# khiner/MeshEditor

Measured on AMD Instinct MI355X. Metric: eigenpairs/sec (K/M assembly + 50-mode solve, 100k-tet mesh), higher is better.
Workload: dtype f64; 1 GPU; cube_s100k: Kuhn mesh 105456 tets / 446631 DOF, NumModes=50 NumFemModes=65, P=10 excitation points, one mesh per GPU; eigenpairs_per_mesh=65, kept_modes_per_mesh=50, parallelism=mesh-per-gpu x1

## Files before the change

mesheditor_amd/csrc/lab/mh_lab.hip:

```cpp
#include "../mh_common.h"
#include "modalhip_lab.h"

#include <algorithm>

void mh_elementwise_apply(mh_context *ctx, const mh_system *sys, double sigma, const double *x, double *y, uint32_t w);

namespace {
constexpr int TB = 256;
__global__ void k_lab_ref_to_panel(const double *__restrict__ x, const uint32_t *__restrict__ perm, uint32_t nnodes, uint32_t width, double *__restrict__ panel) {
    const size_t i = size_t(blockIdx.x) * blockDim.x + threadIdx.x;
    if (i >= size_t(nnodes) * 3 * width) return;
    const uint32_t c = uint32_t(i % width), comp = uint32_t((i / width) % 3), node = uint32_t(i / (size_t(3) * width));
    panel[i] = x[size_t(c) * (size_t(3) * nnodes) + size_t(3) * perm[node] + comp];
}
__global__ void k_lab_panel_to_ref(const double *__restrict__ panel, const uint32_t *__restrict__ perm, uint32_t nnodes, uint32_t width, double *__restrict__ y) {
    const size_t i = size_t(blockIdx.x) * blockDim.x + threadIdx.x;
    if (i >= size_t(nnodes) * 3 * width) return;
    const uint32_t c = uint32_t(i % width), comp = uint32_t((i / width) % 3), node = uint32_t(i / (size_t(3) * width));
    y[size_t(c) * (size_t(3) * nnodes) + size_t(3) * perm[node] + comp] = panel[i];
}
}

namespace {
typedef float f4_stream __attribute__((ext_vector_type(4)));
__global__ void __launch_bounds__(256) k_stream_copy(const f4_stream *__restrict__ src, f4_stream *__restrict__ dst, size_t count) {
    for (size_t i = size_t(blockIdx.x) * 256 + threadIdx.x; i < count; i += size_t(gridDim.x) * 256) dst[i] = src[i];
}
template<int U, bool NT, int T = 256, bool NTL = NT> __global__ void __launch_bounds__(T) k_stream_copy_u(const f4_stream *__restrict__ src, f4_stream *__restrict__ dst, size_t count) {
    const size_t stride = size_t(gridDim.x) * T;
    for (size_t base = size_t(blockIdx.x) * T + threadIdx.x; base < count; base += stride * U) {
        f4_stream v[U];
#pragma unroll
        for (int u = 0; u < U; ++u) {
            const size_t i = base + size_t(u) * stride;
            if (i < count) v[u] = NTL ? __builtin_nontemporal_load(src + i) : src[i];
        }
#pragma unroll
        for (int u = 0; u < U; ++u) {
            const size_t i = base + size_t(u) * stride;
            if (i < count) {
                if (NT) __builtin_nontemporal_store(v[u], dst + i);
                else dst[i] = v[u];
            }
        }
    }
}
template<int U, bool NT> __global__ void __launch_bounds__(256) k_stream_read_u(const f4_stream *__restrict__ src, size_t count, float *__restrict__ out) {
    const size_t stride = size_t(gridDim.x) * 256;
    f4_stream acc = {0, 0, 0, 0};
    for (size_t base = size_t(blockIdx.x) * 256 + threadIdx.x; base < count; base += stride * U) {
        f4_stream v[U];
#pragma unroll
        for (int u = 0; u < U; ++u) {
            const size_t i = base + size_t(u) * stride;
            v[u] = i < count ? (NT ? __builtin_nontemporal_load(src + i) : src[i]) : f4_stream{0, 0, 0, 0};
        }
#pragma unroll
        for (int u = 0; u < U; ++u) acc += v[u];
    }
    float s = acc[0] + acc[1] + acc[2] + acc[3];
    for (int off = 32; off > 0; off >>= 1) s += __shfl_xor(s, off, 64);
    if ((threadIdx.x & 63) == 0) atomicAdd(out + blockIdx.x, s);
}
__global__ void __launch_bounds__(256) k_stream_read(const f4_stream *__restrict__ src, size_t count, float *__restrict__ out) {
    f4_stream acc = {0, 0, 0, 0};
    for (size_t i = size_t(blockIdx.x) * 256 + threadIdx.x; i < count; i += size_t(gridDim.x) * 256) acc += src[i];
    float s = acc[0] + acc[1] + acc[2] + acc[3];
    for (int off = 32; off > 0; off >>= 1) s += __shfl_xor(s, off, 64);
    if ((threadIdx.x & 63) == 0) atomicAdd(out + blockIdx.x, s);
}
}

namespace {
std::vector<uint32_t> lab_point_ref(const mh_system *s) {
    const std::vector<uint32_t> perm = s->perm.to_host(), corner = s->p1_corner.to_host();
    std::vector<uint32_t> ref(s->n_points);
    std::vector<uint8_t> seen(s->n_points, 0);
    for (uint32_t p = 0; p < s->n_points; ++p) {
        ref[p] = perm[corner[p]];
        if (ref[p] >= s->n_points || seen[ref[p]]) mh_throw(MH_EINVAL, "hierarchy export: P1 point %u has reference id %u", p, ref[p]);
        seen[ref[p]] = 1;
    }
    return ref;
}
const PatchSet &lab_patches(const mh_system *s, int level) { return level == 2 ? s->patches2 : s->patches1; }
}

extern "C" {
uint32_t mhl_graph_aggregates(const uint32_t *row_ptr, const uint32_t *col, uint32_t n, uint32_t target, uint32_t max_order, uint32_t *agg_of) {
    std::vector<uint32_t> rp(row_ptr, row_ptr + n + 1), cl(col, col + row_ptr[n]), out;
    const uint32_t na = mh_graph_aggregates(rp, cl, n, target, max_order, out);
    std::copy(out.begin(), out.end(), agg_of);
    return na;
}

int mhl_system_elementwise_matvec(mh_system *s, const double *x, double *y, uint32_t width) {
    if (!s || !x || !y || width == 0) return MH_EINVAL;
    mh_context *ctx = s->ctx;
    try {
        HIP_CHECK(hipSetDevice(ctx->device));
        const size_t n = size_t(3) * s->n_nodes;
        DevArray<double> xr(ctx, n * width), xp(ctx, n * width), yp(ctx, n * width);
        xr.upload(x, n * width);
        k_lab_ref_to_panel<<<div_up(n * width, TB), TB, 0, ctx->stream>>>(xr, s->perm, s->n_nodes, width, xp);
        KERNEL_CHECK();
        mh_elementwise_apply(ctx, s, -15791.367041742974, xp, yp, width);
        k_lab_panel_to_ref<<<div_up(n * width, TB), TB, 0, ctx->stream>>>(yp, s->perm, s->n_nodes, width, xr.get());
        KERNEL_CHECK();
        xr.download(y, n * width);
        return MH_OK;
    } catch (const std::exception &e) { return mh_guard(ctx, e); }
}

int mhl_system_bench_spmm(mh_system *s, uint32_t width, uint32_t reps, double *avg_ms, double *algorithmic_bytes) {
    if (!s || width == 0 || reps == 0 || !avg_ms) return MH_EINVAL;
    mh_context *ctx = s->ctx;
    try {
        HIP_CHECK(hipSetDevice(ctx->device));
        const size_t n = size_t(3) * s->n_nodes;
        DevArray<double> x(ctx, n * width), y(ctx, n * width);
        std::vector<double> hx(n * width);
        for (size_t i = 0; i < hx.size(); ++i) hx[i] = double((i * 2654435761u) % 1000) * 1e-3 - 0.5;
        x.upload(hx.data(), hx.size());
        HIP_CHECK(hipStreamSynchronize(ctx->stream));
        for (int warm = 0; warm < 2; ++warm) mh_spmm(ctx, s->L2, s->L2.kval, x, y, nullptr, nullptr, width);
        hipEvent_t e0, e1;
        HIP_CHECK(hipEventCreate(&e0));
        HIP_CHECK(hipEventCreate(&e1));
        HIP_CHECK(hipEventRecord(e0, ctx->stream));
        for (uint32_t r = 0; r < reps; ++r) mh_spmm(ctx, s->L2, s->L2.kval, x, y, nullptr, nullptr, width);
        HIP_CHECK(hipEventRecord(e1, ctx->stream));
        HIP_CHECK(hipEventSynchronize(e1));
        float ms = 0;
        HIP_CHECK(hipEventElapsedTime(&ms, e0, e1));
        (void)hipEventDestroy(e0);
        (void)hipEventDestroy(e1);
        *avg_ms = ms / reps;
        if (algorithmic_bytes) *algorithmic_bytes = 76.0 * double(s->L2.n_blocks) + 4.0 * (double(s->n_nodes) + 1) + 16.0 * double(n) * width;
        return MH_OK;
    } catch (const std::exception &e) { return mh_guard(ctx, e); }
}

int mhl_system_bench_cheb_step(mh_system *s, int level, uint32_t width, uint32_t slabs, uint32_t reps, double *avg_ms) {
    if (!s || !avg_ms || width == 0 || slabs == 0 || width % (4 * slabs) || reps == 0 || (level != 1 && level != 2)) return MH_EINVAL;
    mh_context *ctx = s->ctx;
    try {
        HIP_CHECK(hipSetDevice(ctx->device));
        const BsrLevel &lvl = level == 2 ? s->L2 : s->L1;
        if (!lvl.aval32.get() || !lvl.dinv32.get()) mh_throw(MH_EINVAL, "bench_cheb_step: no single-precision operator (solve the system once first)");
        const size_t n = size_t(3) * lvl.n_nodes;
        const uint32_t wc = width / slabs;
        std::vector<DevArray<float>> d(slabs), d2(slabs), r(slabs), x(slabs);
        std::vector<float> h(n * wc);
        for (size_t i = 0; i < h.size(); ++i) h[i] = float((i * 2654435761u) % 1000) * 1e-3f - 0.5f;
        for (uint32_t q = 0; q < slabs; ++q) {
            for (auto *a : {&d[q], &d2[q], &r[q], &x[q]}) {
                a->reset(ctx, n * wc);
                a->upload(h.data(), h.size());
            }
        }
        HIP_CHECK(hipStreamSynchronize(ctx->stream));
        auto run = [&] {
            for (uint32_t q = 0; q < slabs; ++q)
                if (!mh_spmm_f32_cheb_step(ctx, lvl, d[q], d2[q], r[q], x[q], lvl.dinv32, 0.3f, 0.1f, wc)) mh_throw(MH_EINVAL, "bench_cheb_step: width %u not served by the wide kernel", wc);
        };
        run();
        run();
        hipEvent_t e0, e1;
        HIP_CHECK(hipEventCreate(&e0));
        HIP_CHECK(hipEventCreate(&e1));
        HIP_CHECK(hipEventRecord(e0, ctx->stream));
        for (uint32_t rep = 0; rep < reps; ++rep) run();
        HIP_CHECK(hipEventRecord(e1, ctx->stream));
        HIP_CHECK(hipEventSynchronize(e1));
        float ms = 0;
        HIP_CHECK(hipEventElapsedTime(&ms, e0, e1));
        (void)hipEventDestroy(e0);
        (void)hipEventDestroy(e1);
        *avg_ms = ms / reps;
        return MH_OK;
    } catch (const std::exception &e) { return mh_guard(ctx, e); }
}

int mhl_system_bench_elementwise(mh_system *s, uint32_t width, uint32_t reps, double *avg_ms) {
    if (!s || width == 0 || reps == 0 || !avg_ms) return MH_EINVAL;
    mh_context *ctx = s->ctx;
    try {
        HIP_CHECK(hipSetDevice(ctx->device));
        const size_t n = size_t(3) * s->n_nodes;
        DevArray<double> x(ctx, n * width), y(ctx, n * width);
        std::vector<double> hx(n * width);
        for (size_t i = 0; i < hx.size(); ++i) hx[i] = double((i * 2654435761u) % 1000) * 1e-3 - 0.5;
        x.upload(hx.data(), hx.size());
        HIP_CHECK(hipStreamSynchronize(ctx->stream));
        for (int warm = 0; warm < 2; ++warm) mh_elementwise_apply(ctx, s, -15791.367041742974, x, y, width);
        hipEvent_t e0, e1;
        HIP_CHECK(hipEventCreate(&e0));
        HIP_CHECK(hipEventCreate(&e1));
        HIP_CHECK(hipEventRecord(e0, ctx->stream));
        for (uint32_t r = 0; r < reps; ++r) mh_elementwise_apply(ctx, s, -15791.367041742974, x, y, width);
        HIP_CHECK(hipEventRecord(e1, ctx->stream));
        HIP_CHECK(hipEventSynchronize(e1));
        float ms = 0;
        HIP_CHECK(hipEventElapsedTime(&ms, e0, e1));
        (void)hipEventDestroy(e0);
        (void)hipEventDestroy(e1);
        *avg_ms = ms / reps;
        return MH_OK;
    } catch (const std::exception &e) { return mh_guard(ctx, e); }
}

}

namespace {
double lab_mapped_update_mismatches(mh_context *ctx, bool gaps, size_t n, uint32_t wa, uint32_t wb) {
    const uint32_t b = (wa + wa / 2 + 3u) & ~1u, pitch = (wa + 1u) & ~1u, m = wa + 2 * wb, nc = wa + wb;
    std::vector<uint32_t> map(wa);
    for (uint32_t k = 0; k < wa; ++k) map[k] = gaps ? k + k / 2 : k;
    auto fill = [](std::vector<double> &v, size_t salt) {
        for (size_t i = 0; i < v.size(); ++i) v[i] = double(((i + salt) * 2654435761u) % 1000) * 1e-3 - 0.5;
    };
    std::vector<double> hx(n * b), hw(n * wb), hp(n * wb), hc(size_t(m) * nc);
    fill(hx, 0), fill(hw, 7919), fill(hp, 104729), fill(hc, 1299709);
    struct Out { std::vector<double> xn, x, p; };
    auto run = [&](int form) {
        DevArray<double> dx(ctx, n * b), dw(ctx, n * wb), dp(ctx, n * wb), dc(ctx, size_t(m) * nc), dxn(ctx, n * pitch), dpo(ctx, n * wb);
        DevArray<uint32_t> dmap(ctx, wa);
        dx.upload(hx.data(), hx.size());
        dw.upload(hw.data(), hw.size());
        dp.upload(hp.data(), hp.size());
        dc.upload(hc.data(), hc.size());
        dmap.upload(map.data(), wa);
        dxn.zero();
        if (form == 0) mh_combine(ctx, n, dx, wa, dw, wb, dp, wb, dc, nc, dxn, wa, dpo, false, b, dmap, pitch);
        else mh_combine(ctx, n, dx, wa, dw, wb, dp, wb, dc, nc, dxn, wa, dpo, false, b, dmap, pitch, nullptr, 0, 0, dx, b, dmap);
        Out o{std::vector<double>(n * pitch), std::vector<double>(n * b), std::vector<double>(n * wb)};
        dxn.download(o.xn.data(), o.xn.size());
        dx.download(o.x.data(), o.x.size());
        dpo.download(o.p.data(), o.p.size());
        return o;
    };
    const Out one = run(0), two = run(1);
    auto differing = [](const std::vector<double> &a, const std::vector<double> &c) {
        size_t d = 0;
        for (size_t i = 0; i < a.size(); ++i) d += !(a[i] == c[i]);
        return d;
    };
    size_t bad = differing(one.x, hx);
    for (size_t r = 0; r < n; ++r)
        for (uint32_t c = 0; c < nc; ++c) {
            double ref = 0, mag = 0;
            for (uint32_t k = 0; k < m; ++k) {
                const double s = k < wa ? hx[r * b + map[k]] : k < wa + wb ? hw[r * wb + (k - wa)] : hp[r * wb + (k - wa - wb)];
                ref += s * hc[size_t(k) * nc + c];
                mag += std::abs(s * hc[size_t(k) * nc + c]);
            }
            const double got = c < wa ? one.xn[r * pitch + c] : one.p[r * wb + (c - wa)];
            bad += !(std::abs(got - ref) <= 2.0 * m * 2.3e-16 * mag);
        }
    std::vector<double> want = hx;
    size_t written = 0;
    for (size_t r = 0; r < n; ++r)
        for (uint32_t k = 0; k < wa; ++k) {
            want[r * b + map[k]] = one.xn[r * pitch + k];
            written += want[r * b + map[k]] != hx[r * b + map[k]];
        }
    if (written < n * wa / 2) mh_throw(MH_EHIP, "mapped update check: the update left %zu of %zu entries as they were", n * wa - written, n * size_t(wa));
    bad += differing(two.xn, one.xn) + differing(two.x, want) + differing(two.p, one.p);
    return double(bad);
}
}

extern "C" {
int mhl_context_bench_dense(mh_context *ctx, int kind, uint64_t n, uint32_t wa, uint32_t wb, uint32_t reps, double *avg_ms) {
    if (!ctx || !avg_ms || n == 0 || wa == 0 || wb == 0 || reps == 0 || kind < 0 || kind > 3) return MH_EINVAL;
    try {
        HIP_CHECK(hipSetDevice(ctx->device));
        std::lock_guard<std::mutex> lock(mh_solve_mutex());
        if (kind >= 2) {
            *avg_ms = lab_mapped_update_mismatches(ctx, kind == 3, n, wa, wb);
            return MH_OK;
        }
        DevArray<double> x(ctx, n * wa), y(ctx, n * wb), g(ctx, size_t(wa + wb) * (wa + wb)), z(ctx, n * wa);
        std::vector<double> h(n * std::max(wa, wb));
        for (size_t i = 0; i < h.size(); ++i) h[i] = double((i * 2654435761u) % 1000) * 1e-3 - 0.5;
        x.upload(h.data(), n * wa);
        y.upload(h.data(), n * wb);
        g.upload(h.data(), g.count);
        HIP_CHECK(hipStreamSynchronize(ctx->stream));
        auto run = [&]() {
            if (kind == 0) mh_gram(ctx, n, x, wa, y, wb, g, wa);
            else mh_combine(ctx, n, x, wa, y, wb, nullptr, 0, g, wa, z, wa, nullptr);
        };
        run();
        hipEvent_t e0, e1;
        HIP_CHECK(hipEventCreate(&e0));
        HIP_CHECK(hipEventCreate(&e1));
        HIP_CHECK(hipEventRecord(e0, ctx->stream));
        for (uint32_t r = 0; r < reps; ++r) run();
        HIP_CHECK(hipEventRecord(e1, ctx->stream));
        HIP_CHECK(hipEventSynchronize(e1));
        float ms = 0;
        HIP_CHECK(hipEventElapsedTime(&ms, e0, e1));
        (void)hipEventDestroy(e0);
        (void)hipEventDestroy(e1);
        *avg_ms = ms / reps;
        return MH_OK;
    } catch (const std::exception &e) { return mh_guard(ctx, e); }
}

int mhl_context_tridiagonalize_full(mh_context *ctx, int variant, uint32_t m, const double *a, double *d, double *e, double *reflectors, double *tau, uint32_t reps, double *avg_ms);
int mhl_context_tridiagonalize(mh_context *ctx, int variant, uint32_t m, const double *a, double *d, double *e, uint32_t reps, double *avg_ms) {
    return mhl_context_tridiagonalize_full(ctx, variant, m, a, d, e, nullptr, nullptr, reps, avg_ms);
}

int mhl_context_tridiagonalize_full(mh_context *ctx, int variant, uint32_t m, const double *a, double *d, double *e, double *reflectors, double *tau, uint32_t reps, double *avg_ms) {
    if (!ctx || !a || !d || !e || m < 2 || variant < 0 || variant > 3 || m > (variant == 2 ? 768u : 256u)) return MH_EINVAL;
    try {
        HIP_CHECK(hipSetDevice(ctx->device));
        MhSharedPhase not_during_a_factorisation(ctx->device);
        DevArray<double> da(ctx, size_t(m) * m), work(ctx, size_t(m) * m), dd(ctx, m), de(ctx, m), dtau(ctx, m);
        da.upload(a, size_t(m) * m);
        hipEvent_t e0, e1;
        HIP_CHECK(hipEventCreate(&e0));
        HIP_CHECK(hipEventCreate(&e1));
        float total = 0;
        for (uint32_t r = 0; r < std::max(1u, reps); ++r) {
            HIP_CHECK(hipMemcpyAsync(work, da, size_t(m) * m * sizeof(double), hipMemcpyDeviceToDevice, ctx->stream));
            HIP_CHECK(hipEventRecord(e0, ctx->stream));
            if (variant == 2) mh_sytrd_wide(ctx, work, m, dd, de, dtau);
            else mh_sytrd_small(ctx, work, m, dd, de, dtau, variant);
            HIP_CHECK(hipEventRecord(e1, ctx->stream));
            HIP_CHECK(hipEventSynchronize(e1));
            float ms = 0;
            HIP_CHECK(hipEventElapsedTime(&ms, e0, e1));
            total += ms;
        }
        (void)hipEventDestroy(e0);
        (void)hipEventDestroy(e1);
        dd.download(d, m);
        de.download(e, m - 1);
        if (reflectors) work.download(reflectors, size_t(m) * m);
        if (tau) dtau.download(tau, m);
        if (mh_sytrd_gave_up(ctx)) mh_throw(MH_EHIP, "tridiagonalisation: a workgroup timed out waiting for the others' values");
        if (avg_ms) *avg_ms = total / std::max(1u, reps);
        return MH_OK;
    } catch (const std::exception &e) { return mh_guard(ctx, e); }
}

int mhl_context_tridiag_lowest(mh_context *ctx, uint32_t m, uint32_t k, const double *d, const double *e, double *w, double *z, double *quality, int *taken) {
    if (!ctx || !d || !e || !w || !z || !quality || !taken || m < 2 || m > 768 || k < 1) return MH_EINVAL;
    try {
        HIP_CHECK(hipSetDevice(ctx->device));
        MhSharedPhase not_during_a_factorisation(ctx->device);
        DevArray<double> dd(ctx, m), de(ctx, m), dw(ctx, k), dz(ctx, size_t(m) * k);
        dd.upload(d, m);
        de.zero();
        de.upload(e, m - 1);
        bool ok;
        double q = std::numeric_limits<double>::quiet_NaN();
        if (m <= 256) {
            DevArray<double> ufac(ctx, size_t(3) * m * k), qv(ctx, 8), lam(ctx, k);
            ok = mh_tridiag_lowest(ctx, dd, de, m, k, dw, dz, m, ufac, qv, lam);
            if (ok) qv.download(&q, 1);
        } else {
            DevArray<double> work(ctx, size_t(5) * k * m + size_t(2) * k * k + 8);
            DevArray<int> info(ctx, 2);
            ok = mh_tridiag_lowest_wide(ctx, dd, de, m, k, dw, dz, m, work, info, &q);
        }
        *taken = ok ? 1 : 0;
        if (ok) {
            dw.download(w, k);
            dz.download(z, size_t(m) * k);
            *quality = q;
        }
        HIP_CHECK(hipStreamSynchronize(ctx->stream));
        return MH_OK;
    } catch (const std::exception &ex) { return mh_guard(ctx, ex); }
}

int mhl_context_rr_solve(mh_context *ctx, uint32_t m, const double *a, const double *mmat, uint32_t nwant, int gm_is_identity, double *evals, double *vectors, uint32_t *ncols,
                         double *host_evals, double *trace) {
    if (!ctx || !a || (!mmat && !gm_is_identity) || !evals || !vectors || !ncols || !trace || m < 1 || m > 1024 || nwant > m) return MH_EINVAL;
    struct TraceOn {
        mh_context *ctx;
        ~TraceOn() { ctx->rr_trace = nullptr; }
    };
    try {
        HIP_CHECK(hipSetDevice(ctx->device));
        MhSharedPhase not_during_a_factorisation(ctx->device);
        const size_t mm = size_t(m) * m;
        DevArray<double> gA(ctx, mm), gM(ctx, mm), ev(ctx, m), ework(ctx, m);
        DevArray<int> info(ctx, 2);
        info.zero();
        gA.upload(a, mm);
        if (mmat) gM.upload(mmat, mm);
        else gM.zero();
        if (ctx->rr_check) HIP_CHECK(hipMemsetAsync(ctx->rr_check, 0, sizeof(unsigned long long), ctx->stream));
        MhRrTrace tr;
        std::vector<double> hv;
        int hinfo;
        {
            ctx->rr_trace = &tr;
            TraceOn off{ctx};
            hinfo = mh_rr_solve(ctx, gA, gM, m, ev, ework, info, nwant, gm_is_identity != 0, host_evals ? &hv : nullptr);
        }
        unsigned long long check = 0;
        if (ctx->rr_check) HIP_CHECK(hipMemcpyAsync(&check, ctx->rr_check, sizeof(check), hipMemcpyDeviceToHost, ctx->stream));
        HIP_CHECK(hipStreamSynchronize(ctx->stream));
        double checkd;
        memcpy(&checkd, &check, sizeof(checkd));
        const bool partial = tr.solver == MhRrTrace::SMALL_PARTIAL || tr.solver == MhRrTrace::WIDE_PARTIAL;
        *ncols = hinfo ? 0 : (partial ? nwant : m);
        trace[0] = tr.reduction, trace[1] = tr.defect, trace[2] = tr.solver, trace[3] = tr.quality, trace[4] = checkd, trace[5] = double(hv.size());
        if (hinfo) return MH_EFACTOR;
        ev.download(evals, *ncols);
        gA.download(vectors, size_t(m) * *ncols);
        if (host_evals && !hv.empty()) std::copy(hv.begin(), hv.end(), host_evals);
        return MH_OK;
    } catch (const std::exception &ex) { return mh_guard(ctx, ex); }
}

int mhl_system_precondition(mh_system *s, double sigma, int precision, const double *x, double *y, uint32_t width) {
    if (!s || !x || !y || width == 0 || width > 1024 || (precision != 0 && precision != 1)) return MH_EINVAL;
    mh_context *ctx = s->ctx;
    try {
        HIP_CHECK(hipSetDevice(ctx->device));
        const size_t n = size_t(3) * s->n_nodes;
        DevArray<double> xr(ctx, n * width), xp(ctx, n * width), yp(ctx, n * width);
        xr.upload(x, n * width);
        k_lab_ref_to_panel<<<div_up(n * width, TB), TB, 0, ctx->stream>>>(xr, s->perm, s->n_nodes, width, xp);
        KERNEL_CHECK();
        mh_precondition_panel(s, sigma, precision, xp, yp, width);
        k_lab_panel_to_ref<<<div_up(n * width, TB), TB, 0, ctx->stream>>>(yp, s->perm, s->n_nodes, width, xr.get());
        KERNEL_CHECK();
        xr.download(y, n * width);
        return MH_OK;
    } catch (const std::exception &e) { return mh_guard(ctx, e); }
}

int mhl_system_hierarchy_sizes(mh_system *s, double sigma, int rebuild, uint64_t *sizes) {
    if (!s || !sizes) return MH_EINVAL;
    mh_context *ctx = s->ctx;
    try {
        HIP_CHECK(hipSetDevice(ctx->device));
        std::lock_guard<std::mutex> lock(mh_solve_mutex());
        if (rebuild) s->hierarchy_ready = false;
        mh_build_hierarchy(s, sigma);
        sizes[0] = s->n_points, sizes[1] = s->n_agg, sizes[2] = uint64_t(6) * s->n_agg, sizes[3] = s->L1.n_blocks;
        for (int level : {2, 1}) {
            const PatchSet &ps = lab_patches(s, level);
            uint64_t *o = sizes + (level == 2 ? 4 : 12);
            o[0] = ps.n_patches, o[1] = ps.npe, o[2] = ps.n_clusters, o[3] = ps.cluster_rows, o[4] = ps.cinv64.count, o[5] = ps.n_bad_elements,
            o[6] = ps.largest_cluster, o[7] = s->dropped_patches[level == 2 ? 0 : 1];
        }
        return MH_OK;
    } catch (const std::exception &e) { return mh_guard(ctx, e); }
}

int mhl_system_hierarchy_export(mh_system *s, uint32_t width, double *scalars, uint32_t *agg_of, double *agg_t, uint32_t *l1_row, uint32_t *l1_col, double *l1_val,
                                double *a0) {
    if (!s || !scalars || width == 0) return MH_EINVAL;
    mh_context *ctx = s->ctx;
    try {
        HIP_CHECK(hipSetDevice(ctx->device));
        std::lock_guard<std::mutex> lock(mh_solve_mutex());
        if (!s->hierarchy_ready) mh_throw(MH_EINVAL, "hierarchy export: no hierarchy built");
        MhCycleShape sh;
        mh_cycle_shape(s, width, &sh);
        const double sc[10] = {s->L2.lmax, s->L1.lmax, mh_coarse_lift(s), double(sh.deg2), sh.ratio, double(sh.deg1), double(sh.gamma), sh.ratio1, s->sigma_built,
                               double(s->worst_quality)};
        std::copy(sc, sc + 10, scalars);
        const std::vector<uint32_t> ref = lab_point_ref(s);
        if (agg_of) {
            const std::vector<uint32_t> h = s->agg_of.to_host();
            for (uint32_t p = 0; p < s->n_points; ++p) agg_of[ref[p]] = h[p];
        }
        if (agg_t) {
            const std::vector<double> h = s->agg_t.to_host();
            for (uint32_t p = 0; p < s->n_points; ++p) std::copy(h.begin() + 18 * size_t(p), h.begin() + 18 * size_t(p + 1), agg_t + 18 * size_t(ref[p]));
        }
        if (l1_row || l1_col) {
            const std::vector<uint32_t> rp = s->L1.row_ptr.to_host(), cl = s->L1.col.to_host();
            for (uint32_t r = 0; r < s->L1.n_nodes; ++r)
                for (uint32_t b = rp[r]; b < rp[r + 1]; ++b) {
                    if (l1_row) l1_row[b] = ref[r];
                    if (l1_col) l1_col[b] = ref[cl[b]];
                }
        }
        if (l1_val) s->L1.aval.download(l1_val, s->L1.n_blocks * 9);
        if (a0) s->a0.download(a0, s->a0.count);
        return MH_OK;
    } catch (const std::exception &e) { return mh_guard(ctx, e); }
}

int mhl_system_patch_export(mh_system *s, int level, uint32_t *nodes, double *weight, double *inv64, uint32_t *cluster_row, uint32_t *cluster_ptr, double *cinv64) {
    if (!s || (level != 1 && level != 2)) return MH_EINVAL;
    mh_context *ctx = s->ctx;
    try {
        HIP_CHECK(hipSetDevice(ctx->device));
        std::lock_guard<std::mutex> lock(mh_solve_mutex());
        if (!s->hierarchy_ready) mh_throw(MH_EINVAL, "patch export: no hierarchy built");
        const PatchSet &ps = lab_patches(s, level);
        std::vector<uint32_t> node_ref;
        if (level == 2) node_ref = s->perm.to_host();
        else node_ref = lab_point_ref(s);
        if (nodes && ps.n_patches) {
            const std::vector<uint32_t> h = ps.nodes.to_host();
            for (size_t i = 0; i < h.size(); ++i) nodes[i] = node_ref[h[i]];
        }
        if (weight && ps.n_patches) ps.weight.download(weight, ps.n_patches);
        if (inv64 && ps.n_patches) ps.inv64.download(inv64, ps.inv64.count);
        if (cluster_row && ps.n_clusters) {
            const std::vector<uint32_t> h = ps.cluster_row.to_host();
            for (size_t i = 0; i < h.size(); ++i) cluster_row[i] = 3 * node_ref[h[i] / 3] + h[i] % 3;
        }
        if (cluster_ptr && ps.n_clusters) std::copy(ps.h_cluster_ptr.begin(), ps.h_cluster_ptr.end(), cluster_ptr);
        if (cinv64 && ps.n_clusters) ps.cinv64.download(cinv64, ps.cinv64.count);
        return MH_OK;
    } catch (const std::exception &e) { return mh_guard(ctx, e); }
}

int mhl_context_potrf_inverse(mh_context *ctx, uint32_t w, const double *a, const double *dscale, double *l, double *linv, int *info2) {
    if (!ctx || !a || !dscale || !l || !linv || !info2 || w < 1 || w > 128) return MH_EINVAL;
    try {
        HIP_CHECK(hipSetDevice(ctx->device));
        MhSharedPhase not_during_a_factorisation(ctx->device);
        DevArray<double> da(ctx, size_t(w) * w), dd(ctx, w), dl(ctx, size_t(w) * w);
        DevArray<int> info(ctx, 2);
        da.upload(a, size_t(w) * w);
        dd.upload(dscale, w);
        mh_potrf_small_inverse(ctx, da, w, info, dd, dl);
        da.download(l, size_t(w) * w);
        dl.download(linv, size_t(w) * w);
        info.download(info2, 2);
        return MH_OK;
    } catch (const std::exception &e) { return mh_guard(ctx, e); }
}

int mhl_context_spd_inverse(mh_context *ctx, uint32_t w, const double *a, double *out, uint32_t reps, double *avg_ms) {
    if (!ctx || !a || !out || w < 1 || w > 128) return MH_EINVAL;
    try {
        HIP_CHECK(hipSetDevice(ctx->device));
        MhSharedPhase not_during_a_factorisation(ctx->device);
        DevArray<double> da(ctx, size_t(w) * w), dout(ctx, size_t(w) * w);
        DevArray<int> info(ctx, 1);
        info.zero();
        da.upload(a, size_t(w) * w);
        hipEvent_t e0, e1;
        HIP_CHECK(hipEventCreate(&e0));
        HIP_CHECK(hipEventCreate(&e1));
        float total = 0;
        for (uint32_t r = 0; r < std::max(1u, reps); ++r) {
            HIP_CHECK(hipEventRecord(e0, ctx->stream));
            mh_spd_inverse_small(ctx, da, w, w, dout, w, info);
            HIP_CHECK(hipEventRecord(e1, ctx->stream));
            HIP_CHECK(hipEventSynchronize(e1));
            float ms = 0;
            HIP_CHECK(hipEventElapsedTime(&ms, e0, e1));
            total += ms;
        }
        (void)hipEventDestroy(e0);
        (void)hipEventDestroy(e1);
        dout.download(out, size_t(w) * w);
        int hinfo = 0;
        info.download(&hinfo, 1);
        if (avg_ms) *avg_ms = total / std::max(1u, reps);
        return hinfo ? MH_EFACTOR : MH_OK;
    } catch (const std::exception &e) { return mh_guard(ctx, e); }
}

int mhl_context_small_gemm(mh_context *ctx, int ta, int tb, uint32_t M, uint32_t N, uint32_t K, double alpha, const double *a, uint32_t lda, const double *b, uint32_t ldb, double beta,
                           double *c, uint32_t ldc, uint32_t reps, double *avg_ms) {
    if (!ctx || !a || !b || !c || !M || !N || !K || lda < (ta ? K : M) || ldb < (tb ? N : K) || ldc < M) return MH_EINVAL;
    try {
        HIP_CHECK(hipSetDevice(ctx->device));
        MhSharedPhase not_during_a_factorisation(ctx->device);
        const size_t na = size_t(lda) * (ta ? M : K), nb = size_t(ldb) * (tb ? K : N), nc = size_t(ldc) * N;
        DevArray<double> da(ctx, na), db(ctx, nb), dc(ctx, nc), work(ctx, nc);
        da.upload(a, na);
        db.upload(b, nb);
// ... 232 lines not shown
```

mesheditor_amd/csrc/mh_common.h:

```cpp
#pragma once
#include "../../include/modalhip.h"

#include <hip/hip_runtime.h>
#include <rocblas/rocblas.h>
#include <rocsolver/rocsolver.h>

#include <algorithm>
#include <cstdarg>
#include <cstdio>
#include <cstdlib>
#include <cstring>
#include <iterator>
#include <limits>
#include <atomic>
#include <map>
#include <memory>
#include <mutex>
#include <stdexcept>
#include <string>
#include <vector>

struct MhError : std::runtime_error {
    int code;
    MhError(int c, const std::string &m) : std::runtime_error(m), code(c) {}
// ... 239 lines not shown
            ahead_ev.push_back(e);
        }
        return aux2_stream != nullptr;
    }
    rocblas_handle blas{nullptr};
    rocblas_handle blas_aux{nullptr};
    DevicePool pool;
    std::string last_error;
    hipEvent_t ev0{nullptr}, ev1{nullptr};
    void *gram_ws{nullptr};
    size_t gram_ws_bytes{0};
    uint32_t *iota{nullptr};
    unsigned long long *sytrd_xch{nullptr};
    uint32_t sytrd_epoch{0};
    int *sytrd_flag{nullptr};
    unsigned long long *sytrd_xch_wide{nullptr};
    uint32_t sytrd_epoch_wide{0};
    bool exchange_disabled{false};
    uint32_t sytrd_redos{0};
    unsigned long long *rr_check{nullptr};
    struct MhRrTrace *rr_trace{nullptr};
    bool time_kernels{false};
    std::vector<std::pair<hipEvent_t, hipEvent_t>> timer_events;
    std::vector<double> timer_work;
    std::vector<int> timer_class;
    size_t timer_used{0};
    struct ClassTotals {
        double ms{0}, work{0};
        uint64_t launches{0};
    } totals[MH_KERNEL_CLASSES];
};
void mh_timer_flush(mh_context *ctx);
struct TimedLaunch {
    mh_context *ctx;
    bool on;
    size_t slot{0};
    TimedLaunch(mh_context *c, int kernel_class, double work) : ctx(c), on(c->time_kernels) {
        if (!on) return;
        if (ctx->timer_used == ctx->timer_events.size()) {
            hipEvent_t a, b;
            HIP_CHECK(hipEventCreate(&a));
            HIP_CHECK(hipEventCreate(&b));
            ctx->timer_events.emplace_back(a, b);
            ctx->timer_work.push_back(0);
            ctx->timer_class.push_back(0);
        }
        slot = ctx->timer_used++;
        ctx->timer_work[slot] = work;
        ctx->timer_class[slot] = kernel_class;
        HIP_CHECK(hipEventRecord(ctx->timer_events[slot].first, ctx->stream));
    }
    ~TimedLaunch() {
        if (on) (void)hipEventRecord(ctx->timer_events[slot].second, ctx->stream);
    }
    TimedLaunch(const TimedLaunch &) = delete;
    TimedLaunch &operator=(const TimedLaunch &) = delete;
};

template<typename T> struct DevArray {
    mh_context *ctx{nullptr};
    T *ptr{nullptr};
    size_t count{0};
    bool owned{true};
    DevArray() = default;
    DevArray(mh_context *c, size_t n) { reset(c, n); }
    DevArray(const DevArray &) = delete;
    DevArray &operator=(const DevArray &) = delete;
    DevArray(DevArray &&o) noexcept : ctx(o.ctx), ptr(o.ptr), count(o.count), owned(o.owned) { o.ptr = nullptr; o.count = 0; o.owned = true; }
    DevArray &operator=(DevArray &&o) noexcept {
        if (this != &o) {
            free();
            ctx = o.ctx; ptr = o.ptr; count = o.count; owned = o.owned;
            o.ptr = nullptr; o.count = 0; o.owned = true;
        }
        return *this;
    }
    void alias_of(const DevArray &o) {
        free();
        ctx = o.ctx; ptr = o.ptr; count = o.count;
        owned = false;
    }
    ~DevArray() { free(); }
    void reset(mh_context *c, size_t n) {
        free();
        ctx = c;
        count = n;
        ptr = n ? static_cast<T *>(c->pool.alloc(n * sizeof(T))) : nullptr;
        static const bool poison = getenv("MH_TEST") && strstr(getenv("MH_TEST"), "poison");
        if (poison && ptr) (void)hipMemsetAsync(ptr, 0xff, n * sizeof(T), c->stream);
    }
    void free() {
        if (ptr && ctx && owned) ctx->pool.release(ptr);
        ptr = nullptr;
        count = 0;
        owned = true;
    }
    T *get() const { return ptr; }
    operator T *() const { return ptr; }
    void zero() const { if (ptr) HIP_CHECK(hipMemsetAsync(ptr, 0, count * sizeof(T), ctx->stream)); }
    void upload(const T *src, size_t n) const { HIP_CHECK(hipMemcpyAsync(ptr, src, n * sizeof(T), hipMemcpyHostToDevice, ctx->stream)); }
    void download(T *dst, size_t n) const {
        HIP_CHECK(hipMemcpyAsync(dst, ptr, n * sizeof(T), hipMemcpyDeviceToHost, ctx->stream));
        HIP_CHECK(hipStreamSynchronize(ctx->stream));
    }
    std::vector<T> to_host() const {
        std::vector<T> h(count);
        if (count) download(h.data(), count);
        return h;
    }
};

struct MhLevelStructure {
    uint32_t n_nodes{0};
    uint64_t n_blocks{0};
    DevArray<uint32_t> row_ptr, col;
    DevArray<uint32_t> seg, pay;
};
struct mh_structure {
    mh_context *ctx{nullptr};
    uint32_t n_points{0}, kept_tets{0}, n_nodes{0}, n_edges{0};
    DevArray<double> points;
    DevArray<uint32_t> tets;
    DevArray<uint32_t> elem_nodes_ref, elem_nodes, elem_p1;
    DevArray<double> elem_basis;
    DevArray<uint32_t> perm, inv_perm;
    bool relative{false};
    double origin[3]{0, 0, 0};
    double node_box[6]{0, 0, 0, 0, 0, 0};
    DevArray<double> node_xyz, p1_xyz;
    DevArray<uint32_t> parent_a, parent_b, p1_edge_ptr, p1_edge_mid, p1_corner;
    DevArray<double> tables2, tables1, support2, support1;
    MhLevelStructure L2, L1;
    uint32_t agg_target{16}, n_agg{0};
    DevArray<uint32_t> agg_of, agg_ptr, agg_nodes;
    DevArray<double> agg_t;
    uint32_t n_components{1}, unreferenced_points{0};
    DevArray<uint32_t> node_component;
    DevArray<double> component_centroid;
    uint64_t device_bytes() const;
};

struct mh_mesh {
    mh_context *ctx;
    uint32_t n_points{0}, n_tets{0};
    DevArray<double> points;
    DevArray<uint32_t> tets;
    mutable std::mutex structure_mutex;
    mutable std::shared_ptr<const mh_structure> structure;
    mutable std::atomic<uint64_t> structure_builds{0};
};

struct BsrLevel {
    int id{0};
    uint32_t n_nodes{0};
    uint64_t n_blocks{0};
    DevArray<uint32_t> row_ptr;
    DevArray<uint32_t> col;
    DevArray<double> kval;
    DevArray<double> mval;
    DevArray<double> aval;
    DevArray<double> dinv;
    DevArray<float> aval32, dinv32;
    double lmax{0};
};

struct PatchSet {
    uint32_t npe{0}, n_patches{0}, n_touched{0};
    DevArray<uint32_t> nodes;
    DevArray<double> inv64;
    DevArray<double> weight;
    DevArray<int> dropped;
    DevArray<float> inv32;
    DevArray<uint32_t> touched, t_ptr, t_patch, t_local;
    uint32_t n_clusters{0}, cluster_rows{0}, cluster_tiles{0};
    uint32_t n_bad_elements{0};
    uint32_t largest_cluster{0};
    std::vector<uint32_t> h_cluster_ptr;
    DevArray<uint32_t> cluster_row;
    DevArray<uint32_t> cluster_ptr;
    DevArray<uint64_t> cluster_inv_ptr;
    DevArray<uint32_t> tile_cluster, tile_row0;
    DevArray<double> cinv64;
    DevArray<float> cinv32;
    bool any() const { return n_patches || n_clusters; }
    static constexpr int kClusterSlices = 8;
    size_t scratch_rows() const { return size_t(n_patches) * 3 * npe + size_t(cluster_rows) * kClusterSlices; }
};

struct mh_system {
    mh_context *ctx;
    std::shared_ptr<const mh_structure> structure;
    uint32_t dropped_patches[2]{0, 0};
    double plain_residual{-1.0};
    mh_material material{};
    uint32_t n_points{0}, kept_tets{0}, n_nodes{0}, n_edges{0};
    bool lmax_widened{false};
    DevArray<double> points;
    DevArray<uint32_t> elem_nodes_ref;
    DevArray<uint32_t> elem_nodes;
    DevArray<double> elem_basis;
    DevArray<uint32_t> perm;
    DevArray<uint32_t> inv_perm;
    DevArray<double> node_xyz;
    DevArray<uint32_t> parent_a, parent_b;
    DevArray<uint32_t> p1_edge_ptr, p1_edge_mid;
    DevArray<uint32_t> p1_corner;
    DevArray<double> p1_xyz;
    BsrLevel L2, L1;
    uint32_t agg_target{16}, n_agg{0};
    DevArray<uint32_t> agg_of, agg_ptr, agg_nodes;
    DevArray<double> agg_t;
    DevArray<double> a0;
    uint32_t n_components{1};
    uint32_t unreferenced_points{0};
    DevArray<uint32_t> node_component;
    DevArray<double> component_centroid;
    PatchSet patches2, patches1;
    DevArray<uint32_t> elem_p1;
    float worst_quality{1.f};
    double sigma_built{0};
    bool hierarchy_ready{false};
    hipEvent_t coarse_done{nullptr};
    bool coarse_pending{false};
    double coarse_lift{0};
    DevArray<double> coarse_ws[5];
    DevArray<int> coarse_info;
    ~mh_system() {
        if (coarse_pending && coarse_done) (void)hipEventSynchronize(coarse_done);
        if (coarse_done) (void)hipEventDestroy(coarse_done);
    }
    DevArray<double> evecs;
    uint32_t evec_cols{0};
    mh_profile profile{};
};

inline int mh_guard(mh_context *ctx, const std::exception &e) {
    if (ctx) ctx->last_error = e.what();
    if (auto *m = dynamic_cast<const MhError *>(&e)) return m->code;
    return MH_EHIP;
}

#define MH_TRY(ctx_expr, body)                         \
    mh_context *ctx_guard_ = (ctx_expr);               \
    try {                                              \
        body;                                          \
        return MH_OK;                                  \
    } catch (const std::exception &e) {                \
        return mh_guard(ctx_guard_, e);                \
    }

inline unsigned div_up(size_t a, size_t b) { return unsigned((a + b - 1) / b); }

struct PerDeviceOnce {
    static constexpr int MaxDevices = 64;
    std::once_flag flag[MaxDevices];
    template<typename F> void run(int device, F &&f) { std::call_once(flag[device >= 0 && device < MaxDevices ? device : 0], std::forward<F>(f)); }
};

void mh_phase_shared_lock(int device);
void mh_phase_shared_unlock(int device);
struct MhSharedPhase {
    const int device;
    explicit MhSharedPhase(int dev) : device(dev) { mh_phase_shared_lock(device); }
    ~MhSharedPhase() { mh_phase_shared_unlock(device); }
    MhSharedPhase(const MhSharedPhase &) = delete;
    MhSharedPhase &operator=(const MhSharedPhase &) = delete;
};
std::mutex &mh_solve_mutex();
void mh_build_system(mh_context *ctx, const mh_mesh *mesh, const mh_material &mat, mh_system *sys);
void mh_build_hierarchy(mh_system *sys, double sigma, bool defer = false);
void mh_finish_hierarchy(mh_system *sys);
uint32_t mh_shift_invert_panel(mh_system *sys, double sigma, const double *b, double *x, uint32_t w, double rel_tol, uint32_t max_iters, double *worst_rel);
struct MhCycleShape {
    int deg2{2}, deg1{5}, gamma{3};
    double ratio{8.0}, ratio1{0.0};
};
void mh_cycle_shape(const mh_system *sys, uint32_t w, MhCycleShape *shape);
double mh_coarse_lift(const mh_system *sys);
void mh_precondition_panel(mh_system *sys, double sigma, int precision, const double *r, double *z, uint32_t w);
uint32_t mh_graph_aggregates(const std::vector<uint32_t> &row_ptr, const std::vector<uint32_t> &col, uint32_t n, uint32_t target, uint32_t max_order, std::vector<uint32_t> &agg_of);
void mh_select_patches(mh_system *sys, float threshold);
void mh_build_patch_inverses(mh_context *ctx, const BsrLevel &lvl, PatchSet &ps);
template<typename T>
void mh_apply_patches(mh_context *ctx, const PatchSet &ps, const T *in, const T *minus, uint32_t w, T coef, T *d, T *x, double *z, uint32_t wz, T *scratch);
void mh_gram(mh_context *ctx, size_t n, const double *x, uint32_t wa, const double *y, uint32_t wb, double *g, uint32_t ld, uint32_t ldy = 0, const uint32_t *ymap = nullptr);
void mh_combine(mh_context *ctx, size_t n, const double *x, uint32_t wx, const double *w, uint32_t ww, const double *p, uint32_t wp, const double *ct, uint32_t nc,
                double *out1, uint32_t n1, double *out2, bool accumulate = false, uint32_t ldx = 0, const uint32_t *xmap = nullptr, uint32_t ld1 = 0,
                const uint32_t *omap = nullptr, uint32_t col_begin = 0, uint32_t col_count = 0,
                double *out1_also = nullptr, uint32_t ld1_also = 0, const uint32_t *omap_also = nullptr);
bool mh_tridiag_lowest_wide(mh_context *ctx, const double *d, const double *e, uint32_t m, uint32_t k, double *w, double *z, uint32_t ldz, double *work, int *info2,
                            double *quality_host);
void mh_apply_q(mh_context *ctx, const double *a, const double *tau, uint32_t m, double *z, uint32_t ldz, uint32_t ncols);
bool mh_tridiag_lowest(mh_context *ctx, const double *d, const double *e, uint32_t m, uint32_t k, double *w, double *z, uint32_t ldz, double *ufac,
                       double *quality, double *lam_scratch);
struct MhRrTrace {
    enum Reduction { GIVEN_IDENTITY = 0, MEASURED_IDENTITY = 1, SERIES = 2, CHOLESKY = 3 };
    enum Solver { SYEVD = 0, SMALL_PARTIAL = 1, SMALL_STEDC = 2, WIDE_PARTIAL = 3, WIDE_STEDC_ORMTR = 4 };
    int reduction{-1};
    double defect{-1};
    int solver{-1};
    double quality{std::numeric_limits<double>::quiet_NaN()};
};
int mh_rr_solve(mh_context *ctx, double *gA, double *gM, uint32_t m, double *evals, double *ework, DevArray<int> &info, uint32_t nwant = 0, bool gm_is_identity = false,
                std::vector<double> *host_evals = nullptr);
void mh_spd_inverse_small(mh_context *ctx, const double *a, uint32_t lda, uint32_t w, double *out, uint32_t ldo, int *info);
void mh_potrf(mh_context *ctx, double *a, uint32_t ld, uint32_t w, int *info);
void mh_potrf_small(mh_context *ctx, double *a, uint32_t w, int *info);
void mh_potrf_small_inverse(mh_context *ctx, double *a, uint32_t w, int *info, const double *dscale, double *linv);
bool mh_sytrd_gave_up(mh_context *ctx);
void mh_sytrd_wide(mh_context *ctx, double *a, uint32_t m, double *d, double *e, double *tau);
void mh_sytrd_small(mh_context *ctx, double *a, uint32_t m, double *d, double *e, double *tau, int variant = -1);
void mh_small_gemm(mh_context *ctx, bool ta, bool tb, uint32_t M, uint32_t N, uint32_t K, double alpha, const double *a, uint32_t lda, const double *b, uint32_t ldb, double beta, double *c,
                   uint32_t ldc);
void mh_short_product(mh_context *ctx, size_t n, const double *a, uint32_t m, const double *ct, uint32_t nc, double *out, double *partial, uint32_t slices);
void mh_pack_stacked(mh_context *ctx, const double *c1, uint32_t r1, const double *c2, uint32_t r2, uint32_t cols, double scale, double *ct);
void mh_pack_coefficients(mh_context *ctx, const double *c1, uint32_t n1, const double *c2, uint32_t n2, uint32_t m, uint32_t ld, double *ct);
void mh_spmm_mapped(mh_context *ctx, const BsrLevel &lvl, const double *vals9, const double *x, double *y, const double *mscal, double *y2, uint32_t w, uint32_t ldy,
                    uint32_t wreal, const uint32_t *omap, const double *res_theta = nullptr, double *res_out = nullptr, double *res_partial = nullptr,
                    const double *res_dinv = nullptr);
bool mh_spmm_f32_cheb_step(mh_context *ctx, const BsrLevel &lvl, const float *d_in, float *d_out, float *r, float *x, const float *dinv, float c1, float c2,
                           uint32_t w);
void mh_spmm_f32(mh_context *ctx, const BsrLevel &lvl, const float *x, float *y, uint32_t w);
void mh_spmm_mixed(mh_context *ctx, const BsrLevel &lvl, const float *x, double *y, uint32_t w);
const uint32_t *mh_identity_map(mh_context *ctx);
void mh_spmm(mh_context *ctx, const BsrLevel &lvl, const double *vals9, const double *x, double *y, const double *mscal, double *y2, uint32_t w);
```

mesheditor_amd/csrc/mh_eigs.hip:

```cpp
#include "mh_common.h"

#include <algorithm>
#include <cmath>
#include <memory>
#include <condition_variable>
#include <mutex>
#include <numeric>
#include <optional>
#include <type_traits>

__global__ void k_shift_values(const double *kval, const double *mval, size_t nblocks, double sigma, double *aval, float *aval32);
__global__ void k_diag_inverse(const uint32_t *row_ptr, const uint32_t *col, const double *aval, uint32_t nnodes, double *dinv);
__global__ void k_coarse_matrix(const uint32_t *row_ptr, const uint32_t *col, const double *aval, const double *tmat, const uint32_t *agg_of, const uint32_t *agg_ptr,
                                const uint32_t *agg_nodes, uint32_t nagg, double *a0);
__global__ void k_fix_coarse_diag(double *a0, uint32_t n0, double rel);

namespace {
constexpr int TB = 256;

std::mutex g_solve_mutex;
struct Switches {
    bool verbose = getenv("MH_VERBOSE") != nullptr;
    bool fp32_prec = !(getenv("MH_PRECOND_FP64") && atoi(getenv("MH_PRECOND_FP64")) != 0);
    int deg2 = 0, deg1 = 0, gamma = 0;
    double cheb_ratio = 0.0, cheb_ratio1 = 0.0;
    bool test_sytrd_giveup = getenv("MH_TEST") && strstr(getenv("MH_TEST"), "sytrd_giveup");
    bool no_tridiag_wide = getenv("MH_TEST") && strstr(getenv("MH_TEST"), "no_tridiag_wide");
    bool test_last_resort = getenv("MH_TEST") && strstr(getenv("MH_TEST"), "last_resort");
    bool test_coarse_pivot = getenv("MH_TEST") && strstr(getenv("MH_TEST"), "coarse_pivot");
    bool test_selfcheck_fail = getenv("MH_TEST") && strstr(getenv("MH_TEST"), "selfcheck_fail");
    bool lmax_low = getenv("MH_TEST") && strstr(getenv("MH_TEST"), "lmax_low");
    bool potrf_chain = getenv("MH_TEST") && strstr(getenv("MH_TEST"), "potrf_chain");
    bool no_poly_start = getenv("MH_TEST") && strstr(getenv("MH_TEST"), "no_poly_start");
    bool fresh_structure = getenv("MH_TEST") && strstr(getenv("MH_TEST"), "fresh_structure");
    bool copy_passes = getenv("MH_TEST") && strstr(getenv("MH_TEST"), "copy_passes");
    Switches() {
        if (const char *c = getenv("MH_CYCLE")) {
            double v[5] = {0, 0, 0, 0, 0};
            sscanf(c, "%lf,%lf,%lf,%lf,%lf", &v[0], &v[1], &v[2], &v[3], &v[4]);
            deg2 = std::max(0, int(v[0])), deg1 = std::max(0, int(v[1])), gamma = std::max(0, int(v[2]));
            cheb_ratio = v[3];
            cheb_ratio1 = v[4];
        }
    }
};
const Switches &switches() {
    static const Switches s;
    return s;
}
constexpr int kPowerIterations = 20;
constexpr uint32_t kPrecondColumns = 256;
constexpr uint32_t kSkipP = 4;
constexpr uint32_t kGuardPercent = 10;
constexpr float kFlatShape = 1e-4f;
constexpr size_t kDenseLastResort = 12288;
constexpr int kLastResortCg = 8;

struct PhaseLock {
    std::mutex m;
    std::condition_variable cv;
    int readers = 0, writers_waiting = 0;
    bool writer = false;
    void lock_shared() {
        std::unique_lock<std::mutex> l(m);
        cv.wait(l, [&] { return !writer && writers_waiting == 0; });
        ++readers;
    }
    void unlock_shared() {
        std::unique_lock<std::mutex> l(m);
        if (--readers == 0) cv.notify_all();
    }
    void lock() {
        std::unique_lock<std::mutex> l(m);
        ++writers_waiting;
        cv.wait(l, [&] { return !writer && readers == 0; });
        --writers_waiting;
        writer = true;
    }
    void unlock() {
        std::unique_lock<std::mutex> l(m);
        writer = false;
        cv.notify_all();
    }
};
constexpr int kMaxDevices = 64;
PhaseLock g_phase_of_device[kMaxDevices];
PhaseLock &phase_of(int device) { return g_phase_of_device[unsigned(device) % kMaxDevices]; }
const bool g_concurrent = !(getenv("MH_CONCURRENT_SOLVES") && atoi(getenv("MH_CONCURRENT_SOLVES")) == 0);
struct SharedPhase {
    PhaseLock &phase;
    bool held = false, enabled = true;
    explicit SharedPhase(int device, bool on = true) : phase(phase_of(device)), enabled(on) { acquire(); }
    ~SharedPhase() { release(); }
    void acquire() { if (g_concurrent && enabled && !held) { phase.lock_shared(); held = true; } }
    void release() { if (held) { phase.unlock_shared(); held = false; } }
};
struct ExclusivePhase {
    PhaseLock &phase;
    bool held = false;
    explicit ExclusivePhase(int device) : phase(phase_of(device)) {
        if (g_concurrent) {
            phase.lock();
            held = true;
            (void)hipSetDevice(device);
            (void)hipDeviceSynchronize();
        }
    }
    ~ExclusivePhase() { if (held) phase.unlock(); }
};

struct Timer {
    mh_context *ctx;
    hipEvent_t a, b;
    explicit Timer(mh_context *c) : ctx(c) {
        HIP_CHECK(hipEventCreate(&a));
        HIP_CHECK(hipEventCreate(&b));
        HIP_CHECK(hipEventRecord(a, ctx->stream));
    }
    double stop() {
        HIP_CHECK(hipEventRecord(b, ctx->stream));
        HIP_CHECK(hipEventSynchronize(b));
        float ms = 0;
        HIP_CHECK(hipEventElapsedTime(&ms, a, b));
        return ms * 1e-3;
    }
    ~Timer() {
        (void)hipEventDestroy(a);
        (void)hipEventDestroy(b);
    }
};

__global__ void k_random_panel(double *__restrict__ x, size_t rows, uint32_t w, uint32_t col0, uint64_t seed) {
    const size_t j = size_t(blockIdx.x) * blockDim.x + threadIdx.x;
    const uint32_t wf = w - col0;
    if (j >= rows * wf) return;
    const size_t i = (j / wf) * w + col0 + j % wf;
    auto mix = [](uint64_t z) {
        z += 0x9e3779b97f4a7c15ull;
        z = (z ^ (z >> 30)) * 0xbf58476d1ce4e5b9ull;
        z = (z ^ (z >> 27)) * 0x94d049bb133111ebull;
        return z ^ (z >> 31);
    };
    const uint64_t a = mix(seed + 2 * i), b = mix(seed + 2 * i + 1);
    const double u1 = (double(a >> 11) + 1.0) * (1.0 / 9007199254740993.0), u2 = double(b >> 11) * (1.0 / 9007199254740992.0);
    x[i] = sqrt(-2.0 * log(u1)) * cos(6.283185307179586 * u2);
}

template<typename T>
__global__ void k_cheb_init(const T *__restrict__ b, const T *__restrict__ t, const T *__restrict__ dinv, T inv_theta, T *__restrict__ r, T *__restrict__ d,
                            T *__restrict__ x, int accumulate, size_t rows, uint32_t w) {
    const size_t i = size_t(blockIdx.x) * blockDim.x + threadIdx.x;
    if (i >= rows * w) return;
    const T rv = t ? b[i] - t[i] : b[i];
    const T dv = dinv[i / w] * rv * inv_theta;
    r[i] = rv;
    d[i] = dv;
    x[i] = accumulate ? x[i] + dv : dv;
}
typedef float f4_t __attribute__((ext_vector_type(4)));
__global__ void k_cheb_init_v4(const f4_t *__restrict__ b, const f4_t *__restrict__ t, const float *__restrict__ dinv, float inv_theta, f4_t *__restrict__ r,
                               f4_t *__restrict__ d, f4_t *__restrict__ x, int accumulate, size_t rows, uint32_t w4) {
    const size_t i = size_t(blockIdx.x) * blockDim.x + threadIdx.x;
    if (i >= rows * w4) return;
    const f4_t rv = t ? b[i] - t[i] : b[i];
    const f4_t dv = (dinv[i / w4] * inv_theta) * rv;
    r[i] = rv;
    d[i] = dv;
    x[i] = accumulate ? x[i] + dv : dv;
}
__global__ void k_cheb_last_v4(const f4_t *__restrict__ t, const float *__restrict__ dinv, float c1, float c2, const f4_t *__restrict__ r, const f4_t *__restrict__ d,
                               const f4_t *__restrict__ x, double *__restrict__ z, size_t rows, uint32_t w4, uint32_t wo) {
    const size_t i = size_t(blockIdx.x) * blockDim.x + threadIdx.x;
    if (i >= rows * w4) return;
    const size_t row = i / w4;
    const uint32_t c = uint32_t(i % w4) * 4;
    const f4_t rv = r[i] - t[i];
    const f4_t zv = x[i] + (c1 * d[i] + (c2 * dinv[row]) * rv);
#pragma unroll
    for (int e = 0; e < 4; ++e)
        if (c + e < wo) z[row * wo + c + e] = double(zv[e]);
}
__global__ void k_prolong_p1_v4(const f4_t *__restrict__ x1, const uint32_t *__restrict__ pa, const uint32_t *__restrict__ pb, f4_t *__restrict__ x2, uint32_t nnodes,
                                uint32_t w4) {
    const size_t i = size_t(blockIdx.x) * blockDim.x + threadIdx.x;
    if (i >= size_t(nnodes) * 3 * w4) return;
    const uint32_t c = uint32_t(i % w4), comp = uint32_t((i / w4) % 3), node = uint32_t(i / (size_t(3) * w4));
    const uint32_t a = pa[node], bb = pb[node];
    const f4_t va = x1[(size_t(3) * a + comp) * w4 + c];
    x2[i] += a == bb ? va : 0.5f * (va + x1[(size_t(3) * bb + comp) * w4 + c]);
}
struct PanelColumns {
    uint32_t pitch;
    uint32_t count;
    const uint32_t *map;
    __device__ __forceinline__ size_t at(size_t row, uint32_t c) const { return row * pitch + (map ? map[c] : c); }
};
__global__ void k_cheb_init_convert(const double *__restrict__ src, PanelColumns sc, const float *__restrict__ dinv, float inv_theta, float *__restrict__ b32,
                                    float *__restrict__ r, float *__restrict__ d, float *__restrict__ x, size_t rows, uint32_t w) {
    const size_t i = size_t(blockIdx.x) * blockDim.x + threadIdx.x;
    if (i >= rows * w) return;
    const size_t row = i / w;
    const uint32_t c = uint32_t(i % w);
    const float rv = c < sc.count ? float(src[sc.at(row, c)]) : 0.f;
    const float dv = dinv[row] * rv * inv_theta;
    b32[i] = rv;
    r[i] = rv;
    d[i] = dv;
    x[i] = dv;
}
template<typename T>
__global__ void k_cheb_step(const T *__restrict__ t, const T *__restrict__ dinv, T c1, T c2, T *__restrict__ r, T *__restrict__ d, T *__restrict__ x, size_t rows,
                            uint32_t w) {
    const size_t i = size_t(blockIdx.x) * blockDim.x + threadIdx.x;
    if (i >= rows * w) return;
    const T rv = r[i] - t[i];
    const T dv = c1 * d[i] + c2 * dinv[i / w] * rv;
    r[i] = rv;
    d[i] = dv;
    x[i] += dv;
}
template<typename T>
__global__ void k_cheb_last(const T *__restrict__ t, const T *__restrict__ dinv, T c1, T c2, const T *__restrict__ r, const T *__restrict__ d, const T *__restrict__ x,
                            double *__restrict__ z, size_t rows, uint32_t w, uint32_t wo) {
    const size_t i = size_t(blockIdx.x) * blockDim.x + threadIdx.x;
    if (i >= rows * w) return;
    const size_t row = i / w;
    const uint32_t c = uint32_t(i % w);
    if (c >= wo) return;
    const T rv = r[i] - t[i];
    z[row * wo + c] = double(x[i] + (c1 * d[i] + c2 * dinv[row] * rv));
}
template<typename S, typename D> __global__ void k_convert(const S *__restrict__ src, D *__restrict__ dst, size_t count) {
    const size_t i = size_t(blockIdx.x) * blockDim.x + threadIdx.x;
    if (i < count) dst[i] = D(src[i]);
}
template<typename S, typename D> __global__ void k_convert_pitch(const S *__restrict__ src, uint32_t ws, D *__restrict__ dst, uint32_t wd, size_t rows) {
    const size_t i = size_t(blockIdx.x) * blockDim.x + threadIdx.x;
    if (i >= rows * wd) return;
    const size_t row = i / wd;
    const uint32_t c = uint32_t(i % wd);
    dst[i] = c < ws ? D(src[row * ws + c]) : D(0);
}

template<typename T>
__global__ void k_restrict_p1(const T *__restrict__ b, const T *__restrict__ t, const uint32_t *__restrict__ p1_corner, const uint32_t *__restrict__ eptr,
                              const uint32_t *__restrict__ emid, T *__restrict__ r1, uint32_t npts, uint32_t w, PanelColumns bc = PanelColumns{0, 0, nullptr}) {
    const size_t i = size_t(blockIdx.x) * blockDim.x + threadIdx.x;
    if (i >= size_t(npts) * 3 * w) return;
    const uint32_t c = uint32_t(i % w), comp = uint32_t((i / w) % 3), p = uint32_t(i / (size_t(3) * w));
    if (!bc.pitch) bc.pitch = bc.count = w;
    auto res = [&](uint32_t node) {
        const size_t row = size_t(3) * node + comp;
        return (c < bc.count ? b[bc.at(row, c)] : T(0)) - t[row * w + c];
    };
    T s = res(p1_corner[p]);
    T h = 0;
    for (uint32_t e = eptr[p]; e < eptr[p + 1]; ++e) h += res(emid[e]);
    r1[i] = s + T(0.5) * h;
}
template<typename T>
__global__ void k_prolong_p1(const T *__restrict__ x1, const uint32_t *__restrict__ pa, const uint32_t *__restrict__ pb, T *__restrict__ x2, uint32_t nnodes,
                             uint32_t w) {
    const size_t i = size_t(blockIdx.x) * blockDim.x + threadIdx.x;
    if (i >= size_t(nnodes) * 3 * w) return;
    const uint32_t c = uint32_t(i % w), comp = uint32_t((i / w) % 3), node = uint32_t(i / (size_t(3) * w));
    const uint32_t a = pa[node], bb = pb[node];
    const T va = x1[(size_t(3) * a + comp) * w + c];
    x2[i] += a == bb ? va : T(0.5) * (va + x1[(size_t(3) * bb + comp) * w + c]);
}
template<typename T>
__global__ void k_restrict_agg(const T *__restrict__ b, const T *__restrict__ t, const double *__restrict__ tmat, double *__restrict__ r0,
                               const uint32_t *__restrict__ agg_ptr, const uint32_t *__restrict__ agg_nodes, uint32_t nagg, uint32_t w) {
    const size_t i = size_t(blockIdx.x) * blockDim.x + threadIdx.x;
    if (i >= size_t(nagg) * 6 * w) return;
    const uint32_t c = uint32_t(i % w), q = uint32_t((i / w) % 6), a = uint32_t(i / (size_t(6) * w));
    double s = 0;
    for (uint32_t l = agg_ptr[a]; l < agg_ptr[a + 1]; ++l) {
        const uint32_t nd = agg_nodes[l];
        const double *tm = tmat + 18 * size_t(nd);
        for (int p = 0; p < 3; ++p) {
            const size_t o = (size_t(3) * nd + p) * w + c;
            s += tm[6 * p + q] * double(b[o] - t[o]);
        }
    }
    r0[i] = s;
}
template<typename T>
__global__ void k_prolong_agg(const double *__restrict__ x0, const double *__restrict__ tmat, T *__restrict__ x1, const uint32_t *__restrict__ agg_of, uint32_t npts,
                              uint32_t w) {
    const size_t i = size_t(blockIdx.x) * blockDim.x + threadIdx.x;
    if (i >= size_t(npts) * 3 * w) return;
    const uint32_t c = uint32_t(i % w), p = uint32_t((i / w) % 3), nd = uint32_t(i / (size_t(3) * w));
    const uint32_t a = agg_of[nd];
    const double *tm = tmat + 18 * size_t(nd) + 6 * p;
    double s = 0;
    for (int q = 0; q < 6; ++q) s += tm[q] * x0[(size_t(6) * a + q) * w + c];
    x1[i] += T(s);
}

__global__ void k_residual(const double *__restrict__ ax, const double *__restrict__ mx, const double *__restrict__ theta, const uint32_t *__restrict__ idx,
                           double *__restrict__ r, size_t rows, uint32_t b, uint32_t w) {
    const size_t i = size_t(blockIdx.x) * blockDim.x + threadIdx.x;
    if (i >= rows * w) return;
    const uint32_t k = uint32_t(i % w);
    const size_t row = i / w;
    const uint32_t src = idx ? idx[k] : k;
    r[i] = ax[row * b + src] - theta[src] * mx[row * b + src];
}

__global__ void k_residual_norms(const double *__restrict__ ax, const double *__restrict__ mx, const double *__restrict__ xx, const double *__restrict__ theta,
                                 double near_limit, double *__restrict__ r, size_t rows, uint32_t b, uint32_t rows_per_block, double *__restrict__ partial,
                                 const double *__restrict__ dinv) {
    const uint32_t c = blockIdx.y * blockDim.x + threadIdx.x;
    if (c >= b) return;
    const size_t r0 = size_t(blockIdx.x) * rows_per_block, r1 = min(rows, r0 + rows_per_block);
    const double th = theta[c];
    const bool need_x = fabs(th) < near_limit;
    double sr = 0, sm = 0, sx = 0;
    for (size_t row = r0; row < r1; ++row) {
        const size_t i = row * b + c;
        const double m = mx[i], res = ax[i] - th * m;
        const double wgt = dinv ? dinv[row] : 1.0;
        r[i] = res;
        sr += res * res * wgt;
        sm += m * m * wgt;
        if (need_x) {
            const double x = xx[i];
            sx += dinv ? x * x / wgt : x * x;
        }
    }
    double *p = partial + size_t(blockIdx.x) * 3 * b;
    p[c] = sr;
    p[b + c] = sm;
    p[2 * size_t(b) + c] = sx;
}

__global__ void k_colsumsq_partial(const double *__restrict__ x, size_t rows, uint32_t w, double *__restrict__ partial, uint32_t rows_per_block) {
    const uint32_t c = blockIdx.y * blockDim.x + threadIdx.x;
    if (c >= w) return;
    const size_t r0 = size_t(blockIdx.x) * rows_per_block, r1 = min(rows, r0 + rows_per_block);
    double s = 0;
    for (size_t r = r0; r < r1; ++r) {
        const double v = x[r * w + c];
        s += v * v;
    }
    partial[size_t(blockIdx.x) * w + c] = s;
}
__global__ void k_colsum_partial(const double *__restrict__ x, size_t rows, uint32_t w, double *__restrict__ partial, uint32_t rows_per_block) {
    const uint32_t c = blockIdx.y * blockDim.x + threadIdx.x;
    if (c >= w) return;
    const size_t r0 = size_t(blockIdx.x) * rows_per_block, r1 = min(rows, r0 + rows_per_block);
    double s = 0;
    for (size_t r = r0; r < r1; ++r) s += x[r * w + c];
    partial[size_t(blockIdx.x) * w + c] = s;
}
__global__ void k_colsumsq_final(const double *__restrict__ partial, uint32_t nblocks, uint32_t w, double *__restrict__ out) {
    __shared__ double s[256];
    const uint32_t c = blockIdx.x;
    double acc = 0;
    for (uint32_t b = threadIdx.x; b < nblocks; b += 256) acc += partial[size_t(b) * w + c];
    s[threadIdx.x] = acc;
    __syncthreads();
    for (int h = 128; h > 0; h >>= 1) {
        if (int(threadIdx.x) < h) s[threadIdx.x] += s[threadIdx.x + h];
        __syncthreads();
    }
    if (threadIdx.x == 0) out[c] = s[0];
}
__global__ void k_scale_cols_inv_sqrt(double *__restrict__ x, const double *__restrict__ sumsq, size_t rows, uint32_t w) {
    const size_t i = size_t(blockIdx.x) * blockDim.x + threadIdx.x;
    if (i >= rows * w) return;
    const double s = sumsq[i % w];
    x[i] *= s > 0 ? rsqrt(s) : 0.0;
}
__global__ void k_dinv_mul(const double *__restrict__ t, const double *__restrict__ dinv, double *__restrict__ v, size_t rows, uint32_t w) {
    const size_t i = size_t(blockIdx.x) * blockDim.x + threadIdx.x;
    if (i < rows * w) v[i] = dinv[i / w] * t[i];
}

__global__ void k_set_identity_blocks(double *__restrict__ ga, double *__restrict__ gm, const double *__restrict__ theta, uint32_t b, uint32_t ld) {
    const uint32_t i = blockIdx.x * blockDim.x + threadIdx.x;
    if (i >= b) return;
    ga[size_t(i) * ld + i] = theta[i];
    gm[size_t(i) * ld + i] = 1.0;
}
__global__ void k_place_block(double *__restrict__ dst, uint32_t ld, const double *__restrict__ src, uint32_t w) {
    const uint32_t i = blockIdx.x * blockDim.x + threadIdx.x;
    if (i >= w * w) return;
    const uint32_t r = i % w, c = i / w;
    dst[size_t(c) * ld + r] = src ? src[size_t(c) * w + r] : (r == c ? 1.0 : 0.0);
}
__global__ void k_scale_gram(double *__restrict__ g, uint32_t w, uint32_t ld, double *__restrict__ dscale) {
    const uint32_t i = blockIdx.x * blockDim.x + threadIdx.x;
    if (i >= w * w) return;
    const uint32_t r = i % w, c = i / w;
    const double dr = g[size_t(r) * ld + r], dc = g[size_t(c) * ld + c];
    const double sr = dr > 0 ? rsqrt(dr) : 0.0, sc = dc > 0 ? rsqrt(dc) : 0.0;
    if (r == c) dscale[r] = sr;
    g[size_t(w) * ld + size_t(c) * ld + r] = g[size_t(c) * ld + r] * sr * sc;
}
__global__ void k_unscale_chol(double *__restrict__ l, uint32_t w, uint32_t ld, const double *__restrict__ dscale) {
    const uint32_t i = blockIdx.x * blockDim.x + threadIdx.x;
    if (i >= w * w) return;
    const uint32_t r = i % w, c = i / w;
    if (r < c) { l[size_t(c) * ld + r] = 0; return; }
    const double d = dscale[r];
    l[size_t(c) * ld + r] = d > 0 ? l[size_t(c) * ld + r] / d : (r == c ? 1.0 : 0.0);
}
__global__ void k_build_cp(const double *__restrict__ c, const uint32_t *__restrict__ idx, uint32_t b, uint32_t m, uint32_t w, uint32_t ldc,
                           double *__restrict__ cp, uint32_t ldp) {
    const uint32_t i = blockIdx.x * blockDim.x + threadIdx.x;
    if (i >= m * w) return;
    const uint32_t r = i % m, k = i / m;
    cp[size_t(k) * ldp + r] = r < b ? 0.0 : c[size_t(idx ? idx[k] : k) * ldc + r];
}
__global__ void k_gather_cols(const double *__restrict__ src, const uint32_t *__restrict__ idx, double *__restrict__ dst, size_t rows, uint32_t wsrc, uint32_t w) {
    const size_t i = size_t(blockIdx.x) * blockDim.x + threadIdx.x;
    if (i >= rows * w) return;
    dst[i] = src[(i / w) * wsrc + idx[i % w]];
}
__global__ void k_scatter_cols(const double *__restrict__ src, const uint32_t *__restrict__ idx, double *__restrict__ dst, size_t rows, uint32_t wdst, uint32_t w) {
    const size_t i = size_t(blockIdx.x) * blockDim.x + threadIdx.x;
    if (i >= rows * w) return;
    dst[(i / w) * wdst + idx[i % w]] = src[i];
}
__global__ void k_scatter_cols_pitch(const double *__restrict__ src, uint32_t wsrc, const uint32_t *__restrict__ idx, double *__restrict__ dst, size_t rows, uint32_t wdst,
                                     uint32_t w) {
    const size_t i = size_t(blockIdx.x) * blockDim.x + threadIdx.x;
    if (i >= rows * w) return;
    dst[(i / w) * wdst + idx[i % w]] = src[(i / w) * wsrc + i % w];
}
__global__ void k_sub_block(double *__restrict__ dst, uint32_t ld, const double *__restrict__ src, uint32_t lds, uint32_t rows, uint32_t cols) {
    const uint32_t i = blockIdx.x * blockDim.x + threadIdx.x;
    if (i >= rows * cols) return;
    const uint32_t r = i % rows, c = i / rows;
    dst[size_t(c) * ld + r] -= src[size_t(c) * lds + r];
}
__global__ void k_wblock_fix(double *__restrict__ bw, uint32_t ld, const double *__restrict__ u, const double *__restrict__ v, uint32_t w) {
    const uint32_t i = blockIdx.x * blockDim.x + threadIdx.x;
    if (i >= w * w) return;
    const uint32_t r = i % w, c = i / w;
    bw[size_t(c) * ld + r] += v[size_t(c) * w + r] - u[size_t(c) * w + r] - u[size_t(r) * w + c];
}
__global__ void k_load_seed(const float *__restrict__ seed, const uint32_t *__restrict__ perm, uint32_t nnodes, uint32_t ncols, uint32_t b, double *__restrict__ x) {
    const size_t i = size_t(blockIdx.x) * blockDim.x + threadIdx.x;
    if (i >= size_t(nnodes) * 3 * ncols) return;
    const uint32_t c = uint32_t(i % ncols), comp = uint32_t((i / ncols) % 3), node = uint32_t(i / (size_t(3) * ncols));
    x[(size_t(3) * node + comp) * b + c] = double(seed[size_t(c) * (size_t(3) * nnodes) + size_t(3) * perm[node] + comp]);
}
__global__ void k_inject_rbm(const double *__restrict__ xyz, const uint32_t *__restrict__ component, const double *__restrict__ centroid, uint32_t ncomp, uint32_t nnodes,
                             double *__restrict__ x, uint32_t b, uint32_t col0) {
    const uint32_t i = blockIdx.x * blockDim.x + threadIdx.x;
    if (i >= nnodes) return;
    const uint32_t mine = component[i];
    const double rx = xyz[3 * size_t(i)] - centroid[3 * size_t(mine)], ry = xyz[3 * size_t(i) + 1] - centroid[3 * size_t(mine) + 1], rz = xyz[3 * size_t(i) + 2] - centroid[3 * size_t(mine) + 2];
    for (uint32_t c = 0; c < ncomp; ++c) {
        double *r0 = x + (size_t(3) * i) * b + col0 + 6 * c, *r1 = r0 + b, *r2 = r1 + b;
        const double on = c == mine ? 1.0 : 0.0;
        r0[0] = on; r1[0] = 0; r2[0] = 0;
        r0[1] = 0; r1[1] = on; r2[1] = 0;
        r0[2] = 0; r1[2] = 0; r2[2] = on;
        r0[3] = 0; r1[3] = -rz * on; r2[3] = ry * on;
        r0[4] = rz * on; r1[4] = 0; r2[4] = -rx * on;
        r0[5] = -ry * on; r1[5] = rx * on; r2[5] = 0;
    }
}
__device__ __forceinline__ unsigned long long mh_ordered_key(double v) {
    const unsigned long long u = (unsigned long long)__double_as_longlong(v);
    return (u >> 63) ? ~u : (u | 0x8000000000000000ull);
}
__device__ __forceinline__ double mh_from_ordered_key(unsigned long long k) {
    const unsigned long long u = (k >> 63) ? (k & 0x7fffffffffffffffull) : ~k;
    return __longlong_as_double((long long)u);
}
__global__ void k_bbox(const double *__restrict__ xyz, uint32_t nnodes, unsigned long long *__restrict__ box) {
    const uint32_t i = blockIdx.x * blockDim.x + threadIdx.x;
    for (int a = 0; a < 3; ++a) {
        double lo = i < nnodes ? xyz[3 * size_t(i) + a] : 1e300, hi = i < nnodes ? xyz[3 * size_t(i) + a] : -1e300;
        for (int off = 32; off > 0; off >>= 1) lo = fmin(lo, __shfl_xor(lo, off, 64)), hi = fmax(hi, __shfl_xor(hi, off, 64));
        if ((threadIdx.x & 63) == 0) {
            atomicMin(box + a, mh_ordered_key(lo));
            atomicMax(box + 3 + a, mh_ordered_key(hi));
        }
    }
}
__global__ void k_inject_poly(const double *__restrict__ xyz, const double *__restrict__ box, uint32_t nnodes, const uint32_t *__restrict__ triples, uint32_t ntriples,
                              double *__restrict__ x, uint32_t b, uint32_t col0) {
    const uint32_t i = blockIdx.x * blockDim.x + threadIdx.x;
    if (i >= nnodes) return;
    double t[3], L[3][7];
    for (int a = 0; a < 3; ++a) {
        const double lo = box[a], hi = box[3 + a];
        const double half = fmax(0.5 * (hi - lo), 1e-300);
        t[a] = (xyz[3 * size_t(i) + a] - 0.5 * (hi + lo)) / half;
        L[a][0] = 1.0, L[a][1] = t[a];
        for (int d = 2; d < 7; ++d) L[a][d] = ((2 * d - 1) * t[a] * L[a][d - 1] - (d - 1) * L[a][d - 2]) / d;
    }
    double *row[3] = {x + (size_t(3) * i) * b + col0, x + (size_t(3) * i + 1) * b + col0, x + (size_t(3) * i + 2) * b + col0};
    uint32_t col = 0;
    auto put = [&](double v0, double v1, double v2) {
        row[0][col] = v0, row[1][col] = v1, row[2][col] = v2;
        ++col;
    };
    put(t[0], 0, 0), put(0, t[1], 0), put(0, 0, t[2]), put(t[1], t[0], 0), put(t[2], 0, t[0]), put(0, t[2], t[1]);
    for (uint32_t q = 0; q < ntriples; ++q) {
        const uint32_t tr = triples[q];
        const double v = L[0][tr & 0xff] * L[1][(tr >> 8) & 0xff] * L[2][(tr >> 16) & 0xff];
        put(v, 0, 0), put(0, v, 0), put(0, 0, v);
    }
}
__global__ void k_copy_cols(const double *__restrict__ src, uint32_t wsrc, double *__restrict__ dst, uint32_t wdst, size_t rows, uint32_t ncols) {
    const size_t i = size_t(blockIdx.x) * blockDim.x + threadIdx.x;
    if (i >= rows * ncols) return;
    dst[(i / ncols) * wdst + i % ncols] = src[(i / ncols) * wsrc + i % ncols];
}
__global__ void k_bsr_to_dense(const uint32_t *__restrict__ row_ptr, const uint32_t *__restrict__ col, const double *__restrict__ v9, const double *__restrict__ ms,
                               uint32_t nnodes, double *__restrict__ a, double *__restrict__ m) {
    const uint32_t r = blockIdx.x * blockDim.x + threadIdx.x;
    if (r >= nnodes) return;
    const size_t n = size_t(3) * nnodes;
    for (uint32_t p = row_ptr[r]; p < row_ptr[r + 1]; ++p) {
        const uint32_t c = col[p];
        for (int i = 0; i < 3; ++i) {
            for (int j = 0; j < 3; ++j) a[(size_t(3) * c + j) * n + size_t(3) * r + i] = v9[9 * size_t(p) + 3 * i + j];
            m[(size_t(3) * c + i) * n + size_t(3) * r + i] = ms[p];
        }
    }
}
__global__ void k_colmajor_to_panel(const double *__restrict__ z, size_t n, uint32_t ncols, double *__restrict__ x) {
    const size_t i = size_t(blockIdx.x) * blockDim.x + threadIdx.x;
    if (i >= n * ncols) return;
    x[i] = z[size_t(i % ncols) * n + i / ncols];
}

__global__ void k_symmetrize_lower(double *__restrict__ a, uint32_t n, uint32_t ld) {
    const size_t i = size_t(blockIdx.x) * blockDim.x + threadIdx.x;
    if (i >= size_t(n) * n) return;
    const uint32_t r = uint32_t(i % n), c = uint32_t(i / n);
    if (r < c) a[size_t(c) * ld + r] = a[size_t(r) * ld + c];
}

unsigned grid1(size_t count) { return div_up(count, TB); }

void gram(mh_context *ctx, size_t n, const double *xa, uint32_t wa, const double *yb, uint32_t wb, double *g, uint32_t ld) {
    mh_gram(ctx, n, xa, wa, yb, wb, g, ld);
}
void panel_mul(mh_context *ctx, size_t n, const double *x, uint32_t wa, const double *c, uint32_t ld, double *z, uint32_t wz, double alpha, double beta) {
    if (!wz) return;
    if (!wa) return;
    ROCBLAS_CHECK(rocblas_dgemm(ctx->blas, rocblas_operation_transpose, rocblas_operation_none, wz, rocblas_int(n), wa, &alpha, c, ld, x, wa, &beta, z, wz));
}
void panel_trsm(mh_context *ctx, size_t n, double *wp, uint32_t w, const double *l, uint32_t ld) {
    const double one = 1;
    ROCBLAS_CHECK(rocblas_dtrsm(ctx->blas, rocblas_side_left, rocblas_fill_lower, rocblas_operation_none, rocblas_diagonal_non_unit, w, rocblas_int(n), &one, l, ld, wp, w));
}


void small_dgemm(mh_context *ctx, rocblas_operation ta, rocblas_operation tb, rocblas_int M, rocblas_int N, rocblas_int K, const double *alpha, const double *a, rocblas_int lda, const double *b,
                 rocblas_int ldb, const double *beta, double *c, rocblas_int ldc) {
    if (M <= 1024 && N <= 1024 && K <= 4096)
        mh_small_gemm(ctx, ta != rocblas_operation_none, tb != rocblas_operation_none, uint32_t(M), uint32_t(N), uint32_t(K), *alpha, a, uint32_t(lda), b, uint32_t(ldb), *beta, c, uint32_t(ldc));
    else
        ROCBLAS_CHECK(rocblas_dgemm(ctx->blas, ta, tb, M, N, K, alpha, a, lda, b, ldb, beta, c, ldc));
}

__global__ void k_identity_defect(const double *__restrict__ g, uint32_t m, unsigned long long *__restrict__ out) {
    const uint32_t i = blockIdx.x * blockDim.x + threadIdx.x;
    double d = 0;
    if (i < m * m) {
        const uint32_t r = i % m, c = i / m;
        if (r >= c) d = fabs(g[i] - (r == c ? 1.0 : 0.0));
    }
    for (int off = 32; off > 0; off >>= 1) d = fmax(d, __shfl_xor(d, off, 64));
    if ((threadIdx.x & 63) == 0 && d > 0) atomicMax(out, (unsigned long long)__double_as_longlong(d));
}

__global__ void k_defect_matrix(const double *__restrict__ g, uint32_t m, double *__restrict__ e) {
    const uint32_t i = blockIdx.x * blockDim.x + threadIdx.x;
    if (i >= m * m) return;
    const uint32_t r = i % m, c = i / m;
    e[i] = (r >= c ? g[i] : g[size_t(r) * m + c]) - (r == c ? 1.0 : 0.0);
}
__global__ void k_inverse_sqrt_series(const double *__restrict__ e, const double *__restrict__ e2, uint32_t m, double *__restrict__ s) {
    const uint32_t i = blockIdx.x * blockDim.x + threadIdx.x;
    if (i >= m * m) return;
    s[i] = (i % m == i / m ? 1.0 : 0.0) - 0.5 * e[i] + 0.375 * e2[i];
}

__global__ void __launch_bounds__(256) k_rr_selfcheck(const double *__restrict__ a, uint32_t m, const double *__restrict__ z, uint32_t ldz, const double *__restrict__ theta, uint32_t ncols,
                                                      unsigned long long *__restrict__ worst) {
    __shared__ double zs[768], red[3][256];
    const uint32_t tid = threadIdx.x, j = blockIdx.x == 0 ? 0 : (blockIdx.x == 1 ? ncols / 2 : ncols - 1);
    for (uint32_t i = tid; i < m; i += 256) zs[i] = z[size_t(j) * ldz + i];
    __syncthreads();
    const double th = theta[j];
    double rmax = 0, azmax = 0, zmax = 0;
    bool nan = false;
    for (uint32_t i = tid; i < m; i += 256) {
        double az = 0, abs_az = 0;
        for (uint32_t c = 0; c < m; ++c) {
            const double t = a[size_t(c) * m + i] * zs[c];
            az += t, abs_az += fabs(t);
        }
        const double r = az - th * zs[i];
        nan = nan || !(r == r);
        rmax = fmax(rmax, fabs(r)), azmax = fmax(azmax, abs_az), zmax = fmax(zmax, fabs(zs[i]));
    }
    red[0][tid] = nan ? INFINITY : rmax, red[1][tid] = azmax, red[2][tid] = zmax;
    __syncthreads();
    for (int h = 128; h > 0; h >>= 1) {
        if (tid < uint32_t(h))
            for (int q = 0; q < 3; ++q) red[q][tid] = fmax(red[q][tid], red[q][tid + h]);
        __syncthreads();
    }
    if (tid == 0) {
        const double rel = red[0][0] / fmax(red[1][0] + fabs(th) * red[2][0], 1e-300);
        atomicMax(worst, (unsigned long long)__double_as_longlong(rel == rel ? rel : INFINITY));
    }
}
void rr_selfcheck(mh_context *ctx, const double *saved, uint32_t m, const double *z, uint32_t ldz, const double *theta, uint32_t ncols) {
    if (!ncols) return;
    if (!ctx->rr_check) {
        ctx->rr_check = static_cast<unsigned long long *>(ctx->pool.alloc(256));
        HIP_CHECK(hipMemsetAsync(ctx->rr_check, 0, 256, ctx->stream));
    }
    k_rr_selfcheck<<<3, 256, 0, ctx->stream>>>(saved, m, z, ldz, theta, ncols, ctx->rr_check);
    KERNEL_CHECK();
}

int host_info(DevArray<int> &info) { int hinfo = 0; info.download(&hinfo, 1); return hinfo; }
bool sytrd_gave_up(mh_context *ctx, int flag, double *gA, const double *saved, uint32_t m) {
    if (!flag && !switches().test_sytrd_giveup) return false;
    ++ctx->sytrd_redos;
    HIP_CHECK(hipMemcpyAsync(gA, saved, size_t(m) * m * sizeof(double), hipMemcpyDeviceToDevice, ctx->stream));
    return true;
}
bool accept_partial(mh_context *ctx, double quality, double *evals, const double *lam, uint32_t nwant) {
    if (!(quality < 1e-10)) return false;
    HIP_CHECK(hipMemcpyAsync(evals, lam, size_t(nwant) * sizeof(double), hipMemcpyDeviceToDevice, ctx->stream));
    return true;
}

int eig_tridiag_small(mh_context *ctx, double *gA, uint32_t m, double *evals, double *ework, DevArray<int> &info, uint32_t nwant, std::vector<double> *host_evals) {
    DevArray<double> z(ctx, size_t(m) * m), tau(ctx, m);
    const bool partial = nwant && nwant < m;
    DevArray<double> zl(ctx, partial ? size_t(m) * nwant : 0);
    double *zres = z.get();
    uint32_t ncols = m;
    HIP_CHECK(hipMemcpyAsync(z.get(), gA, size_t(m) * m * sizeof(double), hipMemcpyDeviceToDevice, ctx->stream));
    for (int attempt = 0; attempt < 2; ++attempt) {
        mh_sytrd_small(ctx, gA, m, evals, ework, tau, attempt == 0 ? -1 : 0);
        int gave_up = 0;
        const bool flagged = attempt == 0 && ctx->sytrd_flag;
        if (flagged) HIP_CHECK(hipMemcpyAsync(&gave_up, ctx->sytrd_flag, sizeof(int), hipMemcpyDeviceToHost, ctx->stream));
        if (partial) {
            DevArray<double> wv(ctx, 2 * m + 8), ufac(ctx, size_t(3) * m * nwant);
            double *zout = attempt == 0 ? zl.get() : z.get();
            if (mh_tridiag_lowest(ctx, evals, ework, m, nwant, wv, zout, m, ufac, wv.get() + m, wv.get() + m + 8)) {
                double qv[5] = {1, 0, 0, 0, 0};
                std::vector<double> lam_host(host_evals ? nwant : 0);
                HIP_CHECK(hipMemcpyAsync(qv, wv.get() + m, sizeof(qv), hipMemcpyDeviceToHost, ctx->stream));
                if (host_evals) HIP_CHECK(hipMemcpyAsync(lam_host.data(), wv.get(), size_t(nwant) * sizeof(double), hipMemcpyDeviceToHost, ctx->stream));
                HIP_CHECK(hipStreamSynchronize(ctx->stream));
                if (flagged && sytrd_gave_up(ctx, gave_up, gA, z, m)) continue;
                if (switches().verbose)
                    fprintf(stderr, "[rr] tridiagonal m %u lowest %u: residual / ||T|| %.2e; us: multisection %.0f, inverse iteration %.0f, Gram-Schmidt %.0f, output %.0f\n", m,
                            nwant, qv[0], qv[1] * 0.01, qv[2] * 0.01, qv[3] * 0.01, qv[4] * 0.01);
                if (ctx->rr_trace) ctx->rr_trace->quality = qv[0];
                if (accept_partial(ctx, qv[0], evals, wv, nwant)) {
                    if (host_evals) host_evals->swap(lam_host);
                    zres = zout, ncols = nwant;
                    break;
                }
            }
        }
        if (flagged) {
            HIP_CHECK(hipStreamSynchronize(ctx->stream));
            if (sytrd_gave_up(ctx, gave_up, gA, z, m)) continue;
        }
        ROCBLAS_CHECK(rocsolver_dstedc(ctx->blas, rocblas_evect_tridiagonal, m, evals, ework, z, m, info));
        if (const int hinfo = host_info(info)) return hinfo;
        break;
    }
    if (ctx->rr_trace) ctx->rr_trace->solver = ncols < m ? MhRrTrace::SMALL_PARTIAL : MhRrTrace::SMALL_STEDC;
    mh_apply_q(ctx, gA, tau, m, zres, m, ncols);
    if (zres == zl.get()) rr_selfcheck(ctx, z.get(), m, zres, m, evals, ncols);
    HIP_CHECK(hipMemcpyAsync(gA, zres, size_t(m) * ncols * sizeof(double), hipMemcpyDeviceToDevice, ctx->stream));
    return 0;
}

std::optional<int> eig_tridiag_wide(mh_context *ctx, double *gA, uint32_t m, double *evals, double *ework, DevArray<int> &info, uint32_t nwant) {
    DevArray<double> z(ctx, size_t(m) * m), saved(ctx, size_t(m) * m), tau(ctx, m);
    HIP_CHECK(hipMemcpyAsync(saved.get(), gA, size_t(m) * m * sizeof(double), hipMemcpyDeviceToDevice, ctx->stream));
    mh_sytrd_wide(ctx, gA, m, evals, ework, tau);
    int gave_up = 0;
    HIP_CHECK(hipMemcpyAsync(&gave_up, ctx->sytrd_flag, sizeof(int), hipMemcpyDeviceToHost, ctx->stream));
    HIP_CHECK(hipStreamSynchronize(ctx->stream));
    if (sytrd_gave_up(ctx, gave_up, gA, saved, m)) return std::nullopt;
    if (nwant && nwant < m && nwant <= 256 && !switches().no_tridiag_wide) {
        DevArray<double> work(ctx, size_t(5) * nwant * m + size_t(2) * nwant * nwant + 8), lam(ctx, nwant);
        double quality = 1.0;
        if (mh_tridiag_lowest_wide(ctx, evals, ework, m, nwant, lam, z, m, work, info, &quality)) {
            if (switches().verbose) fprintf(stderr, "[rr] tridiagonal m %u lowest %u (wide): residual / ||T|| %.2e\n", m, nwant, quality);
            if (ctx->rr_trace) ctx->rr_trace->quality = quality;
            if (accept_partial(ctx, quality, evals, lam, nwant)) {
                if (ctx->rr_trace) ctx->rr_trace->solver = MhRrTrace::WIDE_PARTIAL;
                mh_apply_q(ctx, gA, tau, m, z, m, nwant);
                rr_selfcheck(ctx, saved.get(), m, z, m, evals, nwant);
                HIP_CHECK(hipMemcpyAsync(gA, z.get(), size_t(m) * nwant * sizeof(double), hipMemcpyDeviceToDevice, ctx->stream));
                HIP_CHECK(hipStreamSynchronize(ctx->stream));
                return 0;
            }
        }
    }
    ROCBLAS_CHECK(rocsolver_dstedc(ctx->blas, rocblas_evect_tridiagonal, m, evals, ework, z, m, info));
    if (const int hinfo = host_info(info)) return hinfo;
    ROCBLAS_CHECK(rocsolver_dormtr(ctx->blas, rocblas_side_left, rocblas_fill_lower, rocblas_operation_none, m, m, gA, m, tau, z, m));
    if (ctx->rr_trace) ctx->rr_trace->solver = MhRrTrace::WIDE_STEDC_ORMTR;
    HIP_CHECK(hipMemcpyAsync(gA, z.get(), size_t(m) * m * sizeof(double), hipMemcpyDeviceToDevice, ctx->stream));
    HIP_CHECK(hipStreamSynchronize(ctx->stream));
    return 0;
}

}

int mh_rr_solve(mh_context *ctx, double *gA, double *gM, uint32_t m, double *evals, double *ework, DevArray<int> &info, uint32_t nwant, bool gm_is_identity,
                std::vector<double> *host_evals) {
    const double one = 1, zero = 0;
    k_symmetrize_lower<<<grid1(size_t(m) * m), TB, 0, ctx->stream>>>(gA, m, m);
    KERNEL_CHECK();
    bool identity = gm_is_identity, series = false;
    if (!identity) {
        static_assert(sizeof(unsigned long long) == sizeof(double), "defect word");
        unsigned long long *defect = reinterpret_cast<unsigned long long *>(ework);
        HIP_CHECK(hipMemsetAsync(defect, 0, sizeof(unsigned long long), ctx->stream));
        k_identity_defect<<<grid1(size_t(m) * m), TB, 0, ctx->stream>>>(gM, m, defect);
        KERNEL_CHECK();
        unsigned long long bits = 0;
        HIP_CHECK(hipMemcpyAsync(&bits, defect, sizeof(bits), hipMemcpyDeviceToHost, ctx->stream));
        HIP_CHECK(hipStreamSynchronize(ctx->stream));
        double d;
        memcpy(&d, &bits, sizeof(d));
        identity = d < 1e-11;
        if (switches().verbose) fprintf(stderr, "[rr] m %u identity defect %.2e\n", m, d);
        series = !identity && d < 1e-7;
        if (ctx->rr_trace) ctx->rr_trace->defect = d;
    }
    if (ctx->rr_trace) ctx->rr_trace->reduction = gm_is_identity ? MhRrTrace::GIVEN_IDENTITY : identity ? MhRrTrace::MEASURED_IDENTITY : series ? MhRrTrace::SERIES : MhRrTrace::CHOLESKY;
    DevArray<double> sroot, stmp;
    if (series) {
        sroot.reset(ctx, size_t(m) * m);
        stmp.reset(ctx, size_t(m) * m * 2);
        double *e = stmp.get(), *e2 = stmp.get() + size_t(m) * m;
        k_defect_matrix<<<grid1(size_t(m) * m), TB, 0, ctx->stream>>>(gM, m, e);
        KERNEL_CHECK();
        small_dgemm(ctx, rocblas_operation_none, rocblas_operation_none, m, m, m, &one, e, m, e, m, &zero, e2, m);
        k_inverse_sqrt_series<<<grid1(size_t(m) * m), TB, 0, ctx->stream>>>(e, e2, m, sroot);
        KERNEL_CHECK();
        small_dgemm(ctx, rocblas_operation_none, rocblas_operation_none, m, m, m, &one, sroot, m, gA, m, &zero, e, m);
        small_dgemm(ctx, rocblas_operation_none, rocblas_operation_none, m, m, m, &one, e, m, sroot, m, &zero, gA, m);
        k_symmetrize_lower<<<grid1(size_t(m) * m), TB, 0, ctx->stream>>>(gA, m, m);
        KERNEL_CHECK();
        identity = true;
    }
    if (!identity) {
        mh_potrf(ctx, gM, m, m, info);
        if (const int hinfo = host_info(info)) return hinfo;
        ROCBLAS_CHECK(rocblas_dtrsm(ctx->blas, rocblas_side_left, rocblas_fill_lower, rocblas_operation_none, rocblas_diagonal_non_unit, m, m, &one, gM, m, gA, m));
        ROCBLAS_CHECK(rocblas_dtrsm(ctx->blas, rocblas_side_right, rocblas_fill_lower, rocblas_operation_transpose, rocblas_diagonal_non_unit, m, m, &one, gM, m, gA, m));
    }
    std::optional<int> hinfo;
    if (m >= 8 && m <= 256) hinfo = eig_tridiag_small(ctx, gA, m, evals, ework, info, nwant, host_evals);
    else if (m > 256 && m <= 768 && !ctx->exchange_disabled) hinfo = eig_tridiag_wide(ctx, gA, m, evals, ework, info, nwant);
    if (!hinfo) {
        ROCBLAS_CHECK(rocsolver_dsyevd(ctx->blas, rocblas_evect_original, rocblas_fill_lower, m, gA, m, evals, ework, info));
        hinfo = host_info(info);
        if (ctx->rr_trace) ctx->rr_trace->solver = MhRrTrace::SYEVD;
    }
    if (*hinfo != 0) return *hinfo;
    if (series) {
        small_dgemm(ctx, rocblas_operation_none, rocblas_operation_none, m, m, m, &one, sroot, m, gA, m, &zero, stmp, m);
        HIP_CHECK(hipMemcpyAsync(gA, stmp.get(), size_t(m) * m * sizeof(double), hipMemcpyDeviceToDevice, ctx->stream));
        HIP_CHECK(hipStreamSynchronize(ctx->stream));
    } else if (!identity)
        ROCBLAS_CHECK(rocblas_dtrsm(ctx->blas, rocblas_side_left, rocblas_fill_lower, rocblas_operation_transpose, rocblas_diagonal_non_unit, m, m, &one, gM, m, gA, m));
    return 0;
}

namespace {

void colsumsq(mh_context *ctx, const double *x, size_t rows, uint32_t w, double *out, DevArray<double> &scratch) {
    const uint32_t rpb = 256;
    const uint32_t nb = div_up(rows, rpb);
    if (scratch.count < size_t(nb) * w) scratch.reset(ctx, size_t(nb) * w);
    dim3 grid(nb, div_up(w, 64));
    k_colsumsq_partial<<<grid, 64, 0, ctx->stream>>>(x, rows, w, scratch, rpb);
    KERNEL_CHECK();
    k_colsumsq_final<<<w, 256, 0, ctx->stream>>>(scratch, nb, w, out);
    KERNEL_CHECK();
}

template<typename F> void precondition_in_slabs(mh_context *ctx, size_t n, const double *r, double *z, uint32_t w, F &&one) {
    if (w <= kPrecondColumns) return one(r, z, w);
    const hipStream_t st = ctx->stream;
    const uint32_t slabs = div_up(w, kPrecondColumns), step = (div_up(w, slabs) + 3u) & ~3u;
    if (w > 1024) mh_throw(MH_EINVAL, "a block of %u columns exceeds the 1 024 the column maps cover", w);
    DevArray<double> rs(ctx, n * step), zs(ctx, n * step);
    const uint32_t *iota = mh_identity_map(ctx);
    for (uint32_t c0 = 0; c0 < w; c0 += step) {
        const uint32_t wc = std::min(step, w - c0);
        k_gather_cols<<<grid1(n * wc), TB, 0, st>>>(r, iota + c0, rs.get(), n, w, wc);
        KERNEL_CHECK();
        one(rs, zs, wc);
        k_scatter_cols<<<grid1(n * wc), TB, 0, st>>>(zs.get(), iota + c0, z, n, w, wc);
        KERNEL_CHECK();
    }
    HIP_CHECK(hipStreamSynchronize(st));
}

template<typename T> struct Precond {
    mh_system *sys;
    mh_context *ctx;
    uint32_t wmax;
    int deg2, deg1, gamma;
    double ratio, ratio1;
    DevArray<T> rin, z2, d2, t2, r2, r1, x1, d1, t1, rr1;
    DevArray<double> r0, x0, x0_partial;
    static constexpr uint32_t COARSE_SLICES = 8;
    DevArray<double> t2d, r1d, t1d;
    DevArray<T> patch_y;
    static constexpr bool kDouble = std::is_same<T, double>::value;
    static uint32_t pitch(uint32_t w) { return kDouble ? w : (w + 3u) & ~3u; }
    Precond(mh_system *s, uint32_t w_in) : sys(s), ctx(s->ctx), wmax(w_in) {
        const uint32_t w = pitch(w_in);
        const size_t n2 = size_t(3) * s->n_nodes, n1 = size_t(3) * s->n_points, n0 = size_t(6) * s->n_agg;
        d2.reset(ctx, n2 * w); t2.reset(ctx, n2 * w); r2.reset(ctx, n2 * w); z2.reset(ctx, n2 * w);
        if (!kDouble) {
            rin.reset(ctx, n2 * w);
            t2d.reset(ctx, n2 * w);
            r1d.reset(ctx, n1 * w); t1d.reset(ctx, n1 * w);
        }
        r1.reset(ctx, n1 * w); x1.reset(ctx, n1 * w); d1.reset(ctx, n1 * w); t1.reset(ctx, n1 * w); rr1.reset(ctx, n1 * w);
        r0.reset(ctx, n0 * w);
        x0.reset(ctx, n0 * w);
        x0_partial.reset(ctx, n0 * w * COARSE_SLICES);
        patch_y.reset(ctx, std::max(s->patches2.scratch_rows(), s->patches1.scratch_rows()) * w);
        MhCycleShape shape;
        mh_cycle_shape(s, w_in, &shape);
        deg2 = shape.deg2, deg1 = shape.deg1, gamma = shape.gamma, ratio = shape.ratio, ratio1 = shape.ratio1;
    }
    void spmm(const BsrLevel &lvl, const T *x, T *y, uint32_t w) {
        if constexpr (kDouble) mh_spmm(ctx, lvl, lvl.aval, x, y, nullptr, nullptr, w);
        else mh_spmm_f32(ctx, lvl, x, y, w);
    }
    static const T *dinv_of(const BsrLevel &lvl) {
        if constexpr (kDouble) return lvl.dinv.get();
        else return lvl.dinv32.get();
    }
    const PatchSet &patches_of(const BsrLevel &lvl) const { return lvl.id == 2 ? sys->patches2 : sys->patches1; }
    void cheb(const BsrLevel &lvl, int deg, const T *b, T *x, bool zero_init, T *r, T *d, T *t, uint32_t w, double *z_out = nullptr, uint32_t w_out = 0,
              const double *b_src = nullptr, PanelColumns b_cols = PanelColumns{0, 0, nullptr}, T *b_copy = nullptr) {
        const size_t rows = size_t(3) * lvl.n_nodes;
        const double lmax = lvl.lmax, lmin = lvl.lmax / (lvl.id == 1 && ratio1 > 0 ? ratio1 : ratio);
        const double theta = 0.5 * (lmax + lmin), delta = 0.5 * (lmax - lmin), sig = theta / delta;
        double rho = 1.0 / sig;
        const T *dinv = dinv_of(lvl);
        if (!zero_init) spmm(lvl, x, t, w);
        if constexpr (!kDouble) {
            if (b_src && zero_init) k_cheb_init_convert<<<grid1(rows * w), TB, 0, ctx->stream>>>(b_src, b_cols, dinv, float(1.0 / theta), b_copy, r, d, x, rows, w);
            else k_cheb_init_v4<<<grid1(rows * (w / 4)), TB, 0, ctx->stream>>>(reinterpret_cast<const f4_t *>(b), zero_init ? nullptr : reinterpret_cast<const f4_t *>(t), dinv,
                                                                               float(1.0 / theta), reinterpret_cast<f4_t *>(r), reinterpret_cast<f4_t *>(d),
                                                                               reinterpret_cast<f4_t *>(x), zero_init ? 0 : 1, rows, w / 4);
        } else {
            k_cheb_init<T><<<grid1(rows * w), TB, 0, ctx->stream>>>(b, zero_init ? nullptr : t, dinv, T(1.0 / theta), r, d, x, zero_init ? 0 : 1, rows, w);
        }
        KERNEL_CHECK();
        const PatchSet &ps = patches_of(lvl);
        mh_apply_patches<T>(ctx, ps, r, nullptr, w, T(1.0 / theta), d, x, nullptr, 0, patch_y.get());
        constexpr bool fuse_steps = true;
        T *cur = d, *alt = t;
        for (int k = 1; k < deg; ++k) {
            const double rho_new = 1.0 / (2 * sig - rho);
            const bool last = z_out && k + 1 == deg;
            bool fused = false;
            if constexpr (!kDouble) {
                if (fuse_steps && !last) fused = mh_spmm_f32_cheb_step(ctx, lvl, cur, alt, r, x, dinv, float(rho_new * rho), float(2 * rho_new / delta), w);
            }
            if (fused) {
                std::swap(cur, alt);
                mh_apply_patches<T>(ctx, ps, r, nullptr, w, T(2 * rho_new / delta), cur, x, nullptr, 0, patch_y.get());
            } else {
                spmm(lvl, cur, alt, w);
                if (!last) {
                    k_cheb_step<T><<<grid1(rows * w), TB, 0, ctx->stream>>>(alt, dinv, T(rho_new * rho), T(2 * rho_new / delta), r, cur, x, rows, w);
                } else if constexpr (kDouble) {
                    k_cheb_last<T><<<grid1(rows * w), TB, 0, ctx->stream>>>(alt, dinv, T(rho_new * rho), T(2 * rho_new / delta), r, cur, x, z_out, rows, w, w_out);
                } else {
                    k_cheb_last_v4<<<grid1(rows * (w / 4)), TB, 0, ctx->stream>>>(reinterpret_cast<const f4_t *>(alt), dinv, float(rho_new * rho), float(2 * rho_new / delta),
                                                                             reinterpret_cast<const f4_t *>(r), reinterpret_cast<const f4_t *>(cur),
                                                                             reinterpret_cast<const f4_t *>(x), z_out, rows, w / 4, w_out);
                }
                KERNEL_CHECK();
                if (!last) mh_apply_patches<T>(ctx, ps, r, nullptr, w, T(2 * rho_new / delta), cur, x, nullptr, 0, patch_y.get());
                else mh_apply_patches<T>(ctx, ps, r, alt, w, T(2 * rho_new / delta), nullptr, nullptr, z_out, w_out, patch_y.get());
            }
            rho = rho_new;
        }
        if (z_out && deg == 1) {
            k_convert_pitch<T, double><<<grid1(rows * w_out), TB, 0, ctx->stream>>>(x, w, z_out, w_out, rows);
            KERNEL_CHECK();
        }
    }
    void apply(const double *r_in, double *z_out, uint32_t w_in, uint32_t r_pitch = 0, const uint32_t *r_map = nullptr) {
        mh_finish_hierarchy(sys);
        if (kDouble && (r_map || (r_pitch && r_pitch != w_in))) mh_throw(MH_EINVAL, "the double-precision cycle takes a compact right-hand side");
        const PanelColumns r_cols{r_pitch ? r_pitch : w_in, w_in, r_map};
        const uint32_t w = pitch(w_in);
        const uint32_t nn = sys->n_nodes, np = sys->n_points, na = sys->n_agg;
        const size_t n2 = size_t(3) * nn, n1 = size_t(3) * np, n0 = size_t(6) * na;
        const T *r;
        if constexpr (kDouble) r = r_in;
        else r = rin.get();
        T *z = z2.get();
        if constexpr (kDouble) cheb(sys->L2, deg2, r, z, true, r2, d2, t2, w);
        else cheb(sys->L2, deg2, r, z, true, r2, d2, t2, w, nullptr, 0, r_in, r_cols, rin.get());
        if constexpr (kDouble) {
            spmm(sys->L2, z, t2, w);
            k_restrict_p1<double><<<grid1(n1 * w), TB, 0, ctx->stream>>>(r, t2.get(), sys->p1_corner, sys->p1_edge_ptr, sys->p1_edge_mid, r1.get(), np, w);
            KERNEL_CHECK();
        } else {
            mh_spmm_mixed(ctx, sys->L2, z, t2d, w);
            k_restrict_p1<double><<<grid1(n1 * w), TB, 0, ctx->stream>>>(r_in, t2d.get(), sys->p1_corner, sys->p1_edge_ptr, sys->p1_edge_mid, r1d.get(), np, w, r_cols);
            KERNEL_CHECK();
            k_convert<double, T><<<grid1(n1 * w), TB, 0, ctx->stream>>>(r1d.get(), r1.get(), n1 * w);
            KERNEL_CHECK();
        }
        for (int g = 0; g < gamma; ++g) {
            cheb(sys->L1, deg1, r1, x1, g == 0, rr1, d1, t1, w);
            if constexpr (kDouble) {
                spmm(sys->L1, x1, t1, w);
                k_restrict_agg<double><<<grid1(n0 * w), TB, 0, ctx->stream>>>(r1.get(), t1.get(), sys->agg_t, r0, sys->agg_ptr, sys->agg_nodes, na, w);
            } else {
                mh_spmm_mixed(ctx, sys->L1, x1, t1d, w);
                k_restrict_agg<double><<<grid1(n0 * w), TB, 0, ctx->stream>>>(r1d.get(), t1d.get(), sys->agg_t, r0, sys->agg_ptr, sys->agg_nodes, na, w);
            }
            KERNEL_CHECK();
            mh_short_product(ctx, n0, sys->a0, uint32_t(n0), r0, w, x0, x0_partial, COARSE_SLICES);
            k_prolong_agg<T><<<grid1(n1 * w), TB, 0, ctx->stream>>>(x0, sys->agg_t, x1.get(), sys->agg_of, np, w);
            KERNEL_CHECK();
            cheb(sys->L1, deg1, r1, x1, false, rr1, d1, t1, w);
        }
        if constexpr (kDouble) k_prolong_p1<T><<<grid1(n2 * w), TB, 0, ctx->stream>>>(x1.get(), sys->parent_a, sys->parent_b, z, nn, w);
        else k_prolong_p1_v4<<<grid1(n2 * (w / 4)), TB, 0, ctx->stream>>>(reinterpret_cast<const f4_t *>(x1.get()), sys->parent_a, sys->parent_b, reinterpret_cast<f4_t *>(z), nn, w / 4);
        KERNEL_CHECK();
        cheb(sys->L2, deg2, r, z, false, r2, d2, t2, w, z_out, w_in);
    }
};

double estimate_lmax(mh_context *ctx, BsrLevel &lvl, const PatchSet &ps) {
    const uint32_t w = 8;
    const size_t rows = size_t(3) * lvl.n_nodes;
    DevArray<double> v(ctx, rows * w), t(ctx, rows * w), nrm(ctx, w), scratch, py(ctx, ps.scratch_rows() * w);
    k_random_panel<<<grid1(rows * w), TB, 0, ctx->stream>>>(v, rows, w, 0, 0x5eedull);
    KERNEL_CHECK();
    colsumsq(ctx, v, rows, w, nrm, scratch);
    k_scale_cols_inv_sqrt<<<grid1(rows * w), TB, 0, ctx->stream>>>(v, nrm, rows, w);
    KERNEL_CHECK();
    constexpr int power_its = kPowerIterations;
    for (int it = 0; it < power_its; ++it) {
        mh_spmm(ctx, lvl, lvl.aval, v, t, nullptr, nullptr, w);
        k_dinv_mul<<<grid1(rows * w), TB, 0, ctx->stream>>>(t, lvl.dinv, v, rows, w);
        KERNEL_CHECK();
        mh_apply_patches<double>(ctx, ps, t, nullptr, w, 1.0, v, nullptr, nullptr, 0, py.get());
        const bool last = it + 1 == power_its, rescale = !last && (it % 4 == 3 || it + 2 == power_its);
        if (last || rescale) colsumsq(ctx, v, rows, w, nrm, scratch);
        if (rescale) {
            k_scale_cols_inv_sqrt<<<grid1(rows * w), TB, 0, ctx->stream>>>(v, nrm, rows, w);
            KERNEL_CHECK();
        }
    }
    auto h = nrm.to_host();
    double m = 0;
    for (double s : h) m = std::max(m, std::sqrt(s));
    return 1.1 * m * (switches().lmax_low ? 0.88 : 1.0);
}
}

void mh_cycle_shape(const mh_system *s, uint32_t w_in, MhCycleShape *shape) {
    MhCycleShape sh;
    const Switches &sw = switches();
    const bool surface_dominated = s->kept_tets < 4.5 * s->n_points;
    if (s->patches2.any()) {
        sh.deg2 = 5;
        sh.ratio = 60.0;
        const bool few_patches = uint64_t(s->patches2.n_bad_elements) * 500 < s->kept_tets;
        if (w_in > 128 || few_patches) sh.deg1 = 28, sh.gamma = 1, sh.ratio1 = 800.0;
    } else if (surface_dominated) {
        sh.deg2 = 5;
        sh.ratio = 60.0;
        sh.deg1 = 16, sh.gamma = 1, sh.ratio1 = 250.0;
    } else {
        sh.deg1 = 12, sh.gamma = 1, sh.ratio1 = 100.0;
    }
    if (sw.deg2 > 0) sh.deg2 = sw.deg2;
    if (sw.deg1 > 0) sh.deg1 = sw.deg1;
    if (sw.gamma > 0) sh.gamma = sw.gamma;
    if (sw.cheb_ratio > 0) sh.ratio = std::max(1.5, sw.cheb_ratio), sh.ratio1 = 0.0;
    if (sw.cheb_ratio1 > 0) sh.ratio1 = std::max(1.5, sw.cheb_ratio1);
    *shape = sh;
}

double mh_coarse_lift(const mh_system *sys) { return std::max(sys->coarse_lift, sys->worst_quality < kFlatShape ? 1e-8 : 1e-12); }

void mh_finish_hierarchy(mh_system *sys) {
    if (!sys->coarse_pending) return;
    mh_context *ctx = sys->ctx;
    sys->coarse_pending = false;
    HIP_CHECK(hipStreamWaitEvent(ctx->stream, sys->coarse_done, 0));
    int hinfo = 0;
    sys->coarse_info.download(&hinfo, 1);
    for (auto &ws : sys->coarse_ws) ws.reset(ctx, 0);
    for (PatchSet *ps : {&sys->patches2, &sys->patches1}) {
        if (!ps->any() || !ps->dropped.count) continue;
        int dropped[2] = {0, 0};
        ps->dropped.download(dropped, 2);
        sys->dropped_patches[ps->npe == 10 ? 0 : 1] = uint32_t(dropped[0]);
        if (dropped[0] && switches().verbose)
            fprintf(stderr, "[lobpcg] %d of %u + %u sliver patches / clusters of the %s level dropped (e.g. patch %d; clusters count from 1000000): their nodes keep the diagonal scaling only\n", dropped[0], ps->n_patches, ps->n_clusters,
                    ps->npe == 10 ? "P2" : "P1", dropped[1] - 1);
    }
    if (switches().test_coarse_pivot && sys->coarse_lift == 0) hinfo = 1;
    if (hinfo != 0) {
        sys->hierarchy_ready = false;
        mh_throw(MH_EFACTOR, "coarse operator not positive definite (pivot %d of a diagonal block): shift must be negative", hinfo);
    }
}

void mh_build_hierarchy(mh_system *sys, double sigma, bool defer) {
    mh_context *ctx = sys->ctx;
    if (sys->hierarchy_ready && sys->sigma_built == sigma) {
        if (!defer) mh_finish_hierarchy(sys);
        return;
    }
    mh_finish_hierarchy(sys);
    hipStream_t main_stream = ctx->stream;
    for (BsrLevel *lvl : {&sys->L2, &sys->L1}) {
        lvl->aval.reset(ctx, lvl->n_blocks * 9);
        lvl->dinv.reset(ctx, size_t(3) * lvl->n_nodes);
        lvl->aval32.reset(ctx, lvl->n_blocks * 9);
        k_shift_values<<<grid1(lvl->n_blocks * 9), TB, 0, ctx->stream>>>(lvl->kval, lvl->mval, lvl->n_blocks, sigma, lvl->aval, switches().copy_passes ? nullptr : lvl->aval32.get());
        KERNEL_CHECK();
        k_diag_inverse<<<grid1(lvl->n_nodes), TB, 0, ctx->stream>>>(lvl->row_ptr, lvl->col, lvl->aval, lvl->n_nodes, lvl->dinv);
        KERNEL_CHECK();
        mh_build_patch_inverses(ctx, *lvl, lvl->id == 2 ? sys->patches2 : sys->patches1);
    }
    const size_t n0 = size_t(6) * sys->n_agg;
    sys->a0.reset(ctx, n0 * n0);
    sys->a0.zero();
    k_coarse_matrix<<<sys->n_agg, 64, 0, ctx->stream>>>(sys->L1.row_ptr, sys->L1.col, sys->L1.aval, sys->agg_t, sys->agg_of, sys->agg_ptr, sys->agg_nodes, sys->n_agg, sys->a0);
    KERNEL_CHECK();
    k_fix_coarse_diag<<<grid1(n0), TB, 0, ctx->stream>>>(sys->a0, uint32_t(n0), mh_coarse_lift(sys));
    KERNEL_CHECK();
    DevArray<int> &info = sys->coarse_info;
    info.reset(ctx, 1);
    auto smoother_setup = [&] {
        for (BsrLevel *lvl : {&sys->L2, &sys->L1}) {
            lvl->lmax = estimate_lmax(ctx, *lvl, lvl->id == 2 ? sys->patches2 : sys->patches1);
            if (sys->lmax_widened) lvl->lmax *= 1.25;
            lvl->dinv32.reset(ctx, size_t(3) * lvl->n_nodes);
            if (switches().copy_passes) {
                k_convert<double, float><<<grid1(lvl->n_blocks * 9), TB, 0, ctx->stream>>>(lvl->aval.get(), lvl->aval32.get(), lvl->n_blocks * 9);
                KERNEL_CHECK();
            }
            k_convert<double, float><<<grid1(size_t(3) * lvl->n_nodes), TB, 0, ctx->stream>>>(lvl->dinv.get(), lvl->dinv32.get(), size_t(3) * lvl->n_nodes);
            KERNEL_CHECK();
        }
    };
    {
        const uint32_t nb = 128;
        DevArray<double> &cblk = sys->coarse_ws[0], &rblk = sys->coarse_ws[1], &pnext = sys->coarse_ws[4];
        DevArray<double> *pinv2[2] = {&sys->coarse_ws[2], &sys->coarse_ws[3]};
        cblk.reset(ctx, n0 * nb);
        rblk.reset(ctx, n0 * nb);
        pinv2[0]->reset(ctx, size_t(nb) * nb);
        pinv2[1]->reset(ctx, size_t(nb) * nb);
        pnext.reset(ctx, size_t(nb) * nb);
        info.zero();
        const bool side = ctx->aux_stream_ready();
        struct StreamGuard {
            mh_context *c;
            hipStream_t s;
            bool swapped{false};
            ~StreamGuard() {
                if (c->stream != s) {
                    c->stream = s;
                    if (swapped) std::swap(c->blas, c->blas_aux);
                    (void)hipStreamSynchronize(c->aux_stream);
                    if (c->aux2_stream) (void)hipStreamSynchronize(c->aux2_stream);
                }
            }
        } guard{ctx, main_stream};
        hipEvent_t forked = nullptr;
        if (side) {
            HIP_CHECK(hipEventCreateWithFlags(&forked, hipEventDisableTiming));
            HIP_CHECK(hipEventRecord(forked, main_stream));
            HIP_CHECK(hipStreamWaitEvent(ctx->aux_stream, forked, 0));
            ctx->stream = ctx->aux_stream;
            std::swap(ctx->blas, ctx->blas_aux);
            guard.swapped = true;
        }
        const size_t steps_total = div_up(n0, size_t(nb));
        const bool ahead = side && ctx->aux2_stream_ready(2 * steps_total);
        hipEvent_t *ev_piv = ctx->ahead_ev.data(), *ev_inv = ctx->ahead_ev.data() + steps_total;
        const double one = 1, zero = 0, mone = -1;
        const rocblas_int ld = rocblas_int(n0);
        double *a = sys->a0.get();
        uint32_t step = 0;
        for (size_t k0 = 0; k0 < n0; k0 += nb, ++step) {
            const rocblas_int w = rocblas_int(std::min<size_t>(nb, n0 - k0));
            double *pinv = pinv2[step & 1]->get();
            if (step == 0 || !ahead) mh_spd_inverse_small(ctx, a + k0 * n0 + k0, uint32_t(n0), uint32_t(w), pinv, uint32_t(w), info);
            else HIP_CHECK(hipStreamWaitEvent(ctx->stream, ev_inv[step], 0));
            HIP_CHECK(hipMemcpyAsync(cblk, a + k0 * n0, n0 * size_t(w) * sizeof(double), hipMemcpyDeviceToDevice, ctx->stream));
            ROCBLAS_CHECK(rocblas_dgemm(ctx->blas, rocblas_operation_none, rocblas_operation_none, w, ld, w, &one, pinv, w, a + k0, ld, &zero, rblk, w));
            const size_t k1 = k0 + nb;
            if (ahead && k1 < n0) {
                const uint32_t wn = uint32_t(std::min<size_t>(nb, n0 - k1));
                HIP_CHECK(hipMemcpy2DAsync(pnext.get(), size_t(wn) * sizeof(double), a + k1 * n0 + k1, n0 * sizeof(double), size_t(wn) * sizeof(double), wn, hipMemcpyDeviceToDevice, ctx->stream));
                mh_small_gemm(ctx, false, false, wn, wn, uint32_t(w), -1.0, cblk.get() + k1, uint32_t(n0), rblk.get() + k1 * size_t(w), uint32_t(w), 1.0, pnext.get(), wn);
                HIP_CHECK(hipEventRecord(ev_piv[step], ctx->stream));
                HIP_CHECK(hipStreamWaitEvent(ctx->aux2_stream, ev_piv[step], 0));
                hipStream_t elimination = ctx->stream;
                ctx->stream = ctx->aux2_stream;
                try {
                    mh_spd_inverse_small(ctx, pnext.get(), wn, wn, pinv2[(step + 1) & 1]->get(), wn, info);
                } catch (...) {
                    ctx->stream = elimination;
                    throw;
                }
                ctx->stream = elimination;
                HIP_CHECK(hipEventRecord(ev_inv[step + 1], ctx->aux2_stream));
            }
            ROCBLAS_CHECK(rocblas_dgemm(ctx->blas, rocblas_operation_none, rocblas_operation_none, ld, ld, w, &mone, cblk, ld, rblk, w, &one, a, ld));
            HIP_CHECK(hipMemcpy2DAsync(a + k0, n0 * sizeof(double), rblk.get(), size_t(w) * sizeof(double), size_t(w) * sizeof(double), n0, hipMemcpyDeviceToDevice, ctx->stream));
            ROCBLAS_CHECK(rocblas_dgemm(ctx->blas, rocblas_operation_none, rocblas_operation_none, ld, w, w, &mone, cblk, ld, pinv, w, &zero, a + k0 * n0, ld));
            HIP_CHECK(hipMemcpy2DAsync(a + k0 * n0 + k0, n0 * sizeof(double), pinv, size_t(w) * sizeof(double), size_t(w) * sizeof(double), size_t(w), hipMemcpyDeviceToDevice, ctx->stream));
        }
        k_symmetrize_lower<<<grid1(n0 * n0), TB, 0, ctx->stream>>>(sys->a0, uint32_t(n0), uint32_t(n0));
        KERNEL_CHECK();
        if (side) {
            ctx->stream = main_stream;
            std::swap(ctx->blas, ctx->blas_aux);
        }
        if (!sys->coarse_done) HIP_CHECK(hipEventCreateWithFlags(&sys->coarse_done, hipEventDisableTiming));
        HIP_CHECK(hipEventRecord(sys->coarse_done, side ? ctx->aux_stream : main_stream));
        sys->coarse_pending = true;
        smoother_setup();
        if (side) (void)hipEventDestroy(forked);
    }
    sys->sigma_built = sigma;
    sys->hierarchy_ready = true;
    if (!defer) {
        mh_finish_hierarchy(sys);
        HIP_CHECK(hipStreamSynchronize(ctx->stream));
    }
}

namespace {
__global__ void k_last_columns_to_panel(const double *__restrict__ z, size_t n, uint32_t ncols, const double *__restrict__ scale, double *__restrict__ x) {
    const size_t i = size_t(blockIdx.x) * blockDim.x + threadIdx.x;
    if (i >= n * ncols) return;
    const uint32_t j = uint32_t(i % ncols);
    x[i] = scale[j] * z[(n - 1 - j) * n + i / ncols];
}

void dense_eigs(mh_system *sys, uint32_t nev, double sigma, double *eigenvalues, bool inverse = false) {
    mh_context *ctx = sys->ctx;
    const size_t n = size_t(3) * sys->n_nodes;
    auto &lvl = sys->L2;
    DevArray<double> a(ctx, n * n), m(ctx, n * n), d(ctx, n), e(ctx, n);
    DevArray<int> info(ctx, 1);
    a.zero();
    m.zero();
    lvl.aval.reset(ctx, lvl.n_blocks * 9);
    k_shift_values<<<grid1(lvl.n_blocks * 9), TB, 0, ctx->stream>>>(lvl.kval, lvl.mval, lvl.n_blocks, sigma, lvl.aval, nullptr);
    KERNEL_CHECK();
    k_bsr_to_dense<<<grid1(lvl.n_nodes), TB, 0, ctx->stream>>>(lvl.row_ptr, lvl.col, lvl.aval, lvl.mval, lvl.n_nodes, a, m);
    KERNEL_CHECK();
    HIP_CHECK(hipStreamSynchronize(ctx->stream));
    ExclusivePhase alone_on_the_device(ctx->device);
    double *lhs = inverse ? m.get() : a.get(), *rhs = inverse ? a.get() : m.get();
    ROCBLAS_CHECK(rocsolver_dsygvd(ctx->blas, rocblas_eform_ax, rocblas_evect_original, rocblas_fill_lower, rocblas_int(n), lhs, rocblas_int(n), rhs, rocblas_int(n), d, e, info));
    int hinfo = 0;
    info.download(&hinfo, 1);
    if (hinfo != 0) mh_throw(hinfo > int(n) ? MH_EFACTOR : MH_ENOTCONVERGED, "dense sygvd failed (info %d)", hinfo);
    std::vector<double> th(n);
    d.download(th.data(), n);
    sys->evecs.reset(ctx, n * nev);
    sys->evec_cols = nev;
    if (!inverse) {
        for (uint32_t i = 0; i < nev; ++i) eigenvalues[i] = th[i] + sigma;
        k_colmajor_to_panel<<<grid1(n * nev), TB, 0, ctx->stream>>>(lhs, n, nev, sys->evecs);
    } else {
        std::vector<double> scale(nev);
        for (uint32_t i = 0; i < nev; ++i) {
            const double nu = th[n - 1 - i];
            if (!(nu > 0)) mh_throw(MH_ENOTCONVERGED, "dense inverse eigensolve: non-positive eigenvalue %g at position %u", nu, i);
            eigenvalues[i] = 1.0 / nu + sigma;
            scale[i] = 1.0 / std::sqrt(nu);
        }
        DevArray<double> dscale(ctx, nev);
        dscale.upload(scale.data(), nev);
        k_last_columns_to_panel<<<grid1(n * nev), TB, 0, ctx->stream>>>(lhs, n, nev, dscale, sys->evecs);
    }
    KERNEL_CHECK();
    HIP_CHECK(hipStreamSynchronize(ctx->stream));
}
}

namespace {
__global__ void k_axpy_panel(double *__restrict__ y, const double *__restrict__ b, size_t count) {
    const size_t i = size_t(blockIdx.x) * blockDim.x + threadIdx.x;
    if (i < count) y[i] = b[i] - y[i];
}
__global__ void k_coldot_partial(const double *__restrict__ x, const double *__restrict__ y, size_t rows, uint32_t w, double *__restrict__ partial, uint32_t rows_per_block) {
    const uint32_t c = blockIdx.y * blockDim.x + threadIdx.x;
    if (c >= w) return;
    const size_t r0 = size_t(blockIdx.x) * rows_per_block, r1 = min(rows, r0 + rows_per_block);
    double s = 0;
    for (size_t r = r0; r < r1; ++r) s += x[r * w + c] * y[r * w + c];
    partial[size_t(blockIdx.x) * w + c] = s;
}
__global__ void k_cg_advance(double *__restrict__ x, double *__restrict__ r, const double *__restrict__ p, const double *__restrict__ ap, const double *__restrict__ rz, const double *__restrict__ pap,
                             size_t count, uint32_t w) {
    const size_t i = size_t(blockIdx.x) * blockDim.x + threadIdx.x;
    if (i >= count) return;
    const uint32_t c = uint32_t(i % w);
    const double alpha = pap[c] > 0 ? rz[c] / pap[c] : 0.0;
    x[i] += alpha * p[i];
    r[i] -= alpha * ap[i];
}
__global__ void k_cg_direction(double *__restrict__ p, const double *__restrict__ z, const double *__restrict__ rz_new, const double *__restrict__ rz_old, size_t count, uint32_t w) {
    const size_t i = size_t(blockIdx.x) * blockDim.x + threadIdx.x;
    if (i >= count) return;
    const uint32_t c = uint32_t(i % w);
    const double beta = rz_old[c] > 0 ? rz_new[c] / rz_old[c] : 0.0;
    p[i] = z[i] + beta * p[i];
}
}

namespace {
struct PanelCg {
    mh_system *sys;
    mh_context *ctx;
    size_t n;
    uint32_t wmax;
    DevArray<double> rr, zz, p, ap, rz, rz_new, pap, scratch;
    static constexpr uint32_t rpb = 256;
    PanelCg(mh_system *s, uint32_t w) : sys(s), ctx(s->ctx), n(size_t(3) * s->n_nodes), wmax(w), rr(s->ctx, n * w), zz(s->ctx, n * w), p(s->ctx, n * w), ap(s->ctx, n * w), rz(s->ctx, w), rz_new(s->ctx, w),
                                        pap(s->ctx, w), scratch(s->ctx, size_t(div_up(n, rpb)) * w) {}
    void dot(const double *u, const double *v, double *out, uint32_t w) {
        const uint32_t nb = uint32_t(div_up(n, rpb));
        k_coldot_partial<<<dim3(nb, div_up(w, 64)), 64, 0, ctx->stream>>>(u, v, n, w, scratch, rpb);
        KERNEL_CHECK();
        k_colsumsq_final<<<w, 256, 0, ctx->stream>>>(scratch, nb, w, out);
        KERNEL_CHECK();
    }
    template<typename Prec> void solve(Prec &prec, const double *r, double *z, uint32_t w, int iters) {
        hipStream_t st = ctx->stream;
        HIP_CHECK(hipMemsetAsync(z, 0, n * w * sizeof(double), st));
        HIP_CHECK(hipMemcpyAsync(rr.get(), r, n * w * sizeof(double), hipMemcpyDeviceToDevice, st));
        prec.apply(rr, zz, w);
        HIP_CHECK(hipMemcpyAsync(p.get(), zz.get(), n * w * sizeof(double), hipMemcpyDeviceToDevice, st));
        dot(rr, zz, rz, w);
        for (int k = 0; k < iters; ++k) {
            mh_spmm(ctx, sys->L2, sys->L2.aval, p, ap, nullptr, nullptr, w);
            dot(p, ap, pap, w);
            k_cg_advance<<<grid1(n * w), TB, 0, st>>>(z, rr, p, ap, rz, pap, n * w, w);
            KERNEL_CHECK();
            if (k + 1 == iters) break;
            prec.apply(rr, zz, w);
            dot(rr, zz, rz_new, w);
            k_cg_direction<<<grid1(n * w), TB, 0, st>>>(p, zz, rz_new, rz, n * w, w);
            KERNEL_CHECK();
            HIP_CHECK(hipMemcpyAsync(rz.get(), rz_new.get(), w * sizeof(double), hipMemcpyDeviceToDevice, st));
        }
    }
};
}

namespace {
struct BlockLobpcg {
    mh_system *sys;
    mh_context *ctx;
    hipStream_t st;
    const size_t n;
    const uint32_t nev, b, mmax;
    const double sigma, residual_tol;
    const uint32_t max_iters;
    const float *seed_basis;
    const uint32_t seed_rows, seed_cols;
    const volatile unsigned char *cancel;
    volatile float *progress;
    mh_profile &prof;
    mh_profile *profile;
    SharedPhase iterating;
    Timer t_iter;
    double precond_seconds = 0;
    double best_worst_active = 1e300;
    int floor_strikes = 0;
    std::vector<double> hist_active;
    uint32_t pairs_at_floor = 0;
    DevArray<double> X, AX, MX, Xn, AXn, MXn, W, AW, MW, P, MP, Pn, MPn, R, Rw;
    DevArray<double> gA, gM, gM0, gA0, App, evals, ework, Cp, T1, H, H2, G, dscale, Linv, theta_d, rn_d, mn_d, scratch, Ct, norms_d, theta_act_d, Hp, Up, Vp, T1p;
    DevArray<double> Linv_p, T1p2;
    DevArray<uint32_t> idx_d, pos_d;
    DevArray<double> Rr, res_partial, res_blocks, res_norms_d;
    std::vector<double> rr_evals;
    std::vector<uint32_t> res_act, res_pos;
    std::vector<double> res_norms;
    uint32_t res_pitch = 0;
    bool res_ready = false, rw_from_rr = false;
    DevArray<int> info;
    int inner_cg = 0;
    std::unique_ptr<Precond<float>> prec32;
    std::unique_ptr<Precond<double>> prec64;
    std::unique_ptr<PanelCg> panel_cg;
    const bool verbose = switches().verbose, fp32_prec = switches().fp32_prec;
    const bool pproj_ok;
    const bool scaled_norms;
    bool warm = false;
    bool w_implicit = false;
    int last_spread = 1 << 20;
    bool p_needs_explicit = false;
    uint32_t wp = 0;
    uint32_t iters = 0, nconv = 0, redos_at_start = 0;
    bool poly_allowed = true;
    std::vector<double> theta, rn, mn, xn, norms, theta_act, hist_worst;
    double anorm = 0;
    std::vector<uint32_t> act, order, hist_nconv;
    std::vector<uint8_t> locked;
    bool converged = false;
    bool gm_identity = false;
    bool p_implicit = false;
    bool lazy_images = false;
    uint32_t w = 0, wa = 0, m = 0, wp_new = 0;

    BlockLobpcg(mh_system *system, uint32_t nev_, uint32_t block, double sigma_, double residual_tol_, uint32_t max_iters_, const float *seed_basis_, uint32_t seed_rows_,
                uint32_t seed_cols_, const volatile unsigned char *cancel_, volatile float *progress_, mh_profile &prof_, mh_profile *profile_, int inner_cg_ = 0)
        : sys(system), ctx(system->ctx), st(system->ctx->stream), n(size_t(3) * system->n_nodes), nev(nev_), b(block), mmax(3 * block), sigma(sigma_), residual_tol(residual_tol_),
          max_iters(max_iters_), seed_basis(seed_basis_), seed_rows(seed_rows_), seed_cols(seed_cols_), cancel(cancel_), progress(progress_), prof(prof_), profile(profile_),
          iterating(system->ctx->device, true), t_iter(system->ctx), pproj_ok(block <= 128), scaled_norms(system->patches2.any()), theta(block), rn(block), mn(block), xn(block), norms(3 * size_t(block)),
          theta_act(block), order(block), locked(block, 0) {
        inner_cg = inner_cg_;
        for (DevArray<double> *panel : {&X, &AX, &MX, &Xn, &AXn, &MXn, &W, &AW, &MW, &P, &Pn, &R, &Rw}) panel->reset(ctx, n * b);
        if (!pproj_ok)
            for (DevArray<double> *panel : {&MP, &MPn}) panel->reset(ctx, n * b);
        for (DevArray<double> *small : {&gA, &gM, &gM0, &gA0}) small->reset(ctx, size_t(mmax) * mmax);
        for (DevArray<double> *small : {&App, &H, &H2, &Linv, &Hp, &Up, &Vp, &T1p}) small->reset(ctx, size_t(b) * b);
        Linv_p.reset(ctx, size_t(b) * b);
        T1p2.reset(ctx, size_t(mmax) * b);
        for (DevArray<double> *small : {&Cp, &T1}) small->reset(ctx, size_t(mmax) * b);
        for (DevArray<double> *small : {&evals, &ework}) small->reset(ctx, mmax);
        for (DevArray<double> *small : {&dscale, &theta_d, &rn_d, &mn_d, &theta_act_d}) small->reset(ctx, b);
        G.reset(ctx, size_t(b) * 2 * b);
        Ct.reset(ctx, size_t(mmax) * 2 * b);
        norms_d.reset(ctx, 3 * size_t(b));
        idx_d.reset(ctx, b);
        pos_d.reset(ctx, b);
        if (b <= 128) {
            const uint32_t pmax = (b + 1u) & ~1u;
            Rr.reset(ctx, n * pmax);
            res_partial.reset(ctx, size_t(2) * sys->n_nodes * pmax);
            res_blocks.reset(ctx, size_t(div_up(sys->n_nodes, 48)) * 2 * pmax);
            res_norms_d.reset(ctx, size_t(2) * pmax);
            res_norms.resize(size_t(2) * pmax);
        }
        info.reset(ctx, 2);
        if (fp32_prec && !(sys->worst_quality < kFlatShape) && !inner_cg) prec32 = std::make_unique<Precond<float>>(sys, std::min(b, kPrecondColumns));
        else prec64 = std::make_unique<Precond<double>>(sys, std::min(b, kPrecondColumns));
        if (inner_cg) panel_cg = std::make_unique<PanelCg>(sys, std::min(b, kPrecondColumns));
        auto hd = sys->L2.dinv.to_host();
        double dmin = 1e300;
        for (double v : hd) dmin = std::min(dmin, v);
        anorm = sys->L2.lmax / dmin;
    }


    bool chol_orthonormalise(double *V, double *MV, double *AV, uint32_t w, bool transform_images = true, bool allow_implicit = false,
                             const double *hp = nullptr, uint32_t hp_rows = 0) {
        gram(ctx, n, V, w, MV, w, G, w);
        if (hp) {
            const double minus = -1, plus = 1;
            small_dgemm(ctx, rocblas_operation_transpose, rocblas_operation_none, rocblas_int(w), rocblas_int(w), rocblas_int(hp_rows), &minus, hp,
                                        rocblas_int(hp_rows), hp, rocblas_int(hp_rows), &plus, G, rocblas_int(w));
        }
        k_scale_gram<<<grid1(size_t(w) * w), TB, 0, st>>>(G, w, w, dscale);
        KERNEL_CHECK();
        double *Gs = G.get() + size_t(w) * w;
        int hinfo = 0;
        bool fused_inverse = false;
        {
            last_spread = 1 << 20;
            if (w <= 128) {
                fused_inverse = !switches().potrf_chain;
                if (fused_inverse) mh_potrf_small_inverse(ctx, Gs, w, info, dscale, Linv);
                else mh_potrf_small(ctx, Gs, w, info);
                int both[2] = {0, 0};
                info.download(both, 2);
                hinfo = both[0];
                last_spread = both[1];
            } else {
                mh_potrf(ctx, Gs, w, w, info);
                info.download(&hinfo, 1);
            }
        }
        p_needs_explicit = false;
        if (hp && (hinfo != 0 || last_spread >= 16 * 8)) {
            p_needs_explicit = true;
            return true;
        }
        if (hinfo != 0) return false;
        if (!fused_inverse) {
            k_unscale_chol<<<grid1(size_t(w) * w), TB, 0, st>>>(Gs, w, w, dscale);
            KERNEL_CHECK();
        }
        if (w > 256) {
            panel_trsm(ctx, n, V, w, Gs, w);
            if (MV && transform_images) panel_trsm(ctx, n, MV, w, Gs, w);
            if (AV && transform_images) panel_trsm(ctx, n, AV, w, Gs, w);
        } else {
            if (!fused_inverse) {
                HIP_CHECK(hipMemsetAsync(Linv, 0, size_t(w) * w * sizeof(double), st));
                ROCBLAS_CHECK(rocblas_dtrtri(ctx->blas, rocblas_fill_lower, rocblas_diagonal_non_unit, w, Gs, w, Linv, w));
            }
            w_implicit = allow_implicit && !transform_images && last_spread < 16 * 8;
            if (!w_implicit) mh_combine(ctx, n, V, w, nullptr, 0, nullptr, 0, Linv, w, V, w, nullptr);
            if (MV && transform_images) mh_combine(ctx, n, MV, w, nullptr, 0, nullptr, 0, Linv, w, MV, w, nullptr);
            if (AV && transform_images) mh_combine(ctx, n, AV, w, nullptr, 0, nullptr, 0, Linv, w, AV, w, nullptr);
        }
        return true;
    }

    void precondition(const double *r, double *z, uint32_t w, uint32_t r_pitch = 0, const uint32_t *r_map = nullptr) {
        if ((r_pitch || r_map) && !precondition_reads_columns(w)) mh_throw(MH_EINVAL, "this preconditioner path takes a compact right-hand side");
        precondition_in_slabs(ctx, n, r, z, w, [&](const double *rp, double *zp, uint32_t wc) {
            if (panel_cg) panel_cg->solve(*prec64, rp, zp, wc, inner_cg);
            else if (prec32) prec32->apply(rp, zp, wc, r_pitch, r_map);
            else prec64->apply(rp, zp, wc);
        });
    }
    bool precondition_reads_columns(uint32_t w) const { return prec32 && !panel_cg && w <= kPrecondColumns && !switches().copy_passes; }

    void start() {
        redos_at_start = ctx->sytrd_redos;
        if (ctx->rr_check) HIP_CHECK(hipMemsetAsync(ctx->rr_check, 0, sizeof(unsigned long long), st));
        const bool fill_late = !switches().copy_passes;
        if (!fill_late) {
            k_random_panel<<<grid1(n * b), TB, 0, st>>>(X, n, b, 0, 20260710ull);
            KERNEL_CHECK();
        }
        warm = seed_basis && seed_rows == n && seed_cols >= nev;
        if (warm && fill_late) {
            k_random_panel<<<grid1(n * b), TB, 0, st>>>(X, n, b, 0, 20260710ull);
            KERNEL_CHECK();
        }
        if (warm) {
            const uint32_t ncols = std::min(seed_cols, b);
            DevArray<float> seed(ctx, n * ncols);
            seed.upload(seed_basis, n * ncols);
            k_load_seed<<<grid1(n * ncols), TB, 0, st>>>(seed, sys->perm, sys->n_nodes, ncols, b, X);
            KERNEL_CHECK();
            HIP_CHECK(hipStreamSynchronize(st));
        }
        const uint32_t n_rigid = 6 * sys->n_components;
        const bool seed_rigid = b >= n_rigid + 6;
        if (!seed_rigid && sys->n_components > 1)
            mh_throw(MH_EINVAL, "the mesh consists of %u disconnected bodies (%u zero modes): more than a block of %u columns can seed", sys->n_components, n_rigid, b);
        const auto inject_rigid_modes = [&] {
            k_inject_rbm<<<grid1(sys->n_nodes), TB, 0, st>>>(sys->node_xyz, sys->node_component, sys->component_centroid, sys->n_components, sys->n_nodes, X, b, 0);
            KERNEL_CHECK();
        };
        bool with_poly = !warm && seed_rigid && !switches().no_poly_start && sys->n_components == 1 && poly_allowed;
        if (with_poly) {
            double box[6], longest = 0, shortest = 1e300;
            memcpy(box, sys->structure->node_box, sizeof(box));
            if (switches().fresh_structure) {
                DevArray<unsigned long long> keys(ctx, 6);
                const unsigned long long init[6] = {~0ull, ~0ull, ~0ull, 0, 0, 0};
                keys.upload(init, 6);
                k_bbox<<<grid1(sys->n_nodes), TB, 0, st>>>(sys->node_xyz, sys->n_nodes, keys);
                KERNEL_CHECK();
                unsigned long long hk[6];
                keys.download(hk, 6);
                for (int a = 0; a < 6; ++a) {
                    const unsigned long long u = (hk[a] >> 63) ? (hk[a] & 0x7fffffffffffffffull) : ~hk[a];
                    memcpy(&box[a], &u, sizeof(double));
                }
                if (memcmp(box, sys->structure->node_box, sizeof(box)) != 0) mh_throw(MH_EINVAL, "the structure's bounding box differs from the device's");
            }
            for (int a = 0; a < 3; ++a) longest = std::max(longest, box[3 + a] - box[a]), shortest = std::min(shortest, box[3 + a] - box[a]);
            with_poly = shortest >= 0.25 * longest;
            if (with_poly) {
                const uint32_t room = b - n_rigid, want = room - room / 4;
                std::vector<uint32_t> triples;
                for (uint32_t deg = 2; deg <= 6 && 6 + 3 * (triples.size() + (deg + 1) * (deg + 2) / 2) <= want; ++deg)
                    for (uint32_t a = deg + 1; a-- > 0;)
                        for (uint32_t bb = deg - a + 1; bb-- > 0;) triples.push_back(a | bb << 8 | (deg - a - bb) << 16);
                DevArray<double> box_d(ctx, 6);
                DevArray<uint32_t> tri_d(ctx, std::max<size_t>(1, triples.size()));
                box_d.upload(box, 6);
                if (!triples.empty()) tri_d.upload(triples.data(), triples.size());
                const uint32_t first_random = n_rigid + 6 + 3 * uint32_t(triples.size());
                if (fill_late && first_random < b) {
                    k_random_panel<<<grid1(n * (b - first_random)), TB, 0, st>>>(X, n, b, first_random, 20260710ull);
                    KERNEL_CHECK();
                }
                k_inject_poly<<<grid1(sys->n_nodes), TB, 0, st>>>(sys->node_xyz, box_d, sys->n_nodes, tri_d, uint32_t(triples.size()), X, b, n_rigid);
                KERNEL_CHECK();
                HIP_CHECK(hipStreamSynchronize(st));
            }
        }
        if (fill_late && !warm && !with_poly) {
            k_random_panel<<<grid1(n * b), TB, 0, st>>>(X, n, b, 0, 20260710ull);
            KERNEL_CHECK();
        }
        if (seed_rigid) inject_rigid_modes();
        if (!warm) {
            {
                mh_spmm(ctx, sys->L2, nullptr, X, nullptr, sys->L2.mval, MX, b);
                Timer tp(ctx);
                precondition(MX, Xn, b);
                precond_seconds += tp.stop();
                prof.op_applications += b;
                if (switches().copy_passes) HIP_CHECK(hipMemcpyAsync(X, Xn.get(), n * b * sizeof(double), hipMemcpyDeviceToDevice, st));
                else std::swap(X, Xn);
            }
            if (seed_rigid) inject_rigid_modes();
        }
        mh_spmm(ctx, sys->L2, nullptr, X, nullptr, sys->L2.mval, MX, b);
        if (!chol_orthonormalise(X, MX, nullptr, b, switches().copy_passes)) {
            if (with_poly) {
                if (verbose) fprintf(stderr, "[lobpcg] polynomial start block rank deficient: random block instead\n");
                poly_allowed = false;
                start();
                return;
            }
            mh_throw(MH_ENOTCONVERGED, "initial block is rank deficient");
        }
        mh_spmm(ctx, sys->L2, sys->L2.aval, X, AX, sys->L2.mval, MX, b);
        {
            gram(ctx, n, X, b, AX, b, gA, b);
            gram(ctx, n, X, b, MX, b, gM, b);
            const int hinfo = mh_rr_solve(ctx, gA, gM, b, evals, ework, info);
            if (hinfo != 0) mh_throw(MH_ENOTCONVERGED, "initial Rayleigh-Ritz failed (info %d)", hinfo);
            panel_mul(ctx, n, X, b, gA, b, Xn, b, 1.0, 0.0);
            panel_mul(ctx, n, AX, b, gA, b, AXn, b, 1.0, 0.0);
            panel_mul(ctx, n, MX, b, gA, b, MXn, b, 1.0, 0.0);
            std::swap(X, Xn); std::swap(AX, AXn); std::swap(MX, MXn);
            evals.download(theta.data(), b);
        }
    }

    bool converged_or_locked(uint32_t it) {
        if (cancel && *cancel) mh_throw(MH_ECANCELLED, "cancelled");
        if (g_concurrent) {
            iterating.release();
            iterating.acquire();
        }
        bool fused = res_ready;
        if (fused)
            for (const uint32_t i : res_act) fused = fused && !(std::abs(theta[i]) < 10.0 * std::abs(sigma));
        res_ready = false;
        rw_from_rr = fused;
        if (fused) {
            res_norms_d.download(res_norms.data(), size_t(2) * res_pitch);
            for (size_t k = 0; k < res_act.size(); ++k) {
                rn[res_act[k]] = res_norms[k];
                mn[res_act[k]] = res_norms[res_pitch + k];
            }
        } else {
        theta_d.upload(theta.data(), b);
        {
            const uint32_t rpb = 256, nblk = div_up(n, rpb);
            if (scratch.count < size_t(nblk) * 3 * b) scratch.reset(ctx, size_t(nblk) * 3 * b);
            dim3 grid(nblk, div_up(b, 64));
            k_residual_norms<<<grid, 64, 0, st>>>(AX, MX, X, theta_d, 10.0 * std::abs(sigma), R, n, b, rpb, scratch, scaled_norms ? sys->L2.dinv.get() : nullptr);
            KERNEL_CHECK();
            k_colsumsq_final<<<3 * b, 256, 0, st>>>(scratch, nblk, 3 * b, norms_d);
            KERNEL_CHECK();
            norms_d.download(norms.data(), 3 * size_t(b));
            std::copy(norms.begin(), norms.begin() + b, rn.begin());
            std::copy(norms.begin() + b, norms.begin() + 2 * b, mn.begin());
            std::copy(norms.begin() + 2 * b, norms.end(), xn.begin());
        }
        }
        act.clear();
        for (uint32_t i = 0; i < b; ++i) {
            const double rel = std::sqrt(rn[i]) / (std::abs(theta[i]) * std::sqrt(mn[i]));
            const bool near_shift = std::abs(theta[i]) < 10.0 * std::abs(sigma);
            const double floor_norm = scaled_norms ? sys->L2.lmax * std::sqrt(xn[i]) : anorm * std::sqrt(xn[i]);
            const double floor_factor = it == 0 && !warm && sys->worst_quality < kFlatShape ? 65536.0 : 256.0;
            const bool ok = rel < residual_tol || (near_shift && std::sqrt(rn[i]) < floor_factor * 2.2e-16 * floor_norm);
            if (ok) locked[i] = 1;
            if (!locked[i]) act.push_back(i);
        }
        std::iota(order.begin(), order.end(), 0u);
        std::stable_sort(order.begin(), order.end(), [&](uint32_t a, uint32_t c) { return theta[a] < theta[c]; });
        nconv = 0;
        for (uint32_t k = 0; k < nev; ++k) nconv += locked[order[k]];
        if (progress) *progress = 0.3f + 0.65f * float(nconv) / float(nev);
        if (verbose) {
            double worst = 0;
            for (uint32_t k = 0; k < nev; ++k) { const uint32_t i = order[k]; worst = std::max(worst, std::sqrt(rn[i]) / (std::abs(theta[i]) * std::sqrt(mn[i]))); }
            if (it == 0) fprintf(stderr, "[lobpcg] ||A|| <= %.3e, sliver patches %u + %u clusters (largest %u nodes; worst element shape %.2e), aggregates %u, lmax %.4f / %.4f\n", anorm, sys->patches2.n_patches, sys->patches2.n_clusters, sys->patches2.largest_cluster, double(sys->worst_quality), sys->n_agg, sys->L2.lmax, sys->L1.lmax);
            fprintf(stderr, "[lobpcg] it %3u conv %3u/%u active %zu wp %u worst %.2e  floor-ratio[0..7]:", it, nconv, nev, act.size(), wp, worst);
            for (uint32_t i = 0; i < std::min(8u, b); ++i) fprintf(stderr, " %.1f", xn[i] > 0 ? std::sqrt(rn[i]) / (2.2e-16 * (scaled_norms ? sys->L2.lmax : anorm) * std::sqrt(xn[i])) : 0.0);
            fprintf(stderr, "  theta0 %.6e\n", theta[0]);
        }
        iters = it;
        if (nconv >= nev || act.empty()) { converged = nconv >= nev; return true; }
        if (it == max_iters) return true;
        {
            double worst = 0;
            for (uint32_t k = 0; k < nev; ++k) { const uint32_t i = order[k]; worst = std::max(worst, std::sqrt(rn[i]) / (std::abs(theta[i]) * std::sqrt(mn[i]))); }
            hist_worst.push_back(worst);
            hist_nconv.push_back(nconv);
            const size_t h = hist_worst.size();
            if (prec32 && it >= 10 && h > 6 && hist_nconv[h - 7] == nconv && worst > 0.5 * hist_worst[h - 7]) {
                if (verbose) fprintf(stderr, "[lobpcg] it %3u stagnation: switching the preconditioner to double precision\n", it);
                prec32.reset();
                prec64 = std::make_unique<Precond<double>>(sys, std::min(b, kPrecondColumns));
            }
            double worst_active = 0;
            for (uint32_t k = 0; k < nev; ++k) {
                const uint32_t i = order[k];
                if (!locked[i]) worst_active = std::max(worst_active, std::sqrt(rn[i]) / (std::abs(theta[i]) * std::sqrt(mn[i])));
            }
            best_worst_active = std::min(best_worst_active, worst_active);
            hist_active.push_back(worst_active);
            if (inner_cg > 0 && it >= 40) {
                const size_t h = hist_active.size();
                if (h > 30 && hist_nconv[h - 31] == nconv && worst_active > 0.9 * hist_active[h - 31] && worst_active <= 10.0 * residual_tol) {
                    pairs_at_floor = nev > nconv ? nev - nconv : 0;
                    if (verbose) fprintf(stderr, "[lobpcg] it %3u: %u pairs have sat at a residual of %.2e (tolerance %.1e) for thirty iterations -- the rounding floor of this mesh; handed on as they are\n", it, pairs_at_floor, worst_active, residual_tol);
                    converged = true;
                    return true;
                }
            }
            floor_strikes = it >= 20 && worst_active > 1e3 * best_worst_active ? floor_strikes + 1 : 0;
            if (floor_strikes >= 3)
                mh_throw(MH_ENOTCONVERGED, "LOBPCG: %u of %u pairs converged; the others sit at the rounding floor (residual %.1e and growing, best %.1e, tolerance %.1e)", nconv, nev,
                         worst_active, best_worst_active, residual_tol);
        }
        return false;
    }

    void search_directions(uint32_t it) {
        w = uint32_t(act.size());
        idx_d.upload(act.data(), w);
        const double *residuals = Rw.get();
        const bool in_place = precondition_reads_columns(w);
        uint32_t r_pitch = 0;
        const uint32_t *r_map = nullptr;
        if (rw_from_rr) {
            if (act == res_act && res_pitch == w) {
                residuals = Rr.get();
            } else {
                std::vector<uint32_t> &pos = res_pos;
                pos.assign(w, 0);
                size_t q = 0;
                for (uint32_t k = 0; k < w; ++k) {
                    while (q < res_act.size() && res_act[q] != act[k]) ++q;
                    if (q == res_act.size()) mh_throw(MH_EHIP, "active column %u was not active before", act[k]);
                    pos[k] = uint32_t(q);
                }
                pos_d.upload(pos.data(), w);
                if (in_place) {
                    residuals = Rr.get(), r_pitch = res_pitch, r_map = pos_d;
                } else {
                    k_gather_cols<<<grid1(n * w), TB, 0, st>>>(Rr, pos_d, Rw, n, res_pitch, w);
                    KERNEL_CHECK();
                }
            }
        } else if (in_place) {
            residuals = R.get(), r_pitch = b, r_map = idx_d;
        } else {
            k_gather_cols<<<grid1(n * w), TB, 0, st>>>(R, idx_d, Rw, n, b, w);
            KERNEL_CHECK();
        }
        for (uint32_t k = 0; k < w; ++k) theta_act[k] = theta[act[k]];
        theta_act_d.upload(theta_act.data(), w);
        {
            Timer tp(ctx);
            precondition(residuals, W, w, r_pitch, r_map);
            precond_seconds += tp.stop();
            prof.op_applications += w;
        }
        bool ok = true;
        p_implicit = false;
        if (pproj_ok && wp) {
            gram(ctx, n, MX, b, W, w, H, b);
            mh_pack_stacked(ctx, H, b, nullptr, 0, w, -1.0, Ct);
            mh_combine(ctx, n, X, b, nullptr, 0, nullptr, 0, Ct, w, W, w, nullptr, true);
            mh_spmm(ctx, sys->L2, sys->L2.aval, W, AW, sys->L2.mval, MW, w);
            gram(ctx, n, P, wp, MW, w, Hp, wp);
            lazy_images = true;
            w_implicit = false;
            ok = chol_orthonormalise(W, MW, AW, w, false, true, Hp, wp);
            if (!ok) mh_throw(MH_ENOTCONVERGED, "search directions lost rank at iteration %u", it);
            if (p_needs_explicit) {
                mh_pack_stacked(ctx, Hp, wp, nullptr, 0, w, -1.0, Ct);
                mh_combine(ctx, n, P, wp, nullptr, 0, nullptr, 0, Ct, w, W, w, nullptr, true);
                mh_spmm(ctx, sys->L2, sys->L2.aval, W, AW, sys->L2.mval, MW, w);
                lazy_images = w <= 256;
                ok = chol_orthonormalise(W, MW, AW, w, !lazy_images, lazy_images);
                if (!ok) mh_throw(MH_ENOTCONVERGED, "search directions lost rank at iteration %u", it);
            } else {
                p_implicit = true;
            }
        } else {
            gram(ctx, n, MX, b, W, w, H, b);
            if (wp) gram(ctx, n, MP, wp, W, w, H2, wp);
            mh_pack_stacked(ctx, H, b, H2, wp, w, -1.0, Ct);
            mh_combine(ctx, n, X, b, P, wp, nullptr, 0, Ct, w, W, w, nullptr, true);
            mh_spmm(ctx, sys->L2, sys->L2.aval, W, AW, sys->L2.mval, MW, w);
            lazy_images = w <= 256;
            w_implicit = false;
            ok = chol_orthonormalise(W, MW, AW, w, !lazy_images, lazy_images);
            if (!ok) mh_throw(MH_ENOTCONVERGED, "search directions lost rank at iteration %u", it);
        }
    }

    void rayleigh_ritz(uint32_t it) {
        wa = w;
        m = wa + w + wp;
        for (int attempt = 0; attempt < 2; ++attempt) {
            HIP_CHECK(hipMemsetAsync(gA, 0, size_t(m) * m * sizeof(double), st));
            HIP_CHECK(hipMemsetAsync(gM, 0, size_t(m) * m * sizeof(double), st));
            k_set_identity_blocks<<<grid1(wa), TB, 0, st>>>(gA, gM, theta_act_d, wa, m);
            KERNEL_CHECK();
            const double unit_one = 1;
            auto left_corrected = [&](double *block, uint32_t cols) {
                if (w_implicit)
                    ROCBLAS_CHECK(rocblas_dtrmm(ctx->blas, rocblas_side_left, rocblas_fill_lower, rocblas_operation_none, rocblas_diagonal_non_unit, rocblas_int(w),
                                                rocblas_int(cols), &unit_one, Linv, rocblas_int(w), block, rocblas_int(m), block, rocblas_int(m)));
            };
            mh_gram(ctx, n, W, w, AX, wa, gA.get() + wa, m, b, idx_d);
            left_corrected(gA.get() + wa, wa);
            const double unit = 1;
            auto untransformed = [&](double *block, uint32_t rows) {
                if (lazy_images)
                    ROCBLAS_CHECK(rocblas_dtrmm(ctx->blas, rocblas_side_right, rocblas_fill_lower, rocblas_operation_transpose, rocblas_diagonal_non_unit, rocblas_int(rows),
                                                rocblas_int(w), &unit, Linv, rocblas_int(w), block, rocblas_int(m), block, rocblas_int(m)));
            };
            gram(ctx, n, W, w, AW, w, gA.get() + size_t(wa) * m + wa, m);
            if (p_implicit && wp) {
                const double plus = 1, nil = 0;
                double *bw = gA.get() + size_t(wa) * m + wa, *bp = gA.get() + size_t(wa) * m + wa + w;
                gram(ctx, n, P, wp, AW, w, bp, m);
                small_dgemm(ctx, rocblas_operation_transpose, rocblas_operation_none, rocblas_int(w), rocblas_int(w), rocblas_int(wp), &plus, Hp, rocblas_int(wp), bp,
                                            rocblas_int(m), &nil, Up, rocblas_int(w));
                small_dgemm(ctx, rocblas_operation_none, rocblas_operation_none, rocblas_int(wp), rocblas_int(w), rocblas_int(wp), &plus, App, rocblas_int(wp), Hp,
                                            rocblas_int(wp), &nil, T1p, rocblas_int(wp));
                small_dgemm(ctx, rocblas_operation_transpose, rocblas_operation_none, rocblas_int(w), rocblas_int(w), rocblas_int(wp), &plus, Hp, rocblas_int(wp), T1p,
                                            rocblas_int(wp), &nil, Vp, rocblas_int(w));
                k_sub_block<<<grid1(size_t(wp) * w), TB, 0, st>>>(bp, m, T1p, wp, wp, w);
                k_wblock_fix<<<grid1(size_t(w) * w), TB, 0, st>>>(bw, m, Up, Vp, w);
                KERNEL_CHECK();
            }
            untransformed(gA.get() + size_t(wa) * m + wa, w);
            left_corrected(gA.get() + size_t(wa) * m + wa, w);
            const bool w_block_trusted = last_spread < 16 * 8 && !(p_implicit && wp == 0);
            gm_identity = w_block_trusted;
            if (w_block_trusted) {
                k_place_block<<<grid1(size_t(w) * w), TB, 0, st>>>(gM.get() + size_t(wa) * m + wa, m, nullptr, w);
                KERNEL_CHECK();
            } else {
                gram(ctx, n, W, w, MW, w, gM.get() + size_t(wa) * m + wa, m);
                untransformed(gM.get() + size_t(wa) * m + wa, w);
            }
            if (verbose) fprintf(stderr, "[lobpcg] it %3u Cholesky-QR diagonal spread 2^%.1f%s\n", it, last_spread / 16.0, w_block_trusted ? "" : " (W block measured)");
            if (wp) {
                if (!p_implicit) gram(ctx, n, P, wp, AW, w, gA.get() + size_t(wa) * m + wa + w, m);
                untransformed(gA.get() + size_t(wa) * m + wa + w, wp);
                {
                    k_place_block<<<grid1(size_t(wp) * wp), TB, 0, st>>>(gA.get() + size_t(wa + w) * m + wa + w, m, App, wp);
                    k_place_block<<<grid1(size_t(wp) * wp), TB, 0, st>>>(gM.get() + size_t(wa + w) * m + wa + w, m, nullptr, wp);
                    KERNEL_CHECK();
                }
            }
            k_symmetrize_lower<<<grid1(size_t(m) * m), TB, 0, st>>>(gA, m, m);
            KERNEL_CHECK();
            HIP_CHECK(hipMemcpyAsync(gA0, gA, size_t(m) * m * sizeof(double), hipMemcpyDeviceToDevice, st));
            HIP_CHECK(hipMemcpyAsync(gM0, gM, size_t(m) * m * sizeof(double), hipMemcpyDeviceToDevice, st));
            rr_evals.clear();
            const int hinfo = mh_rr_solve(ctx, gA, gM, m, evals, ework, info, wa, gm_identity, &rr_evals);
            if (hinfo == 0) break;
            if (attempt == 1 || wp == 0) mh_throw(MH_ENOTCONVERGED, "Rayleigh-Ritz failed at iteration %u (info %d)", it, hinfo);
            wp = 0;
            m = wa + w;
        }
        if (rr_evals.size() == wa) std::copy(rr_evals.begin(), rr_evals.end(), theta_act.begin());
        else evals.download(theta_act.data(), wa);
        for (uint32_t k = 0; k < wa; ++k) theta[act[k]] = theta_act[k];
    }

    void conjugate_directions(uint32_t it) {
        const double one = 1, zero = 0, mone = -1;
        wp_new = w;
        k_build_cp<<<grid1(size_t(m) * w), TB, 0, st>>>(gA, nullptr, wa, m, w, m, Cp, m);
        KERNEL_CHECK();
        const double *mcp = gm_identity ? Cp.get() : T1.get();
        if (!gm_identity) ROCBLAS_CHECK(rocblas_dsymm(ctx->blas, rocblas_side_left, rocblas_fill_lower, m, w, &one, gM0, m, Cp, m, &zero, T1, m));
        small_dgemm(ctx, rocblas_operation_transpose, rocblas_operation_none, wa, w, m, &one, gA, m, mcp, m, &zero, H, wa);
        small_dgemm(ctx, rocblas_operation_none, rocblas_operation_none, m, w, wa, &mone, gA, m, H, wa, &one, Cp, m);
        if (!gm_identity) ROCBLAS_CHECK(rocblas_dsymm(ctx->blas, rocblas_side_left, rocblas_fill_lower, m, w, &one, gM0, m, Cp, m, &zero, T1, m));
        small_dgemm(ctx, rocblas_operation_transpose, rocblas_operation_none, w, w, m, &one, Cp, m, mcp, m, &zero, G, w);
        k_scale_gram<<<grid1(size_t(w) * w), TB, 0, st>>>(G, w, w, dscale);
        KERNEL_CHECK();
        {
            double *Gs = G.get() + size_t(w) * w;
            int hinfo = 0;
            const bool fused = w <= 128 && !switches().potrf_chain;
            {
                if (fused) mh_potrf_small_inverse(ctx, Gs, w, info, dscale, Linv_p);
                else mh_potrf(ctx, Gs, w, w, info);
                info.download(&hinfo, 1);
            }
            if (hinfo != 0) {
                wp_new = 0;
            } else if (fused) {
                mh_small_gemm(ctx, false, true, m, w, w, 1.0, Cp, m, Linv_p, w, 0.0, T1p2, m);
                HIP_CHECK(hipMemcpyAsync(Cp, T1p2, size_t(m) * w * sizeof(double), hipMemcpyDeviceToDevice, st));
            } else {
                k_unscale_chol<<<grid1(size_t(w) * w), TB, 0, st>>>(Gs, w, w, dscale);
                KERNEL_CHECK();
                ROCBLAS_CHECK(rocblas_dtrsm(ctx->blas, rocblas_side_right, rocblas_fill_lower, rocblas_operation_transpose, rocblas_diagonal_non_unit, m, w, &one, Gs, w, Cp, m));
            }
        }
        if (!warm && it < kSkipP && !hist_worst.empty() && hist_worst.back() > 0.5) wp_new = 0;
        if (wp_new) {
            small_dgemm(ctx, rocblas_operation_none, rocblas_operation_none, m, wp_new, m, &one, gA0, m, Cp, m, &zero, T1, m);
            small_dgemm(ctx, rocblas_operation_transpose, rocblas_operation_none, wp_new, wp_new, m, &one, Cp, m, T1, m, &zero, App, wp_new);
        }
    }

    void update_basis(uint32_t it) {
        mh_pack_coefficients(ctx, gA, wa, Cp, wp_new, m, m, Ct);
        {
            const uint32_t pitch = (wa + 1u) & ~1u;
            if (w_implicit) {
                const double unit = 1;
                double *rows = Ct.get() + size_t(wa) * (wa + wp_new);
                ROCBLAS_CHECK(rocblas_dtrmm(ctx->blas, rocblas_side_right, rocblas_fill_lower, rocblas_operation_none, rocblas_diagonal_non_unit, rocblas_int(wa + wp_new),
                                            rocblas_int(w), &unit, Linv, rocblas_int(w), rows, rocblas_int(wa + wp_new), rows, rocblas_int(wa + wp_new)));
            }
            if (p_implicit && wp) {
                const double minus = -1, plus = 1;
                const rocblas_int pitchc = rocblas_int(wa + wp_new);
                double *rows_w = Ct.get() + size_t(wa) * (wa + wp_new), *rows_p = Ct.get() + size_t(wa + w) * (wa + wp_new);
                ROCBLAS_CHECK(rocblas_dgemm(ctx->blas, rocblas_operation_none, rocblas_operation_transpose, pitchc, rocblas_int(wp), rocblas_int(w), &minus, rows_w, pitchc, Hp,
                                            rocblas_int(wp), &plus, rows_p, pitchc));
            }
            const bool one_launch = b <= 128 && !switches().copy_passes;
            if (one_launch) mh_combine(ctx, n, X, wa, W, w, P, wp, Ct, wa + wp_new, Xn, wa, Pn, false, b, idx_d, pitch, nullptr, 0, 0, X, b, idx_d);
            else mh_combine(ctx, n, X, wa, W, w, P, wp, Ct, wa + wp_new, Xn, wa, Pn, false, b, idx_d, pitch);
            if (wp_new && !pproj_ok) mh_spmm(ctx, sys->L2, nullptr, Pn, nullptr, sys->L2.mval, MPn, wp_new);
            if (!one_launch) {
                if (pitch == wa) k_scatter_cols<<<grid1(n * wa), TB, 0, st>>>(Xn.get(), idx_d, X.get(), n, b, wa);
                else k_scatter_cols_pitch<<<grid1(n * wa), TB, 0, st>>>(Xn.get(), pitch, idx_d, X.get(), n, b, wa);
                KERNEL_CHECK();
            }
            if (Rr.count) {
                mh_spmm_mapped(ctx, sys->L2, sys->L2.aval, Xn, AX, sys->L2.mval, MX, pitch, b, wa, idx_d, evals, Rr, res_partial, scaled_norms ? sys->L2.dinv.get() : nullptr);
                const uint32_t rpb = 48, nblk = div_up(sys->n_nodes, rpb), w2 = 2 * pitch;
                dim3 grid(nblk, div_up(w2, 64));
                k_colsum_partial<<<grid, 64, 0, st>>>(res_partial, sys->n_nodes, w2, res_blocks, rpb);
                KERNEL_CHECK();
                k_colsumsq_final<<<w2, 256, 0, st>>>(res_blocks, nblk, w2, res_norms_d);
                KERNEL_CHECK();
                res_act = act;
                res_pitch = pitch;
                res_ready = true;
            } else {
                mh_spmm_mapped(ctx, sys->L2, sys->L2.aval, Xn, AX, sys->L2.mval, MX, pitch, b, wa, idx_d);
            }
        }
        std::swap(P, Pn); std::swap(MP, MPn);
        wp = wp_new;
    }

    void finish(double *eigenvalues) {
        prof.restarts = iters;
        prof.op_solve = precond_seconds;
        if (!converged) mh_throw(MH_ENOTCONVERGED, "LOBPCG: %u of %u pairs converged in %u iterations", nconv, nev, iters);
        for (uint32_t k = 0; k < nev; ++k) eigenvalues[k] = theta[order[k]] + sigma;
        sys->plain_residual = -1.0;
        if (scaled_norms) {
            theta_d.upload(theta.data(), b);
            const uint32_t rpb = 256, nblk = div_up(n, rpb);
            if (scratch.count < size_t(nblk) * 3 * b) scratch.reset(ctx, size_t(nblk) * 3 * b);
            k_residual_norms<<<dim3(nblk, div_up(b, 64)), 64, 0, st>>>(AX, MX, X, theta_d, 10.0 * std::abs(sigma), R, n, b, rpb, scratch, nullptr);
            KERNEL_CHECK();
            k_colsumsq_final<<<3 * b, 256, 0, st>>>(scratch, nblk, 3 * b, norms_d);
            KERNEL_CHECK();
            norms_d.download(norms.data(), 3 * size_t(b));
            double worst = 0;
            for (uint32_t k = 0; k < nev; ++k) {
                const uint32_t i = order[k];
                if (std::abs(theta[i]) < 10.0 * std::abs(sigma)) continue;
                worst = std::max(worst, std::sqrt(norms[i]) / (std::abs(theta[i]) * std::sqrt(norms[b + i])));
            }
            sys->plain_residual = worst;
            if (verbose) fprintf(stderr, "[lobpcg] accepted in the Jacobi-scaled norm at %.1e; worst elastic pair in the plain 2-norm: %.2e\n", residual_tol, worst);
        }
        sys->evecs.reset(ctx, n * nev);
        sys->evec_cols = nev;
        idx_d.upload(order.data(), nev);
        k_gather_cols<<<grid1(n * nev), TB, 0, st>>>(X, idx_d, sys->evecs, n, b, nev);
        KERNEL_CHECK();
        HIP_CHECK(hipStreamSynchronize(st));
        prof.iterate = t_iter.stop();
        read_health();
        sys->profile = prof;
        if (profile) *profile = prof;
        if (switches().test_selfcheck_fail && !ctx->exchange_disabled) prof.rr_selfcheck = 1.0;
        if (!(prof.rr_selfcheck < 1e-6))
            mh_throw(MH_EHIP, "Rayleigh-Ritz self-check failed: a step's eigenpairs leave a relative residual of %.2e against the step's own matrix", prof.rr_selfcheck);
    }
    void read_health() {
        prof.sytrd_redos = ctx->sytrd_redos - redos_at_start;
        prof.pairs_at_floor = pairs_at_floor;
        prof.rr_selfcheck = 0.0;
        if (ctx->rr_check) {
            unsigned long long bits = 0;
            HIP_CHECK(hipMemcpyAsync(&bits, ctx->rr_check, sizeof(bits), hipMemcpyDeviceToHost, st));
            HIP_CHECK(hipStreamSynchronize(st));
            memcpy(&prof.rr_selfcheck, &bits, sizeof(double));
        }
    }

    void run(double *eigenvalues) {
        start();
        for (uint32_t it = 0; it <= max_iters; ++it) {
            if (converged_or_locked(it)) break;
            search_directions(it);
            rayleigh_ritz(it);
            conjugate_directions(it);
            update_basis(it);
        }
        finish(eigenvalues);
    }
};
struct Attempt {
    mh_system *sys;
    uint32_t nev, b;
    double sigma, residual_tol;
    const float *seed;
    uint32_t srows, scols;
    const volatile unsigned char *cancel;
    volatile float *progress;
    double *eigenvalues;
    mh_profile &prof;
    mh_profile *profile;
    std::optional<MhError> run(uint32_t max_iters, int inner_cg = 0) {
        try {
            BlockLobpcg solver(sys, nev, b, sigma, residual_tol, max_iters, seed, srows, scols, cancel, progress, prof, profile, inner_cg);
            solver.run(eigenvalues);
            return std::nullopt;
        } catch (const MhError &e) {
            return e;
        }
    }
    void reset_profile() {
        prof = sys->profile;
        prof.dofs = uint32_t(size_t(3) * sys->n_nodes);
    }
    void widen_lmax() {
        if (sys->lmax_widened) return;
        sys->L1.lmax *= 1.25;
        sys->L2.lmax *= 1.25;
        sys->lmax_widened = true;
    }
};
}

static void eigs_impl(mh_system *sys, uint32_t nev, double sigma, double residual_tol, uint32_t max_iters, const float *seed_basis, uint32_t seed_rows,
                      uint32_t seed_cols, const volatile unsigned char *cancel, volatile float *progress, double *eigenvalues, mh_profile *profile) {
    mh_context *ctx = sys->ctx;
    HIP_CHECK(hipSetDevice(ctx->device));
    const size_t n = size_t(3) * sys->n_nodes;
    if (nev >= n) mh_throw(MH_EINVAL, "nev %u must be below the %zu unknowns", nev, n);
    if (!(sigma < 0)) mh_throw(MH_EFACTOR, "shift must be negative for a positive-definite shifted operator");
    if (sys->unreferenced_points) mh_throw(MH_EFACTOR, "%u mesh point(s) belong to no tetrahedron: the shifted operator is singular", sys->unreferenced_points);
    mh_profile prof = sys->profile;
    prof.dofs = uint32_t(n);
    prof.stiffness_nonzeros = uint32_t((sys->L2.n_blocks - sys->n_nodes) / 2 * 9 + uint64_t(6) * sys->n_nodes);
    if (cancel && *cancel) mh_throw(MH_ECANCELLED, "cancelled");
    const uint32_t guards = std::max(15u, nev * kGuardPercent / 100);
    const uint32_t b = (nev + guards + 6u * (sys->n_components - 1u) + 15u) / 16u * 16u;
    if (n <= 768 || n < size_t(5) * b) {
        Timer t(ctx);
        dense_eigs(sys, nev, sigma, eigenvalues);
        prof.iterate = t.stop();
        prof.restarts = 1;
        sys->profile = prof;
        if (profile) *profile = prof;
        return;
    }
    const Switches &sw = switches();
    Attempt attempt{sys, nev, b, sigma, residual_tol, seed_basis, seed_rows, seed_cols, cancel, progress, eigenvalues, prof, profile};
    for (int lifted = 0;; ++lifted) {
        try {
            {
                Timer t(ctx);
                mh_build_hierarchy(sys, sigma, true);
                prof.factorize = t.stop();
            }
            if (progress) *progress = 0.3f;
            std::optional<MhError> err;
            if (sw.test_last_resort) err = MhError(MH_ENOTCONVERGED, "MH_TEST=last_resort");
            else err = attempt.run(max_iters);
            if (err && !sw.test_last_resort && attempt.seed && err->code == MH_ENOTCONVERGED && max_iters >= 50) {
                if (sw.verbose) fprintf(stderr, "[lobpcg] %s -- the seeded basis did not serve: once more from a cold start\n", err->what());
                attempt.seed = nullptr, attempt.srows = 0, attempt.scols = 0;
                attempt.reset_profile();
                err = attempt.run(max_iters);
            }
            if (err && err->code == MH_EHIP && strstr(err->what(), "self-check") && !ctx->exchange_disabled) {
                if (sw.verbose) fprintf(stderr, "[lobpcg] %s -- once more without the exchange kernels\n", err->what());
                ctx->exchange_disabled = true;
                attempt.reset_profile();
                err = attempt.run(max_iters);
            }
            if (err && err->code == MH_ENOTCONVERGED && max_iters >= 50 && !sys->lmax_widened && !sw.test_last_resort && !(sys->worst_quality < kFlatShape)) {
                if (sw.verbose) fprintf(stderr, "[lobpcg] %s -- once more with the smoothers' spectral bounds widened by 25 %%\n", err->what());
                attempt.widen_lmax();
                err = attempt.run(max_iters);
            }
            if (err && err->code == MH_ENOTCONVERGED && n > kDenseLastResort && max_iters >= 50) {
                if (sw.verbose) fprintf(stderr, "[lobpcg] %s -- last resort: conjugate-gradient search directions\n", err->what());
                const MhError stopped = *err;
                attempt.reset_profile();
                attempt.widen_lmax();
                err = attempt.run(max_iters, kLastResortCg);
                if (err && err->code == MH_ENOTCONVERGED) {
                    if (sw.verbose) fprintf(stderr, "[lobpcg] the last resort with %d conjugate-gradient steps: %s -- once more with %d\n", kLastResortCg, err->what(), 5 * kLastResortCg);
                    attempt.reset_profile();
                    err = attempt.run(std::min<uint32_t>(max_iters, 120), 5 * kLastResortCg);
                    if (err && err->code == MH_ENOTCONVERGED) mh_throw(MH_ENOTCONVERGED, "%s (the last resort too: %s)", stopped.what(), err->what());
                }
            }
            if (err && err->code == MH_ENOTCONVERGED && n <= kDenseLastResort && max_iters >= 50) {
                if (sw.verbose) fprintf(stderr, "[lobpcg] %s -- dense eigensolve of order %zu instead\n", err->what(), n);
                Timer t(ctx);
                dense_eigs(sys, nev, sigma, eigenvalues, true);
                attempt.reset_profile();
                prof.iterate += t.stop();
                prof.restarts = max_iters + 1;
                sys->profile = prof;
                if (profile) *profile = prof;
                err.reset();
            }
            if (err) throw *err;
            return;
        } catch (const MhError &e) {
            if (e.code != MH_EFACTOR || !strstr(e.what(), "coarse operator") || lifted >= 2) throw;
            sys->coarse_lift = (sys->coarse_lift > 0 ? sys->coarse_lift : 1e-9) * 1e3;
            sys->hierarchy_ready = false;
            if (sw.verbose) fprintf(stderr, "[lobpcg] %s -- the coarse operator's diagonal lifted by %.0e, once more\n", e.what(), sys->coarse_lift);
        }
    }
}


uint32_t mh_shift_invert_panel(mh_system *sys, double sigma, const double *b, double *x, uint32_t w, double rel_tol, uint32_t max_iters, double *worst_rel) {
    mh_context *ctx = sys->ctx;
    hipStream_t st = ctx->stream;
    const size_t n = size_t(3) * sys->n_nodes;
    if (!(sigma < 0)) mh_throw(MH_EFACTOR, "shift-invert: the shift must be negative (K - sigma M positive definite)");
    if (w == 0 || w > 64) mh_throw(MH_EINVAL, "shift-invert panel: %u columns outside 1..64", w);
    std::unique_lock<std::mutex> one_solve_at_a_time(g_solve_mutex, std::defer_lock);
    if (!g_concurrent) one_solve_at_a_time.lock();
    SharedPhase solving(ctx->device);
    mh_build_hierarchy(sys, sigma);
    Precond<double> prec(sys, w);
    DevArray<double> r(ctx, n * w), z(ctx, n * w), p(ctx, n * w), ap(ctx, n * w), rz(ctx, w), rz_new(ctx, w), pap(ctx, w), rn(ctx, w), scratch;
    const uint32_t rpb = 256, nb = uint32_t(div_up(n, rpb));
    scratch.reset(ctx, size_t(nb) * w);
    const dim3 grid(nb, div_up(w, 64));
    auto dot = [&](const double *u, const double *v, double *out) {
        k_coldot_partial<<<grid, 64, 0, st>>>(u, v, n, w, scratch, rpb);
        KERNEL_CHECK();
        k_colsumsq_final<<<w, 256, 0, st>>>(scratch, nb, w, out);
        KERNEL_CHECK();
    };
    HIP_CHECK(hipMemsetAsync(x, 0, n * w * sizeof(double), st));
    std::vector<double> bn(w), rnh(w);
    dot(b, b, rn);
// ... 89 lines not shown
```

Measured before the change: 646.8 eigenpairs/s.

## Assemble Rayleigh-Ritz pencil blocks in two fused MFMA launches

Replaces the chain of memsets, small dgemms, trmm corrections, block placement, symmetrization and device copies that builds the LOBPCG Rayleigh-Ritz pencil with two kernels. The first computes the W/P/X/M block transforms in one workgroup per job using f64 MFMA, and the second places them into gA/gM/gA0/gM0. Grams are first written to compact raw buffers. The saved symmetric copy is passed to the small tridiagonal solver, presumably so it does not have to re-read or symmetrize. It aims to cut per-iteration launch and rocBLAS overhead for block sizes up to 128, at the cost of extra scratch memory and a separate code path, plus a lab harness that checks it against a long-double reference.

```diff
diff --git a/mesheditor_amd/csrc/lab/mh_lab.hip b/mesheditor_amd/csrc/lab/mh_lab.hip
--- a/mesheditor_amd/csrc/lab/mh_lab.hip
+++ b/mesheditor_amd/csrc/lab/mh_lab.hip
@@ -269,14 +269,168 @@
     bad += differing(two.xn, one.xn) + differing(two.x, want) + differing(two.p, one.p);
     return double(bad);
 }
+
+struct LabMat {
+    uint32_t rows{0}, cols{0};
+    std::vector<long double> v, a;
+    uint32_t k{0};
+    LabMat(uint32_t r, uint32_t c) : rows(r), cols(c), v(size_t(r) * c, 0.0L), a(size_t(r) * c, 0.0L) {}
+    LabMat(uint32_t r, uint32_t c, const std::vector<double> &x) : LabMat(r, c) {
+        for (size_t i = 0; i < v.size(); ++i) v[i] = x[i], a[i] = std::abs((long double)x[i]);
+    }
+    long double bound(size_t i) const { const long double ku = k * 0x1p-53L; return ku / (1.0L - ku) * a[i]; }
+};
+LabMat lab_mul(const LabMat &A, bool ta, const LabMat &B, bool tb, bool lower_a = false, bool upper_b = false) {
+    const uint32_t M = ta ? A.cols : A.rows, K = ta ? A.rows : A.cols, N = tb ? B.rows : B.cols;
+    LabMat C(M, N);
+    C.k = A.k + B.k + K;
+    for (uint32_t j = 0; j < N; ++j)
+        for (uint32_t i = 0; i < M; ++i) {
+            long double s = 0, t = 0;
+            for (uint32_t q = 0; q < K; ++q) {
+                if ((lower_a && q > i) || (upper_b && q > j)) continue;
+                const size_t ia = ta ? size_t(i) * A.rows + q : size_t(q) * A.rows + i, ib = tb ? size_t(q) * B.rows + j : size_t(j) * B.rows + q;
+                s += A.v[ia] * B.v[ib], t += A.a[ia] * B.a[ib];
+            }
+            C.v[size_t(j) * M + i] = s, C.a[size_t(j) * M + i] = t;
+        }
+    return C;
+}
+LabMat lab_sub(const LabMat &A, const LabMat &B, bool tb = false) {
+    LabMat C(A.rows, A.cols);
+    C.k = std::max(A.k, B.k) + 1;
+    for (uint32_t j = 0; j < A.cols; ++j)
+        for (uint32_t i = 0; i < A.rows; ++i) {
+            const size_t e = size_t(j) * A.rows + i, f = tb ? size_t(i) * B.rows + j : e;
+            C.v[e] = A.v[e] - B.v[f], C.a[e] = A.a[e] + B.a[f];
+        }
+    return C;
+}
+double lab_pencil_ratio(mh_context *ctx, uint64_t seed, uint32_t w, uint32_t wp, uint32_t flags) {
+    const bool w_implicit = flags & 1u, lazy = flags & 2u, p_implicit = flags & 4u, trusted = flags & 8u;
+    const uint32_t b = std::max(w, wp), m = 2 * w + wp;
+    uint64_t state = seed * 6364136223846793005ull + 1442695040888963407ull;
+    auto unit = [&] {
+        state = state * 6364136223846793005ull + 1442695040888963407ull;
+        return double(state >> 11) * 0x1p-53 - 0.5;
+    };
+    std::vector<double> theta(w), dw(w), dp(wp);
+    for (uint32_t i = 0; i < w; ++i) theta[i] = 1.6e4 * std::pow(1e11 / 1.6e4, w > 1 ? double(i) / (w - 1) : 0.0);
+    for (uint32_t i = 0; i < w; ++i) dw[i] = std::sqrt(10.0 * theta[w - 1 - i]);
+    for (uint32_t i = 0; i < wp; ++i) dp[i] = std::sqrt(3.0 * theta[std::min(i, w - 1)]);
+    std::vector<double> rx(size_t(w) * w), rw(size_t(w) * w), rp(size_t(wp) * w), rm(size_t(w) * w), linv(size_t(w) * w), hp(size_t(wp) * w), app(size_t(wp) * wp);
+    for (uint32_t j = 0; j < w; ++j)
+        for (uint32_t i = 0; i < w; ++i) {
+            rx[size_t(j) * w + i] = 1e-3 * dw[i] * std::sqrt(theta[j]) * unit();
+            if (i >= j) {
+                rw[size_t(j) * w + i] = rw[size_t(i) * w + j] = dw[i] * dw[j] * (unit() + (i == j ? 1.0 : 0.0));
+                rm[size_t(j) * w + i] = rm[size_t(i) * w + j] = (i == j ? dw[i] * dw[i] * 1e-9 : dw[i] * dw[j] * 1e-10 * unit());
+            }
+            linv[size_t(j) * w + i] = i == j ? std::exp2(8.0 * (w > 1 ? double(i) / (w - 1) : 0.0)) / dw[i] * 3e4 : i > j ? 0.1 * unit() / dw[j] * 3e4 : 1e30;
+        }
+    for (uint32_t j = 0; j < w; ++j)
+        for (uint32_t i = 0; i < wp; ++i) rp[size_t(j) * wp + i] = 0.1 * dp[i] * dw[j] * unit(), hp[size_t(j) * wp + i] = 2e-3 * unit();
+    for (uint32_t j = 0; j < wp; ++j)
+        for (uint32_t i = j; i < wp; ++i) app[size_t(j) * wp + i] = app[size_t(i) * wp + j] = dp[i] * dp[j] * (unit() + (i == j ? 1.0 : 0.0));
+    const LabMat RX(w, w, rx), RW(w, w, rw), RP(wp, w, rp), RM(w, w, rm), L(w, w, linv), HP(wp, w, hp), APP(wp, wp, app);
+    LabMat Bx = RX, Bw = RW, Bp = RP, Mw = RM;
+    if (p_implicit && wp) {
+        const LabMat T = lab_mul(APP, false, HP, false), U = lab_mul(HP, true, RP, false), V = lab_mul(HP, true, T, false);
+        Bp = lab_sub(RP, T);
+        Bw = lab_sub(lab_sub(V, U), U, true);
+        LabMat S(w, w);
+        S.k = std::max(Bw.k, RW.k) + 1;
+        for (size_t e = 0; e < S.v.size(); ++e) S.v[e] = RW.v[e] + Bw.v[e], S.a[e] = RW.a[e] + Bw.a[e];
+        Bw = S;
+    }
+    if (lazy) Bw = lab_mul(Bw, false, L, true, false, true), Mw = lab_mul(Mw, false, L, true, false, true);
+    if (lazy && wp) Bp = lab_mul(Bp, false, L, true, false, true);
+    if (w_implicit) Bw = lab_mul(L, false, Bw, false, true), Bx = lab_mul(L, false, Bx, false, true);
+    std::vector<long double> ref_a(size_t(m) * m, 0.0L), ref_m(size_t(m) * m, 0.0L), bnd_a(size_t(m) * m, 0.0L), bnd_m(size_t(m) * m, 0.0L);
+    for (uint32_t cc = 0; cc < m; ++cc)
+        for (uint32_t rr = 0; rr < m; ++rr) {
+            const uint32_t r = std::max(rr, cc), c = std::min(rr, cc);
+            const size_t e = size_t(cc) * m + rr;
+            ref_m[e] = r == c ? 1.0L : 0.0L;
+            if (r < w) ref_a[e] = r == c ? (long double)theta[r] : 0.0L;
+            else if (r < 2 * w && c < w) ref_a[e] = Bx.v[size_t(c) * w + (r - w)], bnd_a[e] = Bx.bound(size_t(c) * w + (r - w));
+            else if (r < 2 * w) {
+                const size_t f = size_t(c - w) * w + (r - w);
+                ref_a[e] = Bw.v[f], bnd_a[e] = Bw.bound(f);
+                if (!trusted) ref_m[e] = Mw.v[f], bnd_m[e] = Mw.bound(f);
+            } else if (c >= 2 * w) ref_a[e] = app[size_t(c - 2 * w) * wp + (r - 2 * w)];
+            else if (c >= w) ref_a[e] = Bp.v[size_t(c - w) * wp + (r - 2 * w)], bnd_a[e] = Bp.bound(size_t(c - w) * wp + (r - 2 * w));
+        }
+    const size_t slot = size_t(b) * b, mm = size_t(m) * m;
+    DevArray<double> dtheta(ctx, w), dl(ctx, size_t(w) * w), dhp(ctx, std::max<size_t>(1, size_t(wp) * w)), dapp(ctx, std::max<size_t>(1, size_t(wp) * wp)), draw(ctx, 4 * slot),
+        work(ctx, 8 * slot), out(ctx, 12 * mm);
+    dtheta.upload(theta.data(), w), dl.upload(linv.data(), linv.size());
+    if (wp) dhp.upload(hp.data(), hp.size()), dapp.upload(app.data(), app.size());
+    draw.zero();
+    HIP_CHECK(hipMemcpyAsync(draw.get(), rx.data(), rx.size() * sizeof(double), hipMemcpyHostToDevice, ctx->stream));
+    HIP_CHECK(hipMemcpyAsync(draw.get() + slot, rw.data(), rw.size() * sizeof(double), hipMemcpyHostToDevice, ctx->stream));
+    if (wp) HIP_CHECK(hipMemcpyAsync(draw.get() + 2 * slot, rp.data(), rp.size() * sizeof(double), hipMemcpyHostToDevice, ctx->stream));
+    HIP_CHECK(hipMemcpyAsync(draw.get() + 3 * slot, rm.data(), rm.size() * sizeof(double), hipMemcpyHostToDevice, ctx->stream));
+    MhPencil p;
+    p.w = w, p.wp = wp, p.b = b, p.w_implicit = w_implicit, p.lazy_images = lazy, p.p_implicit = p_implicit, p.w_block_trusted = trusted;
+    p.theta = dtheta, p.linv = dl, p.hp = dhp, p.app = dapp, p.work = work;
+    p.raw_x = draw.get(), p.raw_w = draw.get() + slot, p.raw_p = draw.get() + 2 * slot, p.raw_m = draw.get() + 3 * slot;
+    std::vector<double> got[3];
+    for (int run = 0; run < 3; ++run) {
+        double *o = out.get() + size_t(run) * 4 * mm;
+        p.gA = o, p.gM = o + mm, p.gA0 = o + 2 * mm, p.gM0 = o + 3 * mm;
+        HIP_CHECK(hipMemsetAsync(o, run == 2 ? 0 : 0xff, 4 * mm * sizeof(double), ctx->stream));
+        if (run < 2) {
+            work.zero();
+            mh_pencil_launches(ctx, p);
+        } else {
+            auto place = [&](double *dst, const double *src, uint32_t rows, uint32_t cols, uint32_t lds) {
+                if (rows && cols) HIP_CHECK(hipMemcpy2DAsync(dst, size_t(m) * sizeof(double), src, size_t(lds) * sizeof(double), size_t(rows) * sizeof(double), cols, hipMemcpyDeviceToDevice, ctx->stream));
+            };
+            place(o + w, p.raw_x, w, w, w);
+            place(o + size_t(w) * m + w, p.raw_w, w, w, w);
+            place(o + size_t(w) * m + 2 * w, p.raw_p, wp, w, wp);
+            if (!trusted) place(o + mm + size_t(w) * m + w, p.raw_m, w, w, w);
+            mh_pencil_chain(ctx, p);
+        }
+        got[run].resize(4 * mm);
+        HIP_CHECK(hipMemcpyAsync(got[run].data(), o, 4 * mm * sizeof(double), hipMemcpyDeviceToHost, ctx->stream));
+        HIP_CHECK(hipStreamSynchronize(ctx->stream));
+    }
+    if (memcmp(got[0].data(), got[1].data(), 4 * mm * sizeof(double)) != 0) mh_throw(MH_EHIP, "pencil check: two runs of the launches on the same inputs differ");
+    auto worst = [&](const std::vector<double> &g, bool lower_of_m_only) {
+        long double ratio = 0;
+        for (int which = 0; which < 4; ++which)
+            for (uint32_t c = 0; c < m; ++c)
+                for (uint32_t r = 0; r < m; ++r) {
+                    if (lower_of_m_only && (which & 1) && r < c) continue;
+                    const size_t e = size_t(c) * m + r;
+                    const long double ref = which & 1 ? ref_m[e] : ref_a[e], bnd = which & 1 ? bnd_m[e] : bnd_a[e], err = std::abs((long double)g[which * mm + e] - ref);
+                    const long double here = !(err == err) || (err > 0 && !(bnd > 0)) ? std::numeric_limits<long double>::infinity() : err > 0 ? err / bnd : 0.0L;
+                    if (here > 1.0L && !(ratio > 1.0L))
+                        fprintf(stderr, "[lab] pencil: %s(%u, %u) = %.17g, restated %.17Lg, bound %.3Lg\n", which == 0 ? "gA" : which == 1 ? "gM" : which == 2 ? "gA0" : "gM0", r, c,
+                                g[which * mm + e], ref, bnd);
+                    ratio = std::max(ratio, here);
+                }
+        return double(ratio);
+    };
+    const double ratio = worst(got[0], false);
+    fprintf(stderr, "[lab] pencil w %u wp %u flags %u: |launches - long double| / bound <= %.3f (the chain: %.3f)\n", w, wp, flags, ratio, worst(got[2], true));
+    return ratio;
+}
 }
 
 extern "C" {
 int mhl_context_bench_dense(mh_context *ctx, int kind, uint64_t n, uint32_t wa, uint32_t wb, uint32_t reps, double *avg_ms) {
-    if (!ctx || !avg_ms || n == 0 || wa == 0 || wb == 0 || reps == 0 || kind < 0 || kind > 3) return MH_EINVAL;
+    if (!ctx || !avg_ms || wa == 0 || kind < 0 || kind > 4) return MH_EINVAL;
+    if (kind == 4 ? wa > 128 || wb > 128 || reps > 15 : n == 0 || wb == 0 || reps == 0) return MH_EINVAL;
     try {
         HIP_CHECK(hipSetDevice(ctx->device));
         std::lock_guard<std::mutex> lock(mh_solve_mutex());
+        if (kind == 4) {
+            *avg_ms = lab_pencil_ratio(ctx, n, wa, wb, reps);
+            return MH_OK;
+        }
         if (kind >= 2) {
             *avg_ms = lab_mapped_update_mismatches(ctx, kind == 3, n, wa, wb);
             return MH_OK;
diff --git a/mesheditor_amd/csrc/mh_common.h b/mesheditor_amd/csrc/mh_common.h
--- a/mesheditor_amd/csrc/mh_common.h
+++ b/mesheditor_amd/csrc/mh_common.h
@@ -565,7 +565,18 @@
     double quality{std::numeric_limits<double>::quiet_NaN()};
 };
 int mh_rr_solve(mh_context *ctx, double *gA, double *gM, uint32_t m, double *evals, double *ework, DevArray<int> &info, uint32_t nwant = 0, bool gm_is_identity = false,
-                std::vector<double> *host_evals = nullptr);
+                std::vector<double> *host_evals = nullptr, const double *saved_symmetric = nullptr);
+struct MhPencil {
+    uint32_t w{0}, wp{0};
+    bool w_implicit{false}, lazy_images{false}, p_implicit{false}, w_block_trusted{false};
+    const double *theta{nullptr}, *linv{nullptr}, *hp{nullptr}, *app{nullptr};
+    const double *raw_x{nullptr}, *raw_w{nullptr}, *raw_p{nullptr}, *raw_m{nullptr};
+    double *work{nullptr};
+    uint32_t b{0};
+    double *gA{nullptr}, *gM{nullptr}, *gA0{nullptr}, *gM0{nullptr};
+};
+void mh_pencil_launches(mh_context *ctx, const MhPencil &p);
+void mh_pencil_chain(mh_context *ctx, const MhPencil &p);
 void mh_spd_inverse_small(mh_context *ctx, const double *a, uint32_t lda, uint32_t w, double *out, uint32_t ldo, int *info);
 void mh_potrf(mh_context *ctx, double *a, uint32_t ld, uint32_t w, int *info);
 void mh_potrf_small(mh_context *ctx, double *a, uint32_t w, int *info);
diff --git a/mesheditor_amd/csrc/mh_eigs.hip b/mesheditor_amd/csrc/mh_eigs.hip
--- a/mesheditor_amd/csrc/mh_eigs.hip
+++ b/mesheditor_amd/csrc/mh_eigs.hip
@@ -34,6 +34,7 @@
     bool no_poly_start = getenv("MH_TEST") && strstr(getenv("MH_TEST"), "no_poly_start");
     bool fresh_structure = getenv("MH_TEST") && strstr(getenv("MH_TEST"), "fresh_structure");
     bool copy_passes = getenv("MH_TEST") && strstr(getenv("MH_TEST"), "copy_passes");
+    bool pencil_chain = getenv("MH_TEST") && strstr(getenv("MH_TEST"), "pencil_chain");
     Switches() {
         if (const char *c = getenv("MH_CYCLE")) {
             double v[5] = {0, 0, 0, 0, 0};
@@ -442,6 +443,118 @@
     const uint32_t r = i % w, c = i / w;
     bw[size_t(c) * ld + r] += v[size_t(c) * w + r] - u[size_t(c) * w + r] - u[size_t(r) * w + c];
 }
+constexpr uint32_t PK_STEPS = 20;
+template<bool TA, bool TB, bool LA, bool LB, typename Out>
+__device__ __forceinline__ void wg_product(uint32_t M, uint32_t N, uint32_t K, const double *A, uint32_t lda, const double *B, uint32_t ldb, Out &&out) {
+    typedef double double4_t __attribute__((ext_vector_type(4)));
+    const uint32_t lane = threadIdx.x & 63u, wave = threadIdx.x >> 6, c_lane = lane & 15u, k_lane = lane >> 4;
+    const uint32_t ti_n = (M + 15u) / 16u, tj_n = (N + 15u) / 16u;
+    const size_t sai = TA ? lda : 1, sak = TA ? 1 : lda, sbk = TB ? ldb : 1, sbj = TB ? 1 : ldb;
+    for (uint32_t t = wave; t < ti_n * tj_n; t += 16u) {
+        const uint32_t i0 = (t % ti_n) * 16u, j0 = (t / ti_n) * 16u, ia = i0 + c_lane, jb = j0 + c_lane;
+        const bool a_ok = ia < M, b_ok = jb < N;
+        const double *ap = A + (a_ok ? ia : 0u) * sai, *bp = B + (b_ok ? jb : 0u) * sbj;
+        uint32_t kend = K;
+        if (LA) kend = min(kend, i0 + 16u);
+        if (LB) kend = min(kend, j0 + 16u);
+        double4_t acc = {0, 0, 0, 0};
+        for (uint32_t k = 0; k < kend; k += 4u * PK_STEPS) {
+            double af[PK_STEPS], bf[PK_STEPS];
+#pragma unroll
+            for (uint32_t u = 0; u < PK_STEPS; ++u) {
+                const uint32_t kk = k + 4u * u + k_lane;
+                af[u] = a_ok && kk < kend && !(LA && kk > ia) ? ap[kk * sak] : 0.0;
+                bf[u] = b_ok && kk < kend && !(LB && kk > jb) ? bp[kk * sbk] : 0.0;
+            }
+#pragma unroll
+            for (uint32_t u = 0; u < PK_STEPS; ++u) acc = __builtin_amdgcn_mfma_f64_16x16x4f64(af[u], bf[u], acc, 0, 0, 0);
+        }
+#pragma unroll
+        for (uint32_t reg = 0; reg < 4; ++reg) {
+            const uint32_t row = i0 + k_lane + 4u * reg;
+            if (row < M && b_ok) out(row, jb, acc[reg]);
+        }
+    }
+}
+
+__global__ void __launch_bounds__(1024) k_pencil_blocks(uint32_t w, uint32_t wp, uint32_t flags, const double *linv, const double *hp, const double *app, const double *raw_x,
+                                                        const double *raw_w, const double *raw_p, const double *raw_m, double *blk_x, double *blk_w, double *blk_p, double *blk_m,
+                                                        double *scr, size_t slot) {
+    const bool w_implicit = flags & 1u, lazy = flags & 2u, p_implicit = (flags & 4u) && wp, trusted = flags & 8u;
+    const uint32_t job = blockIdx.x;
+    auto copy_to = [&](double *dst, const double *src, uint32_t count) {
+        __syncthreads();
+        for (uint32_t i = threadIdx.x; i < count; i += 1024u) dst[i] = src[i];
+    };
+    if (job == 0) {
+        double *t = scr, *u = scr + slot, *v = scr + 2 * slot;
+        const double *cur = raw_w;
+        if (p_implicit) {
+            wg_product<false, false, false, false>(wp, w, wp, app, wp, hp, wp, [&](uint32_t i, uint32_t j, double x) { t[size_t(j) * wp + i] = x; });
+            wg_product<true, false, false, false>(w, w, wp, hp, wp, raw_p, wp, [&](uint32_t i, uint32_t j, double x) { u[size_t(j) * w + i] = x; });
+            __syncthreads();
+            wg_product<true, false, false, false>(w, w, wp, hp, wp, t, wp, [&](uint32_t i, uint32_t j, double x) {
+                v[size_t(j) * w + i] = raw_w[size_t(j) * w + i] + (x - u[size_t(j) * w + i] - u[size_t(i) * w + j]);
+            });
+            cur = v;
+        }
+        if (lazy) {
+            double *dst = w_implicit ? u : blk_w;
+            __syncthreads();
+            wg_product<false, true, false, true>(w, w, w, cur, w, linv, w, [&](uint32_t i, uint32_t j, double x) { dst[size_t(j) * w + i] = x; });
+            cur = dst;
+        }
+        if (w_implicit) {
+            __syncthreads();
+            wg_product<false, false, true, false>(w, w, w, linv, w, cur, w, [&](uint32_t i, uint32_t j, double x) { blk_w[size_t(j) * w + i] = x; });
+            cur = blk_w;
+        }
+        if (cur != blk_w) copy_to(blk_w, cur, w * w);
+    } else if (job == 1) {
+        if (!wp) return;
+        double *t = scr + 3 * slot;
+        const double *cur = raw_p;
+        if (p_implicit) {
+            double *dst = lazy ? t : blk_p;
+            wg_product<false, false, false, false>(wp, w, wp, app, wp, hp, wp, [&](uint32_t i, uint32_t j, double x) { dst[size_t(j) * wp + i] = raw_p[size_t(j) * wp + i] - x; });
+            cur = dst;
+        }
+        if (lazy) {
+            __syncthreads();
+            wg_product<false, true, false, true>(wp, w, w, cur, wp, linv, w, [&](uint32_t i, uint32_t j, double x) { blk_p[size_t(j) * wp + i] = x; });
+            cur = blk_p;
+        }
+        if (cur != blk_p) copy_to(blk_p, cur, wp * w);
+    } else if (job == 2) {
+        if (w_implicit) wg_product<false, false, true, false>(w, w, w, linv, w, raw_x, w, [&](uint32_t i, uint32_t j, double x) { blk_x[size_t(j) * w + i] = x; });
+        else copy_to(blk_x, raw_x, w * w);
+    } else {
+        if (trusted) return;
+        if (lazy) wg_product<false, true, false, true>(w, w, w, raw_m, w, linv, w, [&](uint32_t i, uint32_t j, double x) { blk_m[size_t(j) * w + i] = x; });
+        else copy_to(blk_m, raw_m, w * w);
+    }
+}
+
+__global__ void k_pencil_assemble(uint32_t w, uint32_t wp, uint32_t trusted, const double *__restrict__ theta, const double *__restrict__ app, const double *__restrict__ blk_x,
+                                  const double *__restrict__ blk_w, const double *__restrict__ blk_p, const double *__restrict__ blk_m, double *__restrict__ ga,
+                                  double *__restrict__ gm, double *__restrict__ ga0, double *__restrict__ gm0) {
+    const uint32_t m = 2 * w + wp, e = blockIdx.x * blockDim.x + threadIdx.x;
+    if (e >= m * m) return;
+    const uint32_t r = max(e % m, e / m), c = min(e % m, e / m);
+    double a = 0.0, g = r == c ? 1.0 : 0.0;
+    if (r < w) {
+        if (r == c) a = theta[r];
+    } else if (r < 2 * w) {
+        if (c < w) a = blk_x[size_t(c) * w + (r - w)];
+        else {
+            a = blk_w[size_t(c - w) * w + (r - w)];
+            if (!trusted) g = blk_m[size_t(c - w) * w + (r - w)];
+        }
+    } else if (c >= 2 * w) a = app[size_t(c - 2 * w) * wp + (r - 2 * w)];
+    else if (c >= w) a = blk_p[size_t(c - w) * wp + (r - 2 * w)];
+    ga[e] = a, ga0[e] = a, gm[e] = g, gm0[e] = g;
+}
+
 __global__ void k_load_seed(const float *__restrict__ seed, const uint32_t *__restrict__ perm, uint32_t nnodes, uint32_t ncols, uint32_t b, double *__restrict__ x) {
     const size_t i = size_t(blockIdx.x) * blockDim.x + threadIdx.x;
     if (i >= size_t(nnodes) * 3 * ncols) return;
@@ -641,13 +754,15 @@
     return true;
 }
 
-int eig_tridiag_small(mh_context *ctx, double *gA, uint32_t m, double *evals, double *ework, DevArray<int> &info, uint32_t nwant, std::vector<double> *host_evals) {
+int eig_tridiag_small(mh_context *ctx, double *gA, uint32_t m, double *evals, double *ework, DevArray<int> &info, uint32_t nwant, std::vector<double> *host_evals,
+                      const double *saved_given = nullptr) {
     DevArray<double> z(ctx, size_t(m) * m), tau(ctx, m);
     const bool partial = nwant && nwant < m;
     DevArray<double> zl(ctx, partial ? size_t(m) * nwant : 0);
     double *zres = z.get();
     uint32_t ncols = m;
-    HIP_CHECK(hipMemcpyAsync(z.get(), gA, size_t(m) * m * sizeof(double), hipMemcpyDeviceToDevice, ctx->stream));
+    const double *saved = saved_given ? saved_given : z.get();
+    if (!saved_given) HIP_CHECK(hipMemcpyAsync(z.get(), gA, size_t(m) * m * sizeof(double), hipMemcpyDeviceToDevice, ctx->stream));
     for (int attempt = 0; attempt < 2; ++attempt) {
         mh_sytrd_small(ctx, gA, m, evals, ework, tau, attempt == 0 ? -1 : 0);
         int gave_up = 0;
@@ -662,7 +777,7 @@
                 HIP_CHECK(hipMemcpyAsync(qv, wv.get() + m, sizeof(qv), hipMemcpyDeviceToHost, ctx->stream));
                 if (host_evals) HIP_CHECK(hipMemcpyAsync(lam_host.data(), wv.get(), size_t(nwant) * sizeof(double), hipMemcpyDeviceToHost, ctx->stream));
                 HIP_CHECK(hipStreamSynchronize(ctx->stream));
-                if (flagged && sytrd_gave_up(ctx, gave_up, gA, z, m)) continue;
+                if (flagged && sytrd_gave_up(ctx, gave_up, gA, saved, m)) continue;
                 if (switches().verbose)
                     fprintf(stderr, "[rr] tridiagonal m %u lowest %u: residual / ||T|| %.2e; us: multisection %.0f, inverse iteration %.0f, Gram-Schmidt %.0f, output %.0f\n", m,
                             nwant, qv[0], qv[1] * 0.01, qv[2] * 0.01, qv[3] * 0.01, qv[4] * 0.01);
@@ -676,7 +791,7 @@
         }
         if (flagged) {
             HIP_CHECK(hipStreamSynchronize(ctx->stream));
-            if (sytrd_gave_up(ctx, gave_up, gA, z, m)) continue;
+            if (sytrd_gave_up(ctx, gave_up, gA, saved, m)) continue;
         }
         ROCBLAS_CHECK(rocsolver_dstedc(ctx->blas, rocblas_evect_tridiagonal, m, evals, ework, z, m, info));
         if (const int hinfo = host_info(info)) return hinfo;
@@ -684,7 +799,7 @@
     }
     if (ctx->rr_trace) ctx->rr_trace->solver = ncols < m ? MhRrTrace::SMALL_PARTIAL : MhRrTrace::SMALL_STEDC;
     mh_apply_q(ctx, gA, tau, m, zres, m, ncols);
-    if (zres == zl.get()) rr_selfcheck(ctx, z.get(), m, zres, m, evals, ncols);
+    if (zres == zl.get()) rr_selfcheck(ctx, saved, m, zres, m, evals, ncols);
     HIP_CHECK(hipMemcpyAsync(gA, zres, size_t(m) * ncols * sizeof(double), hipMemcpyDeviceToDevice, ctx->stream));
     return 0;
 }
@@ -724,11 +839,79 @@
 
 }
 
+void mh_pencil_launches(mh_context *ctx, const MhPencil &p) {
+    if (p.w == 0 || p.w > 128 || p.wp > 128 || p.b < std::max(p.w, p.wp)) mh_throw(MH_EINVAL, "pencil: orders %u, %u outside the two-launch form", p.w, p.wp);
+    const size_t slot = size_t(p.b) * p.b;
+    double *blk = p.work, *scr = p.work + 4 * slot;
+    const uint32_t flags = (p.w_implicit ? 1u : 0u) | (p.lazy_images ? 2u : 0u) | (p.p_implicit ? 4u : 0u) | (p.w_block_trusted ? 8u : 0u), m = 2 * p.w + p.wp;
+    k_pencil_blocks<<<4, 1024, 0, ctx->stream>>>(p.w, p.wp, flags, p.linv, p.hp, p.app, p.raw_x, p.raw_w, p.raw_p, p.raw_m, blk, blk + slot, blk + 2 * slot, blk + 3 * slot, scr, slot);
+    KERNEL_CHECK();
+    k_pencil_assemble<<<grid1(size_t(m) * m), TB, 0, ctx->stream>>>(p.w, p.wp, p.w_block_trusted ? 1u : 0u, p.theta, p.app, blk, blk + slot, blk + 2 * slot, blk + 3 * slot, p.gA,
+                                                                   p.gM, p.gA0, p.gM0);
+    KERNEL_CHECK();
+}
+
+void mh_pencil_chain(mh_context *ctx, const MhPencil &p) {
+    const hipStream_t st = ctx->stream;
+    const uint32_t w = p.w, wa = p.w, wp = p.wp, m = 2 * p.w + p.wp;
+    const size_t slot = size_t(p.b) * p.b;
+    double *Up = p.work, *Vp = p.work + slot, *T1p = p.work + 2 * slot;
+    double *gA = p.gA, *gM = p.gM;
+    k_set_identity_blocks<<<grid1(wa), TB, 0, st>>>(gA, gM, p.theta, wa, m);
+    KERNEL_CHECK();
+    const double unit = 1;
+    auto left_corrected = [&](double *block, uint32_t cols) {
+        if (p.w_implicit)
+            ROCBLAS_CHECK(rocblas_dtrmm(ctx->blas, rocblas_side_left, rocblas_fill_lower, rocblas_operation_none, rocblas_diagonal_non_unit, rocblas_int(w), rocblas_int(cols),
+                                        &unit, p.linv, rocblas_int(w), block, rocblas_int(m), block, rocblas_int(m)));
+    };
+    auto untransformed = [&](double *block, uint32_t rows) {
+        if (p.lazy_images)
+            ROCBLAS_CHECK(rocblas_dtrmm(ctx->blas, rocblas_side_right, rocblas_fill_lower, rocblas_operation_transpose, rocblas_diagonal_non_unit, rocblas_int(rows),
+                                        rocblas_int(w), &unit, p.linv, rocblas_int(w), block, rocblas_int(m), block, rocblas_int(m)));
+    };
+    double *bw = gA + size_t(wa) * m + wa, *bp = gA + size_t(wa) * m + wa + w, *mw = gM + size_t(wa) * m + wa;
+    left_corrected(gA + wa, wa);
+    if (p.p_implicit && wp) {
+        const double plus = 1, nil = 0;
+        small_dgemm(ctx, rocblas_operation_transpose, rocblas_operation_none, rocblas_int(w), rocblas_int(w), rocblas_int(wp), &plus, p.hp, rocblas_int(wp), bp, rocblas_int(m), &nil, Up,
+                    rocblas_int(w));
+        small_dgemm(ctx, rocblas_operation_none, rocblas_operation_none, rocblas_int(wp), rocblas_int(w), rocblas_int(wp), &plus, p.app, rocblas_int(wp), p.hp, rocblas_int(wp), &nil, T1p,
+                    rocblas_int(wp));
+        small_dgemm(ctx, rocblas_operation_transpose, rocblas_operation_none, rocblas_int(w), rocblas_int(w), rocblas_int(wp), &plus, p.hp, rocblas_int(wp), T1p, rocblas_int(wp), &nil, Vp,
+                    rocblas_int(w));
+        k_sub_block<<<grid1(size_t(wp) * w), TB, 0, st>>>(bp, m, T1p, wp, wp, w);
+        k_wblock_fix<<<grid1(size_t(w) * w), TB, 0, st>>>(bw, m, Up, Vp, w);
+        KERNEL_CHECK();
+    }
+    untransformed(bw, w);
+    left_corrected(bw, w);
+    if (p.w_block_trusted) {
+        k_place_block<<<grid1(size_t(w) * w), TB, 0, st>>>(mw, m, nullptr, w);
+        KERNEL_CHECK();
+    } else {
+        untransformed(mw, w);
+    }
+    if (wp) {
+        untransformed(bp, wp);
+        k_place_block<<<grid1(size_t(wp) * wp), TB, 0, st>>>(gA + size_t(wa + w) * m + wa + w, m, p.app, wp);
+        k_place_block<<<grid1(size_t(wp) * wp), TB, 0, st>>>(gM + size_t(wa + w) * m + wa + w, m, nullptr, wp);
+        KERNEL_CHECK();
+    }
+    k_symmetrize_lower<<<grid1(size_t(m) * m), TB, 0, st>>>(gA, m, m);
+    KERNEL_CHECK();
+    HIP_CHECK(hipMemcpyAsync(p.gA0, gA, size_t(m) * m * sizeof(double), hipMemcpyDeviceToDevice, st));
+    HIP_CHECK(hipMemcpyAsync(p.gM0, gM, size_t(m) * m * sizeof(double), hipMemcpyDeviceToDevice, st));
+}
+
 int mh_rr_solve(mh_context *ctx, double *gA, double *gM, uint32_t m, double *evals, double *ework, DevArray<int> &info, uint32_t nwant, bool gm_is_identity,
-                std::vector<double> *host_evals) {
+                std::vector<double> *host_evals, const double *saved_symmetric) {
     const double one = 1, zero = 0;
-    k_symmetrize_lower<<<grid1(size_t(m) * m), TB, 0, ctx->stream>>>(gA, m, m);
-    KERNEL_CHECK();
+    if (!gm_is_identity) saved_symmetric = nullptr;
+    if (!saved_symmetric) {
+        k_symmetrize_lower<<<grid1(size_t(m) * m), TB, 0, ctx->stream>>>(gA, m, m);
+        KERNEL_CHECK();
+    }
     bool identity = gm_is_identity, series = false;
     if (!identity) {
         static_assert(sizeof(unsigned long long) == sizeof(double), "defect word");
@@ -770,7 +953,7 @@
         ROCBLAS_CHECK(rocblas_dtrsm(ctx->blas, rocblas_side_right, rocblas_fill_lower, rocblas_operation_transpose, rocblas_diagonal_non_unit, m, m, &one, gM, m, gA, m));
     }
     std::optional<int> hinfo;
-    if (m >= 8 && m <= 256) hinfo = eig_tridiag_small(ctx, gA, m, evals, ework, info, nwant, host_evals);
+    if (m >= 8 && m <= 256) hinfo = eig_tridiag_small(ctx, gA, m, evals, ework, info, nwant, host_evals, saved_symmetric);
     else if (m > 256 && m <= 768 && !ctx->exchange_disabled) hinfo = eig_tridiag_wide(ctx, gA, m, evals, ework, info, nwant);
     if (!hinfo) {
         ROCBLAS_CHECK(rocsolver_dsyevd(ctx->blas, rocblas_evect_original, rocblas_fill_lower, m, gA, m, evals, ework, info));
@@ -1312,7 +1495,7 @@
     std::vector<double> hist_active;
     uint32_t pairs_at_floor = 0;
     DevArray<double> X, AX, MX, Xn, AXn, MXn, W, AW, MW, P, MP, Pn, MPn, R, Rw;
-    DevArray<double> gA, gM, gM0, gA0, App, evals, ework, Cp, T1, H, H2, G, dscale, Linv, theta_d, rn_d, mn_d, scratch, Ct, norms_d, theta_act_d, Hp, Up, Vp, T1p;
+    DevArray<double> gA, gM, gM0, gA0, App, evals, ework, Cp, T1, H, H2, G, dscale, Linv, theta_d, rn_d, mn_d, scratch, Ct, norms_d, theta_act_d, Hp, Pw;
     DevArray<double> Linv_p, T1p2;
     DevArray<uint32_t> idx_d, pos_d;
     DevArray<double> Rr, res_partial, res_blocks, res_norms_d;
@@ -1357,7 +1540,8 @@
         if (!pproj_ok)
             for (DevArray<double> *panel : {&MP, &MPn}) panel->reset(ctx, n * b);
         for (DevArray<double> *small : {&gA, &gM, &gM0, &gA0}) small->reset(ctx, size_t(mmax) * mmax);
-        for (DevArray<double> *small : {&App, &H, &H2, &Linv, &Hp, &Up, &Vp, &T1p}) small->reset(ctx, size_t(b) * b);
+        for (DevArray<double> *small : {&App, &H, &H2, &Linv, &Hp}) small->reset(ctx, size_t(b) * b);
+        Pw.reset(ctx, size_t(b <= 128 ? 12 : 3) * b * b);
         Linv_p.reset(ctx, size_t(b) * b);
         T1p2.reset(ctx, size_t(mmax) * b);
         for (DevArray<double> *small : {&Cp, &T1}) small->reset(ctx, size_t(mmax) * b);
@@ -1736,66 +1920,35 @@
         wa = w;
         m = wa + w + wp;
         for (int attempt = 0; attempt < 2; ++attempt) {
-            HIP_CHECK(hipMemsetAsync(gA, 0, size_t(m) * m * sizeof(double), st));
-            HIP_CHECK(hipMemsetAsync(gM, 0, size_t(m) * m * sizeof(double), st));
-            k_set_identity_blocks<<<grid1(wa), TB, 0, st>>>(gA, gM, theta_act_d, wa, m);
-            KERNEL_CHECK();
-            const double unit_one = 1;
-            auto left_corrected = [&](double *block, uint32_t cols) {
-                if (w_implicit)
-                    ROCBLAS_CHECK(rocblas_dtrmm(ctx->blas, rocblas_side_left, rocblas_fill_lower, rocblas_operation_none, rocblas_diagonal_non_unit, rocblas_int(w),
-                                                rocblas_int(cols), &unit_one, Linv, rocblas_int(w), block, rocblas_int(m), block, rocblas_int(m)));
-            };
-            mh_gram(ctx, n, W, w, AX, wa, gA.get() + wa, m, b, idx_d);
-            left_corrected(gA.get() + wa, wa);
-            const double unit = 1;
-            auto untransformed = [&](double *block, uint32_t rows) {
-                if (lazy_images)
-                    ROCBLAS_CHECK(rocblas_dtrmm(ctx->blas, rocblas_side_right, rocblas_fill_lower, rocblas_operation_transpose, rocblas_diagonal_non_unit, rocblas_int(rows),
-                                                rocblas_int(w), &unit, Linv, rocblas_int(w), block, rocblas_int(m), block, rocblas_int(m)));
-            };
-            gram(ctx, n, W, w, AW, w, gA.get() + size_t(wa) * m + wa, m);
-            if (p_implicit && wp) {
-                const double plus = 1, nil = 0;
-                double *bw = gA.get() + size_t(wa) * m + wa, *bp = gA.get() + size_t(wa) * m + wa + w;
-                gram(ctx, n, P, wp, AW, w, bp, m);
-                small_dgemm(ctx, rocblas_operation_transpose, rocblas_operation_none, rocblas_int(w), rocblas_int(w), rocblas_int(wp), &plus, Hp, rocblas_int(wp), bp,
-                                            rocblas_int(m), &nil, Up, rocblas_int(w));
-                small_dgemm(ctx, rocblas_operation_none, rocblas_operation_none, rocblas_int(wp), rocblas_int(w), rocblas_int(wp), &plus, App, rocblas_int(wp), Hp,
-                                            rocblas_int(wp), &nil, T1p, rocblas_int(wp));
-                small_dgemm(ctx, rocblas_operation_transpose, rocblas_operation_none, rocblas_int(w), rocblas_int(w), rocblas_int(wp), &plus, Hp, rocblas_int(wp), T1p,
-                                            rocblas_int(wp), &nil, Vp, rocblas_int(w));
-                k_sub_block<<<grid1(size_t(wp) * w), TB, 0, st>>>(bp, m, T1p, wp, wp, w);
-                k_wblock_fix<<<grid1(size_t(w) * w), TB, 0, st>>>(bw, m, Up, Vp, w);
-                KERNEL_CHECK();
-            }
-            untransformed(gA.get() + size_t(wa) * m + wa, w);
-            left_corrected(gA.get() + size_t(wa) * m + wa, w);
             const bool w_block_trusted = last_spread < 16 * 8 && !(p_implicit && wp == 0);
             gm_identity = w_block_trusted;
-            if (w_block_trusted) {
-                k_place_block<<<grid1(size_t(w) * w), TB, 0, st>>>(gM.get() + size_t(wa) * m + wa, m, nullptr, w);
-                KERNEL_CHECK();
+            if (verbose) fprintf(stderr, "[lobpcg] it %3u Cholesky-QR diagonal spread 2^%.1f%s\n", it, last_spread / 16.0, w_block_trusted ? "" : " (W block measured)");
+            const bool two_launches = b <= 128 && attempt == 0 && !switches().pencil_chain;
+            MhPencil pen;
+            pen.w = w, pen.wp = wp, pen.b = b;
+            pen.w_implicit = w_implicit, pen.lazy_images = lazy_images, pen.p_implicit = p_implicit, pen.w_block_trusted = w_block_trusted;
+            pen.theta = theta_act_d, pen.linv = Linv, pen.hp = Hp, pen.app = App, pen.work = Pw;
+            pen.gA = gA, pen.gM = gM, pen.gA0 = gA0, pen.gM0 = gM0;
+            if (two_launches) {
+                double *raw = Pw.get() + size_t(8) * b * b;
+                const size_t slot = size_t(b) * b;
+                pen.raw_x = raw, pen.raw_w = raw + slot, pen.raw_p = raw + 2 * slot, pen.raw_m = raw + 3 * slot;
+                mh_gram(ctx, n, W, w, AX, wa, raw, w, b, idx_d);
+                gram(ctx, n, W, w, AW, w, raw + slot, w);
+                if (wp) gram(ctx, n, P, wp, AW, w, raw + 2 * slot, wp);
+                if (!w_block_trusted) gram(ctx, n, W, w, MW, w, raw + 3 * slot, w);
+                mh_pencil_launches(ctx, pen);
             } else {
-                gram(ctx, n, W, w, MW, w, gM.get() + size_t(wa) * m + wa, m);
-                untransformed(gM.get() + size_t(wa) * m + wa, w);
-            }
-            if (verbose) fprintf(stderr, "[lobpcg] it %3u Cholesky-QR diagonal spread 2^%.1f%s\n", it, last_spread / 16.0, w_block_trusted ? "" : " (W block measured)");
-            if (wp) {
-                if (!p_implicit) gram(ctx, n, P, wp, AW, w, gA.get() + size_t(wa) * m + wa + w, m);
-                untransformed(gA.get() + size_t(wa) * m + wa + w, wp);
-                {
-                    k_place_block<<<grid1(size_t(wp) * wp), TB, 0, st>>>(gA.get() + size_t(wa + w) * m + wa + w, m, App, wp);
-                    k_place_block<<<grid1(size_t(wp) * wp), TB, 0, st>>>(gM.get() + size_t(wa + w) * m + wa + w, m, nullptr, wp);
-                    KERNEL_CHECK();
-                }
-            }
-            k_symmetrize_lower<<<grid1(size_t(m) * m), TB, 0, st>>>(gA, m, m);
-            KERNEL_CHECK();
-            HIP_CHECK(hipMemcpyAsync(gA0, gA, size_t(m) * m * sizeof(double), hipMemcpyDeviceToDevice, st));
-            HIP_CHECK(hipMemcpyAsync(gM0, gM, size_t(m) * m * sizeof(double), hipMemcpyDeviceToDevice, st));
+                HIP_CHECK(hipMemsetAsync(gA, 0, size_t(m) * m * sizeof(double), st));
+                HIP_CHECK(hipMemsetAsync(gM, 0, size_t(m) * m * sizeof(double), st));
+                mh_gram(ctx, n, W, w, AX, wa, gA.get() + wa, m, b, idx_d);
+                gram(ctx, n, W, w, AW, w, gA.get() + size_t(wa) * m + wa, m);
+                if (wp) gram(ctx, n, P, wp, AW, w, gA.get() + size_t(wa) * m + wa + w, m);
+                if (!w_block_trusted) gram(ctx, n, W, w, MW, w, gM.get() + size_t(wa) * m + wa, m);
+                mh_pencil_chain(ctx, pen);
+            }
             rr_evals.clear();
-            const int hinfo = mh_rr_solve(ctx, gA, gM, m, evals, ework, info, wa, gm_identity, &rr_evals);
+            const int hinfo = mh_rr_solve(ctx, gA, gM, m, evals, ework, info, wa, gm_identity, &rr_evals, two_launches ? gA0.get() : nullptr);
             if (hinfo == 0) break;
             if (attempt == 1 || wp == 0) mh_throw(MH_ENOTCONVERGED, "Rayleigh-Ritz failed at iteration %u (info %d)", it, hinfo);
             wp = 0;
```

Result: no change. 651.1 eigenpairs/s, median of 6 (+0.7%).
